# MingyuKim87/Safe_Denoiser

Hardware: AMD Instinct MI355X
Metric: images/sec (512x512, 50 steps, SD-v1.4 + repellency) (higher is better)
Workload: dtype bf16; 1 GPU; README-default end to end (safree = svf = lra = true, safree_neg_prompt_config.json:26-28): token ids -> CLIP -> SAFREE projection -> DDPM 50 steps x UNet on 3 guidance branches with per-prompt text switching + safe_denoiser.yaml repellency (kernel_fast, M=515, sigma 3.15, scale .33, margin 1.6, window 780<=t<=1000) -> VAE decode -> uint8 512x512 images; SD-v1.4 UNet / CLIP / VAE with random weigh; guidance_branches=3, text_encoder_precision=bf16x3, prompts_per_batch=64, latent_repeat=3, renoise_draws_rank0=3520, parallelism=prompt-shard x1

## Files before the change

include/sdn.h:

```cpp
#ifndef SDN_H_
#define SDN_H_

#include <stddef.h>
#include <stdint.h>

#ifdef __cplusplus
extern "C" {
#endif

#define SDN_OK            0
#define SDN_E_INVALID    -1
#define SDN_E_LAUNCH     -2
#define SDN_E_WORKSPACE  -3
#define SDN_E_ARCH       -4

int sdn_abi_version(void);
const char* sdn_device_arch_host(void);


#define SDN_REPEL_RBF     0
#define SDN_REPEL_SPARSE  1
#define SDN_QNORM_NONE    0
#define SDN_QNORM_CHANNEL 1
#define SDN_OUT_REPELLED  0
// ... 133 lines not shown
                          int32_t ld_mod, int32_t rows_per_batch, void* out, void* stream);

int sdn_patchify_bf16(const float* latents, int32_t batch, int32_t c, int32_t h, int32_t w, int32_t p, void* out, void* stream);
int sdn_patchify_f16(const float* latents, int32_t batch, int32_t c, int32_t h, int32_t w, int32_t p, void* out, void* stream);
int sdn_unpatchify_f32(const float* tokens, int32_t batch, int32_t c, int32_t h, int32_t w, int32_t p, float* out, void* stream);

int sdn_conv_in_bf16(const float* latents_nchw, const void* w, const float* bias, int32_t batch, int32_t cin,
                     int32_t h, int32_t wd, int32_t cout, void* out_nhwc, void* stream);
int sdn_conv_in_f16(const float* latents_nchw, const void* w, const float* bias, int32_t batch, int32_t cin,
                    int32_t h, int32_t wd, int32_t cout, void* out_nhwc, void* stream);

int sdn_timestep_embed_bf16(float timestep, int32_t batch, int32_t dim, void* out, void* stream);
int sdn_timestep_embed_f16(float timestep, int32_t batch, int32_t dim, void* out, void* stream);

int sdn_gemm_f32(const sdn_gemm_desc* d_host, const void* a, const void* a2, const void* w,
                 const float* bias, const float* rowbias, const float* rowgate, const void* residual, void* out,
                 void* stream);
int sdn_groupnorm_f32(const void* x, const void* x2, int32_t batch, int32_t hw, int32_t c1, int32_t c2,
                      int32_t groups, float eps, int32_t silu, const float* gamma, const float* beta,
                      void* out, float* stats_ws, void* stream);
int sdn_layernorm_f32(const void* x, int64_t rows, int32_t c, float eps, const float* gamma,
                      const float* beta, void* out, void* stream);
int sdn_attention_f32(const void* q, const void* k, const void* v, void* out, int32_t batch, int32_t heads,
                      int32_t nq, int32_t nk, int32_t head_dim, int32_t ldq, int32_t ldk, int32_t ldv,
                      int32_t ldo, float scale, void* stream);
int sdn_conv_in_f32(const float* latents_nchw, const void* w, const float* bias, int32_t batch, int32_t cin,
                    int32_t h, int32_t wd, int32_t cout, void* out_nhwc, void* stream);
int sdn_timestep_embed_f32(float timestep, int32_t batch, int32_t dim, void* out, void* stream);

int sdn_gemm_x3(const sdn_gemm_desc* d_host, const void* a, const void* a2, const void* w,
                const float* bias, const float* rowbias, const float* rowgate, const void* residual, void* out,
                void* stream);
int sdn_attention_x3(const void* q, const void* k, const void* v, void* out, int32_t batch, int32_t heads,
                     int32_t nq, int32_t nk, int32_t head_dim, int32_t ldq, int32_t ldk, int32_t ldv,
                     int32_t ldo, float scale, void* stream);

int sdn_layernorm_mod_f32(const void* x, int64_t rows, int32_t c, float eps, const float* scale, const float* shift,
                          int32_t ld_mod, int32_t rows_per_batch, void* out, void* stream);
int sdn_patchify_f32(const float* latents, int32_t batch, int32_t c, int32_t h, int32_t w, int32_t p, void* out, void* stream);
int sdn_joint_attention_f32(int32_t mode, const void* q, const void* k, const void* v, void* out,
                            const sdn_attn_segment2* seg2_host, int32_t batch, int32_t heads, int32_t n_total,
                            int32_t head_dim, int32_t ldq, int32_t ldk, int32_t ldv, int32_t ldo, float scale,
                            void* stream);

int sdn_split3(const float* x, const float* x2, int64_t rows, int32_t c1, int32_t c2, void* out_triple, void* stream);
int sdn_expand3_weights(const float* w, int64_t rows, int32_t cols, int32_t group, void* out_bf16, void* stream);
int sdn_groupnorm_f32_triple(const void* x, const void* x2, int32_t batch, int32_t hw, int32_t c1, int32_t c2, int32_t groups,
                             float eps, int32_t silu, const float* gamma, const float* beta, void* out_triple, float* stats_ws,
                             void* stream);
int sdn_layernorm_f32_triple(const void* x, int64_t rows, int32_t c, float eps, const float* gamma, const float* beta,
                             void* out_triple, void* stream);
int sdn_attention_x3_triple(const void* q, const void* k, const void* v, void* out_triple, int32_t batch, int32_t heads, int32_t nq,
                            int32_t nk, int32_t head_dim, int32_t ldq, int32_t ldk, int32_t ldv, int32_t ldo, float scale,
                            void* stream);
int sdn_attention_x3_pairs(const void* q, const void* k, const void* v, int32_t lo_offset_q, int32_t lo_offset_kv, void* out,
                           int32_t batch, int32_t heads, int32_t nq, int32_t nk, int32_t head_dim, int32_t ldq, int32_t ldk,
                           int32_t ldv, int32_t ldo, float scale, int32_t triple_out, void* stream);

int sdn_randn_philox_plan(int64_t numel, int32_t* grid_out, int64_t* offset_increment_out);
int sdn_randn_philox(const uint64_t* seeds, const uint64_t* offsets, const int32_t* rows, int32_t n_gen, int64_t numel,
                     float* out, void* stream);
int sdn_randn_philox_state(const uint64_t* seeds, uint64_t* offsets, const int32_t* flags, int32_t n_gen, int64_t numel,
                           float* out, void* stream);

typedef struct sdn_unet_config {
  int32_t in_channels, out_channels, sample_size;
  int32_t n_levels;
  int32_t block_out_channels[4];
  int32_t level_has_attn[4];
  int32_t layers_per_block;
  int32_t n_heads;
  int32_t cross_dim, text_len;
  int32_t norm_groups;
  int32_t dtype;
  int32_t latent_repeat;
} sdn_unet_config;

typedef struct sdn_unet sdn_unet;

#define SDN_P_VEC_F32     0
#define SDN_P_MAT         1
#define SDN_P_CONV3X3     2
#define SDN_P_GEGLU_MAT   3
#define SDN_P_GEGLU_VEC   4
#define SDN_P_POS_CROP    5
#define SDN_P_GLU_VALUE   7
#define SDN_P_GLU_GATE    8
#define SDN_P_DERIVED     6

typedef struct sdn_param_info {
  char     name[128];
  int32_t  kind;
  int32_t  rows, cols;
  int32_t  rows_padded;
  int64_t  offset;
} sdn_param_info;

int    sdn_unet_create(const sdn_unet_config* cfg_host, sdn_unet** out_host);
void   sdn_unet_destroy(sdn_unet* u);
int    sdn_unet_param_count(const sdn_unet* u);
int    sdn_unet_param_info(const sdn_unet* u, int32_t index, sdn_param_info* info_host);
size_t sdn_unet_weight_bytes(const sdn_unet* u);
size_t sdn_unet_workspace_bytes(sdn_unet* u, int32_t batch);
double sdn_unet_flops(sdn_unet* u, int32_t batch, double* attention_core_flops_host);

int sdn_unet_forward(sdn_unet* u, const void* weights, const float* latents, float timestep, const void* text,
                     float* out, int32_t batch, void* workspace, size_t workspace_bytes, void* stream);

typedef struct sdn_mmdit_config {
  int32_t in_channels, out_channels;
  int32_t sample_size, patch_size;
  int32_t num_layers;
  int32_t num_heads, head_dim;
  int32_t joint_dim, pooled_dim;
  int32_t text_len;
  int32_t time_dim;
  int32_t dtype;
} sdn_mmdit_config;
int sdn_mmdit_create(const sdn_mmdit_config* cfg_host, sdn_unet** out_host);
int sdn_mmdit_forward(sdn_unet* m, const void* weights, const float* latents, float timestep, const void* text,
                      const void* pooled, float* out, int32_t batch, void* workspace, size_t workspace_bytes,
                      void* stream);

int sdn_ln_fold(int32_t dtype, const void* w, const float* gamma, const float* beta, const float* bias, int32_t rows,
                int32_t cols, void* w_folded, float* c, float* d, void* stream);
int sdn_gemm_ln_bf16(const sdn_gemm_desc* desc, const void* a, const void* w_folded, const float* c, const float* d, float eps,
                     const float* row_stats, void* out, void* stream);
int sdn_gemm_ln_f16(const sdn_gemm_desc* desc, const void* a, const void* w_folded, const float* c, const float* d, float eps,
                    const float* row_stats, void* out, void* stream);
int sdn_row_stats_bf16(const void* x, int64_t rows, int32_t c, float eps, float* out, void* stream);
int sdn_row_stats_f16(const void* x, int64_t rows, int32_t c, float eps, float* out, void* stream);

int sdn_ffn_geglu_fused(int32_t dtype, int64_t M, int32_t C, const void* x, const float* row_stats, const void* w1_folded,
                        const float* c1, const float* d1, const void* w_cat, const float* b_cat, const void* residual, void* out,
                        float* col_stats, void* stream);

int sdn_gemm_stats_bf16(const sdn_gemm_desc* desc, const void* a, const void* a2, const void* w, const float* bias,
                        const float* rowbias, const void* residual, void* out, float* col_stats, void* stream);
int sdn_gemm_stats_f16(const sdn_gemm_desc* desc, const void* a, const void* a2, const void* w, const float* bias,
                       const float* rowbias, const void* residual, void* out, float* col_stats, void* stream);
int sdn_groupnorm_cols_bf16(const void* x, const void* x2, int32_t batch, int32_t hw, int32_t c1, int32_t c2, int32_t groups,
                            float eps, int32_t silu, const float* gamma, const float* beta, void* out, float* stats_ws,
                            const float* cols1, const float* cols2, void* stream);
int sdn_groupnorm_cols_f16(const void* x, const void* x2, int32_t batch, int32_t hw, int32_t c1, int32_t c2, int32_t groups,
                           float eps, int32_t silu, const float* gamma, const float* beta, void* out, float* stats_ws,
                           const float* cols1, const float* cols2, void* stream);

int sdn_gemm_splitk_bf16(const sdn_gemm_desc* d, const void* a, const void* a2, const void* w, const float* bias,
                         const float* rowbias, const float* rowgate, const void* residual, void* out, void* partials,
                         size_t partial_bytes, void* stream);
int sdn_gemm_splitk_f16(const sdn_gemm_desc* d, const void* a, const void* a2, const void* w, const float* bias,
                        const float* rowbias, const float* rowgate, const void* residual, void* out, void* partials,
                        size_t partial_bytes, void* stream);

int sdn_repeat(const void* in, size_t bytes, int32_t rep, void* out, void* stream);

int sdn_unet_prepare(sdn_unet* u, void* weights, void* stream);

typedef struct sdn_vae_config {
  int32_t latent_channels, out_channels;
  int32_t sample_size;
  int32_t n_levels;
  int32_t block_out_channels[4];
  int32_t layers_per_block;
  int32_t norm_groups;
  int32_t dtype;
} sdn_vae_config;
int sdn_vae_decoder_create(const sdn_vae_config* cfg_host, sdn_unet** out_host);
int sdn_vae_decode(sdn_unet* vae, const void* weights, const float* latents, float latent_scale, float* image,
                   int32_t batch, void* workspace, size_t workspace_bytes, void* stream);
int sdn_vae_encoder_create(const sdn_vae_config* cfg_host, sdn_unet** out_host);
int sdn_vae_encode(sdn_unet* vae_encoder, const void* weights, const float* image, float* moments, int32_t batch,
                   void* workspace, size_t workspace_bytes, void* stream);
int sdn_gaussian_sample(const float* moments, const float* noise, int32_t batch, int32_t latent_channels, int32_t hw,
                        float scale, float* out, void* stream);
int sdn_image_postprocess(const float* image_nchw, int32_t batch, int32_t channels, int32_t height, int32_t width,
                          float* out_nhwc01, uint8_t* out_nhwc_u8, void* stream);
int sdn_latent_mix(const float* z, const float* w, const float* bias, int32_t batch, int32_t channels, int32_t hw,
                   float in_scale, float* out, void* stream);
int sdn_softmax_rows(int32_t dtype, const float* scores, int64_t ld_scores, int64_t rows, int32_t n, float scale,
                     void* out, int64_t ld_out, void* stream);
int sdn_transpose16(const void* in, int32_t rows, int32_t cols, int64_t ld_in, void* out, int64_t ld_out, void* stream);

typedef struct sdn_clip_config {
  int32_t vocab_size;
  int32_t hidden_size, intermediate_size;
  int32_t num_layers, num_heads;
  int32_t max_position_embeddings;
  int32_t dtype;
} sdn_clip_config;
int sdn_clip_create(const sdn_clip_config* cfg_host, sdn_unet** out_host);
int sdn_clip_forward(sdn_unet* clip, const void* weights, const int32_t* input_ids, const int32_t* attention_mask,
                     void* last_hidden_state, int32_t batch, void* workspace, size_t workspace_bytes, void* stream);
int sdn_clip_embed(int32_t dtype, const int32_t* input_ids, const void* token_embedding, const void* position_embedding,
                   int64_t rows, int32_t seq_len, int32_t hidden, int32_t vocab, void* out, void* stream);
int sdn_masked_attention(int32_t dtype, const void* q, const void* k, const void* v, void* out, const int32_t* key_mask,
                         int32_t causal, int32_t batch, int32_t heads, int32_t n, int32_t head_dim, int32_t ldq,
                         int32_t ldk, int32_t ldv, int32_t ldo, float scale, void* stream);
int sdn_clip_embed_f32(const int32_t* input_ids, const void* token_embedding, const void* position_embedding, int64_t rows,
                       int32_t seq_len, int32_t hidden, int32_t vocab, void* out, void* stream);
int sdn_masked_attention_f32(const void* q, const void* k, const void* v, void* out, const int32_t* key_mask, int32_t causal,
                             int32_t batch, int32_t heads, int32_t n, int32_t head_dim, int32_t ldq, int32_t ldk, int32_t ldv,
                             int32_t ldo, float scale, void* stream);

typedef struct sdn_clip_proj_config {
  int32_t vocab_size;
  int32_t hidden_size, intermediate_size;
  int32_t num_layers, num_heads;
  int32_t max_position_embeddings;
  int32_t dtype;
  int32_t projection_dim;
  int32_t act;
  int32_t eos_token_id;
  int32_t hidden_tap;
} sdn_clip_proj_config;
int sdn_clip_proj_create(const sdn_clip_proj_config* cfg_host, sdn_unet** out_host);
int sdn_clip_proj_forward(sdn_unet* clip, const void* weights, const int32_t* input_ids, void* hidden, int64_t hidden_batch_stride,
                          int64_t hidden_row_stride, void* text_embeds, int64_t embeds_row_stride, int32_t batch, void* workspace,
                          size_t workspace_bytes, void* stream);
int sdn_clip_eos_rows(int32_t dtype, const int32_t* input_ids, const void* x, const float* gamma, const float* beta, int32_t batch,
                      int32_t seq_len, int32_t hidden, int32_t vocab, int32_t eos_token_id, float eps, void* out,
                      int32_t* positions, void* stream);
int sdn_copy_rows_strided(const void* src, int32_t batch, int32_t rows_per_batch, int32_t cols, int32_t elem_bytes, void* dst,
                          int64_t dst_batch_stride, int64_t dst_row_stride, void* stream);

typedef struct sdn_clip_vision_config {
  int32_t image_size, patch_size;
  int32_t hidden_size, intermediate_size;
  int32_t num_layers, num_heads;
  int32_t projection_dim;
  int32_t act;
  int32_t dtype;
} sdn_clip_vision_config;
int sdn_clip_vision_create(const sdn_clip_vision_config* cfg_host, sdn_unet** out_host);
int sdn_clip_vision_forward(sdn_unet* vision, const void* weights, const float* pixel_values, void* last_hidden_state,
                            void* image_embeds, int32_t batch, void* workspace, size_t workspace_bytes, void* stream);
int sdn_clip_patch_rows(int32_t dtype, const float* pixels, int32_t batch, int32_t image_size, int32_t patch_size, int32_t kpad,
                        void* out, void* stream);
int sdn_clip_vision_embed(int32_t dtype, const void* patch_proj, const float* class_embedding, const void* position_embedding,
                          const float* gamma, const float* beta, int32_t batch, int32_t tokens, int32_t hidden, float eps, void* out,
                          void* stream);
int sdn_clip_class_rows(int32_t dtype, const void* x, const float* gamma, const float* beta, int32_t batch, int32_t seq_len,
                        int32_t hidden, float eps, void* out, void* stream);
int sdn_image_resize_u8(const uint8_t* in, int32_t batch, int32_t in_size, int32_t out_size, const int32_t* coeffs,
                        const int32_t* bounds, int32_t ksize, uint8_t* tmp, uint8_t* out, void* stream);
int sdn_clip_normalize_u8(const uint8_t* in, int32_t batch, int32_t size, float mean_r, float mean_g, float mean_b, float std_r,
                          float std_g, float std_b, float* out, void* stream);
int sdn_embed_row_scores(const void* x, int32_t dtype_x, int64_t ldx, const void* y, int32_t dtype_y, int64_t ldy,
                         int32_t y_rows, int32_t rows, int32_t dim, int32_t normalize_y, float scale, float bias,
                         float* out, void* stream);
int sdn_image_resize_rect_u8(const uint8_t* in, int32_t batch, int32_t in_h, int32_t in_w, int32_t out_h, int32_t out_w,
                             const int32_t* coeffs_x, const int32_t* bounds_x, int32_t ksize_x, const int32_t* coeffs_y,
                             const int32_t* bounds_y, int32_t ksize_y, uint8_t* tmp, uint8_t* out_u8, float* out_f32, float mean_r,
                             float mean_g, float mean_b, float std_r, float std_g, float std_b, void* stream);

typedef struct sdn_t5_config {
  int32_t vocab_size;
  int32_t d_model, d_kv, d_ff;
  int32_t num_layers, num_heads;
  int32_t num_buckets, max_distance;
  float   eps;
  int32_t dtype;
} sdn_t5_config;
int sdn_t5_create(const sdn_t5_config* cfg_host, sdn_unet** out_host);
size_t sdn_t5_workspace_bytes(sdn_unet* t5, int32_t batch, int32_t n);
double sdn_t5_flops(sdn_unet* t5, int32_t batch, int32_t n, double* attention_core_flops_host);
int sdn_t5_forward(sdn_unet* t5, const void* weights, const int32_t* input_ids, const int32_t* attention_mask, int32_t n,
                   void* out, int32_t batch, void* workspace, size_t workspace_bytes, void* stream);
int sdn_rmsnorm(int32_t dtype, const void* x, int32_t x_is_f32, int64_t rows, int32_t c, float eps, const float* weight, void* out,
                void* stream);
int sdn_embed_tokens(int32_t dtype, const int32_t* input_ids, const void* token_embedding, int64_t rows, int32_t hidden,
                     int32_t vocab, float* out, void* stream);
int sdn_t5_bucket(int32_t relative_position, int32_t num_buckets, int32_t max_distance);
int sdn_t5_relative_bias(int32_t dtype, const void* table, int32_t num_buckets, int32_t max_distance, int32_t heads, int32_t n,
                         float* out, void* stream);
int sdn_bias_attention(int32_t dtype, const void* q, const void* k, const void* v, void* out, const float* bias,
                       const int32_t* key_mask, int32_t batch, int32_t heads, int32_t n, int32_t head_dim, int32_t ldq,
                       int32_t ldk, int32_t ldv, int32_t ldo, float scale, void* stream);

void sdn_unet_set_text_version(sdn_unet* u, uint64_t version);

void sdn_unet_set_graph_mode(sdn_unet* u, int32_t on);
void sdn_unet_set_split_k(sdn_unet* u, int32_t on);

typedef struct sdn_profile_row {
  char    kernel[24];
  int32_t launches;
  double  ms;
  double  flops;
  double  bytes;
} sdn_profile_row;
void sdn_unet_profile_next(sdn_unet* u);
int  sdn_unet_profile_read(sdn_unet* u, sdn_profile_row* rows_host, int32_t max_rows);

#ifdef __cplusplus
}
#endif
#endif
```

safe_denoiser_amd/_lib.py:

```python
from __future__ import annotations

import ctypes as C
import os

import torch

_HERE = os.path.dirname(os.path.abspath(__file__))
_LIB = None


class SdnUnavailable(RuntimeError):
    """libsdn.so is missing/unloadable, or there is no gfx950 device for a compute call."""


class SdnError(RuntimeError):
    """A libsdn entry point returned a negative status."""


_ERR = {-1: "SDN_E_INVALID (bad shape / null or misaligned pointer)", -2: "SDN_E_LAUNCH", -3: "SDN_E_WORKSPACE",
        -4: "SDN_E_ARCH"}


def lib_path() -> str:
    return os.environ.get("SDN_LIB", os.path.join(_HERE, "libsdn.so"))
# ... 44 lines not shown
class ClipProjConfig(C.Structure):
    _fields_ = [(n, C.c_int32) for n in ("vocab_size", "hidden_size", "intermediate_size", "num_layers", "num_heads",
                                         "max_position_embeddings", "dtype", "projection_dim", "act", "eos_token_id", "hidden_tap")]


class ClipVisionConfig(C.Structure):
    _fields_ = [(n, C.c_int32) for n in ("image_size", "patch_size", "hidden_size", "intermediate_size", "num_layers", "num_heads",
                                         "projection_dim", "act", "dtype")]


class T5Config(C.Structure):
    _fields_ = [(n, C.c_int32) for n in ("vocab_size", "d_model", "d_kv", "d_ff", "num_layers", "num_heads", "num_buckets",
                                         "max_distance")] + [("eps", C.c_float), ("dtype", C.c_int32)]


class AttnSegment2(C.Structure):
    _fields_ = [("q2", C.c_void_p), ("k2", C.c_void_p), ("v2", C.c_void_p), ("out2", C.c_void_p), ("n1", C.c_int32),
                ("ldq2", C.c_int32), ("ldk2", C.c_int32), ("ldv2", C.c_int32), ("ldo2", C.c_int32)]


class ParamInfo(C.Structure):
    _fields_ = [("name", C.c_char * 128), ("kind", C.c_int32), ("rows", C.c_int32), ("cols", C.c_int32),
                ("rows_padded", C.c_int32), ("offset", C.c_int64)]


_vp, _i32, _i64, _f32, _sz = C.c_void_p, C.c_int32, C.c_int64, C.c_float, C.c_size_t

SIGNATURES = {
    "sdn_abi_version": (C.c_int, []),
    "sdn_device_arch_host": (C.c_char_p, []),
    "sdn_repel_workspace_bytes": (_sz, [_i32, _i32, _i32, _i32]),
    "sdn_repel_apply": (C.c_int, [C.POINTER(RepelParams), _vp, _vp, _vp, _vp, _vp, _vp, _sz, _vp]),
    "sdn_repel_calibrate": (C.c_int, [C.POINTER(RepelParams), _vp, _vp, _vp, _vp, _sz, _vp]),
    "sdn_cfg_combine": (C.c_int, [_vp, _i32, _i32, _i64, _f32, _vp, _vp]),
    "sdn_sld_guidance": (C.c_int, [_vp, _i32, _i64, _f32, _f32, _f32, _f32, _f32, _i32, _vp, _vp, _vp]),
    "sdn_cfg_combine_rows": (C.c_int, [_vp, _i32, _i32, _i64, _vp, _vp, _vp]),
    "sdn_sld_guidance_rows": (C.c_int, [_vp, _i32, _i64, _vp, _f32, _f32, _f32, _f32, _i32, _vp, _vp, _vp]),
    "sdn_pred_x0": (C.c_int, [_vp, _vp, _i64, _f32, _f32, _f32, _vp, _vp]),
    "sdn_sched_step": (C.c_int, [_vp, _vp, _vp, _i64, _f32, _f32, _f32, _f32, _f32, _f32, _f32, _vp, _vp]),
    "sdn_add_noise": (C.c_int, [_vp, _vp, _i64, _f32, _f32, _vp, _vp]),
    "sdn_renoise_select": (C.c_int, [_vp, _vp, _vp, _vp, _i32, _i64, _f32, _f32, _vp]),
    "sdn_flow_euler_step": (C.c_int, [_vp, _vp, _i64, _f32, _f32, _vp, _vp]),
    "sdn_flow_endpoints": (C.c_int, [_vp, _vp, _i64, _f32, _vp, _vp, _vp]),
    "sdn_flow_renoise": (C.c_int, [_vp, _vp, _vp, _i64, _f32, _vp, _vp]),
    "sdn_gemm_bf16": (C.c_int, [C.POINTER(GemmDesc), _vp, _vp, _vp, _vp, _vp, _vp, _vp, _vp, _vp]),
    "sdn_gemm_f16": (C.c_int, [C.POINTER(GemmDesc), _vp, _vp, _vp, _vp, _vp, _vp, _vp, _vp, _vp]),
    "sdn_ln_fold": (C.c_int, [_i32, _vp, _vp, _vp, _vp, _i32, _i32, _vp, _vp, _vp, _vp]),
    "sdn_gemm_ln_bf16": (C.c_int, [C.POINTER(GemmDesc), _vp, _vp, _vp, _vp, _f32, _vp, _vp, _vp]),
    "sdn_gemm_ln_f16": (C.c_int, [C.POINTER(GemmDesc), _vp, _vp, _vp, _vp, _f32, _vp, _vp, _vp]),
    "sdn_row_stats_bf16": (C.c_int, [_vp, _i64, _i32, _f32, _vp, _vp]),
    "sdn_row_stats_f16": (C.c_int, [_vp, _i64, _i32, _f32, _vp, _vp]),
    "sdn_ffn_geglu_fused": (C.c_int, [_i32, _i64, _i32, _vp, _vp, _vp, _vp, _vp, _vp, _vp, _vp, _vp, _vp, _vp]),
    "sdn_gemm_stats_bf16": (C.c_int, [C.POINTER(GemmDesc), _vp, _vp, _vp, _vp, _vp, _vp, _vp, _vp, _vp]),
    "sdn_gemm_stats_f16": (C.c_int, [C.POINTER(GemmDesc), _vp, _vp, _vp, _vp, _vp, _vp, _vp, _vp, _vp]),
    "sdn_groupnorm_cols_bf16": (C.c_int, [_vp, _vp, _i32, _i32, _i32, _i32, _i32, _f32, _i32, _vp, _vp, _vp, _vp, _vp, _vp, _vp]),
    "sdn_groupnorm_cols_f16": (C.c_int, [_vp, _vp, _i32, _i32, _i32, _i32, _i32, _f32, _i32, _vp, _vp, _vp, _vp, _vp, _vp, _vp]),
    "sdn_gemm_splitk_bf16": (C.c_int, [C.POINTER(GemmDesc), _vp, _vp, _vp, _vp, _vp, _vp, _vp, _vp, _vp, _sz, _vp]),
    "sdn_gemm_splitk_f16": (C.c_int, [C.POINTER(GemmDesc), _vp, _vp, _vp, _vp, _vp, _vp, _vp, _vp, _vp, _sz, _vp]),
    "sdn_groupnorm_bf16": (C.c_int, [_vp, _vp, _i32, _i32, _i32, _i32, _i32, _f32, _i32, _vp, _vp, _vp, _vp, _vp]),
    "sdn_groupnorm_f16": (C.c_int, [_vp, _vp, _i32, _i32, _i32, _i32, _i32, _f32, _i32, _vp, _vp, _vp, _vp, _vp]),
    "sdn_layernorm_f16": (C.c_int, [_vp, _i64, _i32, _f32, _vp, _vp, _vp, _vp]),
    "sdn_conv_in_f16": (C.c_int, [_vp, _vp, _vp, _i32, _i32, _i32, _i32, _i32, _vp, _vp]),
    "sdn_timestep_embed_f16": (C.c_int, [_f32, _i32, _i32, _vp, _vp]),
    "sdn_layernorm_bf16": (C.c_int, [_vp, _i64, _i32, _f32, _vp, _vp, _vp, _vp]),
    "sdn_attention_bf16": (C.c_int, [_vp, _vp, _vp, _vp, _i32, _i32, _i32, _i32, _i32, _i32, _i32, _i32, _i32, _f32,
                                     _vp]),
    "sdn_attention_f16": (C.c_int, [_vp, _vp, _vp, _vp, _i32, _i32, _i32, _i32, _i32, _i32, _i32, _i32, _i32, _f32,
                                    _vp]),
    "sdn_conv_in_bf16": (C.c_int, [_vp, _vp, _vp, _i32, _i32, _i32, _i32, _i32, _vp, _vp]),
    "sdn_timestep_embed_bf16": (C.c_int, [_f32, _i32, _i32, _vp, _vp]),
    "sdn_gemm_f32": (C.c_int, [C.POINTER(GemmDesc), _vp, _vp, _vp, _vp, _vp, _vp, _vp, _vp, _vp]),
    "sdn_groupnorm_f32": (C.c_int, [_vp, _vp, _i32, _i32, _i32, _i32, _i32, _f32, _i32, _vp, _vp, _vp, _vp, _vp]),
    "sdn_layernorm_f32": (C.c_int, [_vp, _i64, _i32, _f32, _vp, _vp, _vp, _vp]),
    "sdn_attention_f32": (C.c_int, [_vp, _vp, _vp, _vp, _i32, _i32, _i32, _i32, _i32, _i32, _i32, _i32, _i32, _f32, _vp]),
    "sdn_randn_philox_plan": (C.c_int, [C.c_int64, C.POINTER(C.c_int32), C.POINTER(C.c_int64)]),
    "sdn_randn_philox": (C.c_int, [_vp, _vp, _vp, _i32, C.c_int64, _vp, _vp]),
    "sdn_randn_philox_state": (C.c_int, [_vp, _vp, _vp, _i32, C.c_int64, _vp, _vp]),
    "sdn_gemm_x3": (C.c_int, [C.POINTER(GemmDesc), _vp, _vp, _vp, _vp, _vp, _vp, _vp, _vp, _vp]),
    "sdn_attention_x3": (C.c_int, [_vp, _vp, _vp, _vp, _i32, _i32, _i32, _i32, _i32, _i32, _i32, _i32, _i32, _f32, _vp]),
    "sdn_conv_in_f32": (C.c_int, [_vp, _vp, _vp, _i32, _i32, _i32, _i32, _i32, _vp, _vp]),
    "sdn_timestep_embed_f32": (C.c_int, [_f32, _i32, _i32, _vp, _vp]),
    "sdn_unet_create": (C.c_int, [C.POINTER(UnetConfig), C.POINTER(_vp)]),
    "sdn_unet_destroy": (None, [_vp]),
    "sdn_unet_param_count": (C.c_int, [_vp]),
    "sdn_unet_param_info": (C.c_int, [_vp, _i32, C.POINTER(ParamInfo)]),
    "sdn_unet_weight_bytes": (_sz, [_vp]),
    "sdn_unet_workspace_bytes": (_sz, [_vp, _i32]),
    "sdn_unet_flops": (C.c_double, [_vp, _i32, C.POINTER(C.c_double)]),
    "sdn_unet_forward": (C.c_int, [_vp, _vp, _vp, _f32, _vp, _vp, _i32, _vp, _sz, _vp]),
    "sdn_mmdit_create": (C.c_int, [C.POINTER(MmditConfig), C.POINTER(_vp)]),
    "sdn_mmdit_forward": (C.c_int, [_vp, _vp, _vp, _f32, _vp, _vp, _vp, _i32, _vp, _sz, _vp]),
    "sdn_joint_attention": (C.c_int, [_i32, _vp, _vp, _vp, _vp, C.POINTER(AttnSegment2), _i32, _i32, _i32, _i32, _i32,
                                      _i32, _i32, _i32, _f32, _vp]),
    "sdn_layernorm_mod_bf16": (C.c_int, [_vp, _i64, _i32, _f32, _vp, _vp, _i32, _i32, _vp, _vp]),
    "sdn_layernorm_mod_f16": (C.c_int, [_vp, _i64, _i32, _f32, _vp, _vp, _i32, _i32, _vp, _vp]),
    "sdn_patchify_bf16": (C.c_int, [_vp, _i32, _i32, _i32, _i32, _i32, _vp, _vp]),
    "sdn_patchify_f16": (C.c_int, [_vp, _i32, _i32, _i32, _i32, _i32, _vp, _vp]),
    "sdn_unpatchify_f32": (C.c_int, [_vp, _i32, _i32, _i32, _i32, _i32, _vp, _vp]),
    "sdn_layernorm_mod_f32": (C.c_int, [_vp, _i64, _i32, _f32, _vp, _vp, _i32, _i32, _vp, _vp]),
    "sdn_patchify_f32": (C.c_int, [_vp, _i32, _i32, _i32, _i32, _i32, _vp, _vp]),
    "sdn_joint_attention_f32": (C.c_int, [_i32, _vp, _vp, _vp, _vp, C.POINTER(AttnSegment2), _i32, _i32, _i32, _i32, _i32,
                                          _i32, _i32, _i32, _f32, _vp]),
    "sdn_repeat": (C.c_int, [_vp, _sz, _i32, _vp, _vp]),
    "sdn_vae_decoder_create": (C.c_int, [C.POINTER(VaeConfig), C.POINTER(_vp)]),
    "sdn_vae_decode": (C.c_int, [_vp, _vp, _vp, _f32, _vp, _i32, _vp, _sz, _vp]),
    "sdn_vae_encoder_create": (C.c_int, [C.POINTER(VaeConfig), C.POINTER(_vp)]),
    "sdn_vae_encode": (C.c_int, [_vp, _vp, _vp, _vp, _i32, _vp, _sz, _vp]),
    "sdn_gaussian_sample": (C.c_int, [_vp, _vp, _i32, _i32, _i32, _f32, _vp, _vp]),
    "sdn_image_postprocess": (C.c_int, [_vp, _i32, _i32, _i32, _i32, _vp, _vp, _vp]),
    "sdn_latent_mix": (C.c_int, [_vp, _vp, _vp, _i32, _i32, _i32, _f32, _vp, _vp]),
    "sdn_softmax_rows": (C.c_int, [_i32, _vp, _i64, _i64, _i32, _f32, _vp, _i64, _vp]),
    "sdn_transpose16": (C.c_int, [_vp, _i32, _i32, _i64, _vp, _i64, _vp]),
    "sdn_clip_create": (C.c_int, [C.POINTER(ClipConfig), C.POINTER(_vp)]),
    "sdn_clip_forward": (C.c_int, [_vp, _vp, _vp, _vp, _vp, _i32, _vp, _sz, _vp]),
    "sdn_clip_embed": (C.c_int, [_i32, _vp, _vp, _vp, _i64, _i32, _i32, _i32, _vp, _vp]),
    "sdn_masked_attention": (C.c_int, [_i32, _vp, _vp, _vp, _vp, _vp, _i32, _i32, _i32, _i32, _i32, _i32, _i32, _i32, _i32,
                                       _f32, _vp]),
    "sdn_clip_proj_create": (C.c_int, [C.POINTER(ClipProjConfig), C.POINTER(_vp)]),
    "sdn_clip_proj_forward": (C.c_int, [_vp, _vp, _vp, _vp, _i64, _i64, _vp, _i64, _i32, _vp, _sz, _vp]),
    "sdn_clip_eos_rows": (C.c_int, [_i32, _vp, _vp, _vp, _vp, _i32, _i32, _i32, _i32, _i32, _f32, _vp, _vp, _vp]),
    "sdn_copy_rows_strided": (C.c_int, [_vp, _i32, _i32, _i32, _i32, _vp, _i64, _i64, _vp]),
    "sdn_clip_vision_create": (C.c_int, [C.POINTER(ClipVisionConfig), C.POINTER(_vp)]),
    "sdn_clip_vision_forward": (C.c_int, [_vp, _vp, _vp, _vp, _vp, _i32, _vp, _sz, _vp]),
    "sdn_clip_patch_rows": (C.c_int, [_i32, _vp, _i32, _i32, _i32, _i32, _vp, _vp]),
    "sdn_clip_vision_embed": (C.c_int, [_i32, _vp, _vp, _vp, _vp, _vp, _i32, _i32, _i32, _f32, _vp, _vp]),
    "sdn_clip_class_rows": (C.c_int, [_i32, _vp, _vp, _vp, _i32, _i32, _i32, _f32, _vp, _vp]),
    "sdn_image_resize_u8": (C.c_int, [_vp, _i32, _i32, _i32, _vp, _vp, _i32, _vp, _vp, _vp]),
    "sdn_clip_normalize_u8": (C.c_int, [_vp, _i32, _i32, _f32, _f32, _f32, _f32, _f32, _f32, _vp, _vp]),
    "sdn_image_resize_rect_u8": (C.c_int, [_vp, _i32, _i32, _i32, _i32, _i32, _vp, _vp, _i32, _vp, _vp, _i32, _vp, _vp, _vp, _f32, _f32,
                                           _f32, _f32, _f32, _f32, _vp]),
    "sdn_embed_row_scores": (C.c_int, [_vp, _i32, _i64, _vp, _i32, _i64, _i32, _i32, _i32, _i32, _f32, _f32, _vp, _vp]),
    "sdn_t5_create": (C.c_int, [C.POINTER(T5Config), C.POINTER(_vp)]),
    "sdn_t5_workspace_bytes": (_sz, [_vp, _i32, _i32]),
    "sdn_t5_flops": (C.c_double, [_vp, _i32, _i32, C.POINTER(C.c_double)]),
    "sdn_t5_forward": (C.c_int, [_vp, _vp, _vp, _vp, _i32, _vp, _i32, _vp, _sz, _vp]),
    "sdn_rmsnorm": (C.c_int, [_i32, _vp, _i32, _i64, _i32, _f32, _vp, _vp, _vp]),
    "sdn_embed_tokens": (C.c_int, [_i32, _vp, _vp, _i64, _i32, _i32, _vp, _vp]),
    "sdn_t5_bucket": (C.c_int, [_i32, _i32, _i32]),
    "sdn_t5_relative_bias": (C.c_int, [_i32, _vp, _i32, _i32, _i32, _i32, _vp, _vp]),
    "sdn_bias_attention": (C.c_int, [_i32, _vp, _vp, _vp, _vp, _vp, _vp, _i32, _i32, _i32, _i32, _i32, _i32, _i32, _i32, _f32,
                                     _vp]),
    "sdn_split3": (C.c_int, [_vp, _vp, _i64, _i32, _i32, _vp, _vp]),
    "sdn_expand3_weights": (C.c_int, [_vp, _i64, _i32, _i32, _vp, _vp]),
    "sdn_groupnorm_f32_triple": (C.c_int, [_vp, _vp, _i32, _i32, _i32, _i32, _i32, _f32, _i32, _vp, _vp, _vp, _vp, _vp]),
    "sdn_layernorm_f32_triple": (C.c_int, [_vp, _i64, _i32, _f32, _vp, _vp, _vp, _vp]),
    "sdn_attention_x3_triple": (C.c_int, [_vp, _vp, _vp, _vp, _i32, _i32, _i32, _i32, _i32, _i32, _i32, _i32, _i32, _f32, _vp]),
    "sdn_attention_x3_pairs": (C.c_int, [_vp, _vp, _vp, _i32, _i32, _vp, _i32, _i32, _i32, _i32, _i32, _i32, _i32, _i32, _i32, _f32, _i32, _vp]),
    "sdn_clip_embed_f32": (C.c_int, [_vp, _vp, _vp, _i64, _i32, _i32, _i32, _vp, _vp]),
    "sdn_masked_attention_f32": (C.c_int, [_vp, _vp, _vp, _vp, _vp, _i32, _i32, _i32, _i32, _i32, _i32, _i32, _i32, _i32, _f32, _vp]),
    "sdn_unet_prepare": (C.c_int, [_vp, _vp, _vp]),
    "sdn_unet_set_graph_mode": (None, [_vp, _i32]),
    "sdn_unet_set_text_version": (None, [_vp, C.c_uint64]),
    "sdn_unet_set_split_k": (None, [_vp, _i32]),
    "sdn_unet_profile_next": (None, [_vp]),
    "sdn_unet_profile_read": (C.c_int, [_vp, C.POINTER(ProfileRow), _i32]),
}


def lib():
    global _LIB
    if _LIB is None:
        path = lib_path()
        if not os.path.exists(path):
            raise SdnUnavailable(f"{path} not found: build it with `python -c 'import __graft_entry__ as g; g.build()'` "
                                 f"(or `make -C safe_denoiser_amd/csrc`).  There is no CPU fallback.")
        try:
            handle = C.CDLL(path)
        except OSError as e:
            raise SdnUnavailable(f"cannot load {path}: {e}") from e
        for name, (res, args) in SIGNATURES.items():
            fn = getattr(handle, name)
            fn.restype, fn.argtypes = res, args
        _LIB = handle
    return _LIB


def check(rc: int, what: str):
    if rc != 0:
        raise SdnError(f"{what} failed: {_ERR.get(rc, rc)}")


def require_gpu():
    if not torch.cuda.is_available():
        raise SdnUnavailable("no GPU visible: the safe-denoiser hot path only runs on an MI355X (gfx950); "
                             "there is no CPU fallback")


def dptr(t: torch.Tensor | None, dtype=None) -> int | None:
    if t is None:
        return None
    if not t.is_cuda:
        raise SdnUnavailable("tensor is not on the GPU: libsdn takes device pointers only (no CPU fallback)")
    if not t.is_contiguous():
        raise SdnError("tensor must be contiguous")
    if dtype is not None and t.dtype != dtype:
        raise SdnError(f"expected {dtype}, got {t.dtype}")
    return t.data_ptr()


def stream_ptr() -> int:
    return torch.cuda.current_stream().cuda_stream
```

safe_denoiser_amd/csrc/sdn_gemm.hip:

```cpp
#include <stdlib.h>

#include <type_traits>

#include "sdn_common.h"
#include "sdn_ops.h"

static int g_gemm_variant = 0;
static unsigned long long* g_gemm_stamps = nullptr;

#include "sdn_gemm_common.h"

namespace sdn_gemm_detail {

#define SDN_STAMP(IDX)                                                                                   \
  if (g.stamps && threadIdx.x == 0) {                                                                    \
    unsigned long long t_;                                                                               \
    asm volatile("s_memtime %0\n\ts_waitcnt lgkmcnt(0)" : "=s"(t_)::"memory");                          \
    g.stamps[(long)blockIdx.x * 8 + (IDX)] = t_;                                                         \
  }

template <typename T, int NREP, int WGM, int NSTAGE, int LNF, bool H8>
__device__ __forceinline__ void gemm_dma_body(const GemmArgs& g) {
#if defined(__HIP_DEVICE_COMPILE__)
  SDN_STAMP(0)
  constexpr int BM = 64 * WGM, THREADS = 128 * WGM, NWAVES = 2 * WGM;
  constexpr int BN = 32 * NREP;
  constexpr int A_PIECES = BM / 8 / NWAVES;
  constexpr int W_PIECES = (BN / 8 + NWAVES - 1) / NWAVES;
  constexpr int STAGE = (BM + BN) * 128;
  constexpr unsigned OOB = 0x80000000u;
  constexpr int LPI = A_PIECES + W_PIECES;
  static_assert(NSTAGE == 2 || (BN / 8) % NWAVES == 0, "counted waits need the same number of loads in every wave");
  __shared__ __attribute__((aligned(1024))) unsigned char smem[NSTAGE * STAGE];

  const int nt = g.tiles_m * g.tiles_n;
  const int tid = threadIdx.x, lane = tid & 63;
  const int wid = __builtin_amdgcn_readfirstlane(tid >> 6);
  const int wm = wid >> 1, wn = wid & 1;
  const int lrow = lane >> 3;
  int tile;
  {
    const int vid = blockIdx.x;
    const int q = nt >> 3, r = nt & 7, x = vid & 7;
    tile = (x < r ? x * (q + 1) : r * (q + 1) + (x - r) * q) + (vid >> 3);
  }
  int tm = tile / g.tiles_n, tn = tile - tm * g.tiles_n;
  if (g.panel) {
    const int per_blk = 8 * g.tiles_n;
    const int blk = tile / per_blk, rem = tile - blk * per_blk;
    const int rows = min(8, g.tiles_m - blk * 8);
    const int full = rows * g.panel;
    const int p = rem / full, r2 = rem - p * full;
    const int w = min(g.panel, g.tiles_n - p * g.panel);
    const int tl = r2 / w;
    tm = blk * 8 + tl; tn = p * g.panel + (r2 - tl * w);
  }
  const int m0 = tm * BM, n0 = tn * BN;
  const int lchunk = (lane & 7) ^ lrow;

  unsigned a_base[A_PIECES];
  unsigned a_aux[A_PIECES];
  const int ld1 = g.a_mode == 1 ? g.Cin : g.K1, ld2 = g.K - g.K1;
  if (g.a_mode == 1) {
    const int hw = g.Ho * g.Wo;
    const int Hi = g.upsample ? g.Hs * 2 : g.Hs, Wi = g.upsample ? g.Ws * 2 : g.Ws;
    const int mb = m0 + wid * A_PIECES * 8 + lrow;
    const int mm0 = mb < g.M ? mb : 0;
    int bb = mm0 / hw;
    int oy, ox;
    { const int p = mm0 - bb * hw; oy = p / g.Wo; ox = p - oy * g.Wo; }
#pragma unroll
    for (int i = 0; i < A_PIECES; ++i) {
      const int m = mb + i * 8;
      const bool ok = m < g.M;
      if (i > 0) {
        if (g.Wo >= 8) {
          ox += 8;
          if (ox >= g.Wo) { ox -= g.Wo; if (++oy >= g.Ho) { oy = 0; ++bb; } }
        } else {
          const int mm = ok ? m : 0;
          bb = mm / hw;
          const int p = mm - bb * hw;
          oy = p / g.Wo; ox = p - oy * g.Wo;
        }
      }
      const int cy = oy * g.stride + g.conv_off, cx = ox * g.stride + g.conv_off;
      const unsigned rb = (cy >= 1 ? 1u : 0u) | (cy < Hi ? 2u : 0u) | (cy + 1 < Hi ? 4u : 0u);
      const unsigned cb = (cx >= 1 ? 1u : 0u) | (cx < Wi ? 2u : 0u) | (cx + 1 < Wi ? 4u : 0u);
      unsigned mask = ((rb & 1u) ? cb : 0u) | ((rb & 2u) ? cb << 3 : 0u) | ((rb & 4u) ? cb << 6 : 0u);
      if (!ok) mask = 0u;
      a_aux[i] = mask | ((unsigned)(cy & 1) << 9) | ((unsigned)(cx & 1) << 10);
      const int sy = g.upsample ? cy >> 1 : cy, sx = g.upsample ? cx >> 1 : cx;
      a_base[i] = ok ? (unsigned)((((bb * g.Hs + sy) * g.Ws + sx) * g.Cin + lchunk * 8) * 2) : 0u;
    }
  } else {
#pragma unroll
    for (int i = 0; i < A_PIECES; ++i) {
      const int m = m0 + (wid * A_PIECES + i) * 8 + lrow;
      const bool ok = m < g.M;
      a_base[i] = ok ? (unsigned)(((long)m * ld1 + lchunk * 8) * 2) : OOB;
      a_aux[i] = (g.a2 && ok) ? (unsigned)(((long)m * ld2 + lchunk * 8) * 2) : OOB;
    }
  }
  unsigned w_off[W_PIECES];
  bool w_ok[W_PIECES];
#pragma unroll
  for (int i = 0; i < W_PIECES; ++i) {
    const int piece = wid * W_PIECES + i;
    w_ok[i] = piece * 8 < BN;
    w_off[i] = (unsigned)(((long)(n0 + piece * 8 + lrow) * g.K + lchunk * 8) * 2);
  }
  const __amdgpu_buffer_rsrc_t rs_w = make_rsrc(g.w, (unsigned)((long)g.N * g.K * 2));
  const long a_rows = g.a_mode == 1 ? (long)(g.M / (g.Ho * g.Wo)) * g.Hs * g.Ws : (long)g.M;
  const __amdgpu_buffer_rsrc_t rs_a1 = make_rsrc(g.a, (unsigned)(a_rows * ld1 * 2));
  const __amdgpu_buffer_rsrc_t rs_a2 = make_rsrc(g.a2 ? g.a2 : g.a, (unsigned)(g.a2 ? a_rows * ld2 * 2 : 0));

  const int kt0 = g.kt_per_split > 0 ? (int)blockIdx.y * g.kt_per_split : 0;
  int cur_k0 = kt0 * BK, cur_c0 = (kt0 / 9) * BK, cur_ty = (kt0 % 9) / 3, cur_tx = kt0 % 3, w_k0 = 0;
  auto issue_aw = [&](int buf, bool with_w) {
    unsigned char* sa = smem + buf * STAGE;
    unsigned char* sw = sa + BM * 128;
    if (g.a_mode == 1) {
      const int dy = cur_ty - 1, dx = cur_tx - 1, tap = cur_ty * 3 + cur_tx;
      if (!g.upsample) {
        const int delta = ((dy * g.Ws + dx) * g.Cin + cur_c0) * 2;
#pragma unroll
        for (int i = 0; i < A_PIECES; ++i) {
          const unsigned off = ((a_aux[i] >> tap) & 1u) ? a_base[i] + (unsigned)delta : OOB;
          __builtin_amdgcn_raw_ptr_buffer_load_lds(rs_a1, (lds_ptr_t)(sa + (wid * A_PIECES + i) * 1024), 16, off, 0, 0, 0);
        }
      } else {
#pragma unroll
        for (int i = 0; i < A_PIECES; ++i) {
          const int sy = ((int)((a_aux[i] >> 9) & 1u) + dy) >> 1, sx = ((int)((a_aux[i] >> 10) & 1u) + dx) >> 1;
          const int delta = ((sy * g.Ws + sx) * g.Cin + cur_c0) * 2;
          const unsigned off = ((a_aux[i] >> tap) & 1u) ? a_base[i] + (unsigned)delta : OOB;
          __builtin_amdgcn_raw_ptr_buffer_load_lds(rs_a1, (lds_ptr_t)(sa + (wid * A_PIECES + i) * 1024), 16, off, 0, 0, 0);
        }
      }
      w_k0 = (cur_ty * 3 + cur_tx) * g.Cin + cur_c0;
      if (++cur_tx == 3) { cur_tx = 0; if (++cur_ty == 3) { cur_ty = 0; cur_c0 += BK; } }
    } else {
      if (cur_k0 >= g.K1) {
        const unsigned kb = (unsigned)((cur_k0 - g.K1) * 2);
#pragma unroll
        for (int i = 0; i < A_PIECES; ++i)
          __builtin_amdgcn_raw_ptr_buffer_load_lds(rs_a2, (lds_ptr_t)(sa + (wid * A_PIECES + i) * 1024), 16, a_aux[i] + kb, 0, 0, 0);
      } else {
        const unsigned kb = (unsigned)(cur_k0 * 2);
#pragma unroll
        for (int i = 0; i < A_PIECES; ++i)
          __builtin_amdgcn_raw_ptr_buffer_load_lds(rs_a1, (lds_ptr_t)(sa + (wid * A_PIECES + i) * 1024), 16, a_base[i] + kb, 0, 0, 0);
      }
    }
    if (!with_w) return;
#pragma unroll
    for (int i = 0; i < W_PIECES; ++i) {
      if (w_ok[i])
        __builtin_amdgcn_raw_ptr_buffer_load_lds(rs_w, (lds_ptr_t)(sw + (wid * W_PIECES + i) * 1024), 16,
                                                 w_off[i] + (unsigned)((g.a_mode == 1 ? w_k0 : cur_k0) * 2), 0, 0, 0);
    }
    cur_k0 += BK;
  };
  auto issue = [&](int buf) { issue_aw(buf, true); };
  auto issue_w_only = [&](int buf) {
    unsigned char* sw = smem + buf * STAGE + BM * 128;
#pragma unroll
    for (int i = 0; i < W_PIECES; ++i) {
      if (w_ok[i])
        __builtin_amdgcn_raw_ptr_buffer_load_lds(rs_w, (lds_ptr_t)(sw + (wid * W_PIECES + i) * 1024), 16,
                                                 w_off[i] + (unsigned)((g.a_mode == 1 ? w_k0 : cur_k0) * 2), 0, 0, 0);
    }
    cur_k0 += BK;
  };

  const int fr = lane & 15, fq = lane >> 4;
  const int nk = g.kt_per_split > 0 ? min(g.kt_per_split, g.K / BK - kt0) : g.K / BK;
  SDN_STAMP(7)
  if constexpr (NSTAGE == 2) issue(0);
  f32x4 acc[4][NREP];
  if (g.bias) {
    f32x4 bv[NREP];
#pragma unroll
    for (int j = 0; j < NREP; ++j) bv[j] = *reinterpret_cast<const f32x4*>(g.bias + n0 + wn * 16 * NREP + j * 16 + fq * 4);
#pragma unroll
    for (int i = 0; i < 4; ++i)
#pragma unroll
      for (int j = 0; j < NREP; ++j) acc[i][j] = bv[j];
  } else {
#pragma unroll
    for (int i = 0; i < 4; ++i)
#pragma unroll
      for (int j = 0; j < NREP; ++j) acc[i][j] = (f32x4){0.f, 0.f, 0.f, 0.f};
  }
  if (g.rowbias) {
#pragma unroll
    for (int i = 0; i < 4; ++i) {
      const int m = m0 + wm * 64 + i * 16 + fr;
      const int b = m < g.M ? m / g.rows_per_batch : 0;
      const float* rbp = g.rowbias + (long)b * g.ld_rowbias + n0 + wn * 16 * NREP + fq * 4;
#pragma unroll
      for (int j = 0; j < NREP; ++j) acc[i][j] += *reinterpret_cast<const f32x4*>(rbp + j * 16);
    }
  }

  if (g.res_pre) {
    const unsigned short* r16 = reinterpret_cast<const unsigned short*>(g.res_pre);
#pragma unroll
    for (int i = 0; i < 4; ++i) {
      const int m = m0 + wm * 64 + i * 16 + fr;
      const unsigned short* rp = r16 + (long)(m < g.M ? m : 0) * g.ldc + n0 + wn * 16 * NREP + fq * 4;
#pragma unroll
      for (int j = 0; j < NREP; ++j) {
        const uint2 rr = *reinterpret_cast<const uint2*>(rp + j * 16);
        acc[i][j][0] += T::to_f(rr.x & 0xffff); acc[i][j][1] += T::to_f(rr.x >> 16);
        acc[i][j][2] += T::to_f(rr.y & 0xffff); acc[i][j][3] += T::to_f(rr.y >> 16);
      }
    }
  }
  if (g.x3_out && g.residual) {
    const float* resf = reinterpret_cast<const float*>(g.residual);
#pragma unroll
    for (int i = 0; i < 4; ++i) {
      const int m = m0 + wm * 64 + i * 16 + fr;
      const float* rp = resf + (long)(m < g.M ? m : 0) * g.ldc + n0 + wn * 16 * NREP + fq * 4;
#pragma unroll
      for (int j = 0; j < NREP; ++j) acc[i][j] += *reinterpret_cast<const f32x4*>(rp + j * 16);
    }
  }

  if constexpr (NSTAGE == 2) {
    asm volatile("s_waitcnt vmcnt(0)" ::: "memory");
    __syncthreads();
  } else {
#pragma unroll
    for (int s = 0; s < NSTAGE - 1; ++s) issue(s);
    asm volatile("s_waitcnt vmcnt(%0)" ::"n"((NSTAGE - 2) * LPI) : "memory");
    __builtin_amdgcn_s_barrier();
  }
  SDN_STAMP(1)

  [[maybe_unused]] float ln_s1[4] = {0.f, 0.f, 0.f, 0.f}, ln_s2[4] = {0.f, 0.f, 0.f, 0.f};
  [[maybe_unused]] float ln_mu[4], ln_rs[4];
  if constexpr (LNF == 2) {
#pragma unroll
    for (int i = 0; i < 4; ++i) {
      const int m = m0 + wm * 64 + i * 16 + fr;
      const float2 st2 = *reinterpret_cast<const float2*>(g.ln_stats + 2 * (long)(m < g.M ? m : 0));
      ln_mu[i] = st2.x; ln_rs[i] = st2.y;
    }
  }
  auto k_iter = [&](const int kt, auto f8_c) __attribute__((always_inline)) {
    const int buf = kt & (NSTAGE - 1);
    int ipos = (NSTAGE == 2 && WGM == 4 && !(g.dbg & 8)) ? ((g.dbg & 4) ? 1 : (g.a_mode == 1 ? 2 : ((g.act == 2 && g.K >= 1280) ? 1 : 4))) : 0;
    if (NSTAGE == 2 && WGM == 4 && !(g.dbg & (32 | 8 | 4))) ipos = ((wid >= 4) != ((g.dbg & 64) != 0)) ? 0 : ((g.dbg & 128) ? ipos : 2);
    const bool more = kt + NSTAGE - 1 < nk && !(g.dbg & 2);
    if (ipos == 0 && more) issue((kt + NSTAGE - 1) & (NSTAGE - 1));
    const unsigned char* sa = smem + buf * STAGE + (wm * 64) * 128;
    const unsigned char* sw = smem + buf * STAGE + BM * 128 + (wn * 16 * NREP) * 128;
#ifdef SDN_NO_FRAG_PIPE
    constexpr bool kFragPipe = false;
#else
    constexpr bool kFragPipe = WGM == 4 && (NREP == 10 || NREP == 8) && LNF != 1;
#endif
    constexpr bool f8_tile = decltype(f8_c)::value;
    if constexpr (H8 && f8_tile) {
      {
        typedef __attribute__((ext_vector_type(8))) int i32x8;
        union F8 { typename T::v8 h[2]; i32x8 v; };
        const bool seg1 = kt < g.h8_t16 + (nk - g.h8_t16) / 2;
        const int s_act = seg1 ? 0x74747474 : 0x7f7f7f7f, s_w = seg1 ? 0x7f7f7f7f : 0x74747474;
        F8 av[4], wv[3];
#pragma unroll
        for (int i = 0; i < 4; ++i) {
          av[i].h[0] = *reinterpret_cast<const typename T::v8*>(sa + lds_off(i * 16 + fr, fq));
          av[i].h[1] = *reinterpret_cast<const typename T::v8*>(sa + lds_off(i * 16 + fr, 4 + fq));
        }
#pragma unroll
        for (int j = 0; j < 2; ++j) {
          wv[j].h[0] = *reinterpret_cast<const typename T::v8*>(sw + lds_off(j * 16 + fr, fq));
          wv[j].h[1] = *reinterpret_cast<const typename T::v8*>(sw + lds_off(j * 16 + fr, 4 + fq));
        }
        __builtin_amdgcn_sched_barrier(0);
#pragma unroll
        for (int j = 0; j < NREP; ++j) {
          if (j + 2 < NREP) {
            wv[(j + 2) % 3].h[0] = *reinterpret_cast<const typename T::v8*>(sw + lds_off((j + 2) * 16 + fr, fq));
            wv[(j + 2) % 3].h[1] = *reinterpret_cast<const typename T::v8*>(sw + lds_off((j + 2) * 16 + fr, 4 + fq));
          }
          __builtin_amdgcn_sched_barrier(0);
          __builtin_amdgcn_s_setprio(1);
#pragma unroll
          for (int i = 0; i < 4; ++i)
            acc[i][j] = __builtin_amdgcn_mfma_scale_f32_16x16x128_f8f6f4(wv[j % 3].v, av[i].v, acc[i][j], 0, 0, 0, s_w, 0, s_act);
          __builtin_amdgcn_s_setprio(0);
          __builtin_amdgcn_sched_barrier(0);
          if (j == NREP / 2 - 1 && more && ipos != 0) issue((kt + 1) & 1);
        }
      }
    }
    if constexpr (kFragPipe) {
      if constexpr (!f8_tile) {
      typename T::v8 fa[2][4], fw[2][2];
#pragma unroll
      for (int i = 0; i < 4; ++i) fa[0][i] = *reinterpret_cast<const typename T::v8*>(sa + lds_off(i * 16 + fr, fq));
#pragma unroll
      for (int j = 0; j < 2; ++j) fw[0][j] = *reinterpret_cast<const typename T::v8*>(sw + lds_off(j * 16 + fr, fq));
      constexpr int G = NREP / 2;
#pragma unroll
      for (int gi = 0; gi < 2 * G; ++gi) {
        const int ks = gi / G, g = gi % G;
        if (gi + 1 < 2 * G) {
          const int ks1 = (gi + 1) / G, g1 = (gi + 1) % G;
#pragma unroll
          for (int j = 0; j < 2; ++j)
            fw[(gi + 1) & 1][j] = *reinterpret_cast<const typename T::v8*>(sw + lds_off((2 * g1 + j) * 16 + fr, ks1 * 4 + fq));
        }
        if (gi == 2) {
#pragma unroll
          for (int i = 0; i < 4; ++i) fa[1][i] = *reinterpret_cast<const typename T::v8*>(sa + lds_off(i * 16 + fr, 4 + fq));
        }
        __builtin_amdgcn_s_setprio(1);
#pragma unroll
        for (int i = 0; i < 4; ++i)
#pragma unroll
          for (int j = 0; j < 2; ++j) acc[i][2 * g + j] = T::mfma16(fw[gi & 1][j], fa[ks][i], acc[i][2 * g + j]);
        __builtin_amdgcn_s_setprio(0);
        if (gi == 2 && more) { if (ipos == 1) issue((kt + 1) & 1); else if (ipos == 4) issue_aw((kt + 1) & 1, false); }
        if (gi == G - 1 && more) { if (ipos == 2) issue((kt + 1) & 1); else if (ipos == 4) issue_w_only((kt + 1) & 1); }
      }
      }
    } else {
#pragma unroll
    for (int ks = 0; ks < 2; ++ks) {
      constexpr int JC = NREP > 5 ? NREP / 2 : NREP;
      typename T::v8 fa[4];
#pragma unroll
      for (int i = 0; i < 4; ++i) fa[i] = *reinterpret_cast<const typename T::v8*>(sa + lds_off(i * 16 + fr, ks * 4 + fq));
      if constexpr (LNF == 1) {
#pragma unroll
        for (int i = 0; i < 4; ++i) { ln_s1[i] = T::dot_ones(fa[i], ln_s1[i]); ln_s2[i] = T::dot_self(fa[i], ln_s2[i]); }
      }
#define SDN_MMA_PART(J0)                                                                                              \
      {                                                                                                                \
        typename T::v8 fw[JC];                                                                                         \
        _Pragma("unroll") for (int j = 0; j < JC; ++j)                                                                 \
          fw[j] = *reinterpret_cast<const typename T::v8*>(sw + lds_off(((J0) + j) * 16 + fr, ks * 4 + fq));          \
        _Pragma("unroll") for (int i = 0; i < 4; ++i)                                                                  \
          _Pragma("unroll") for (int j = 0; j < JC; ++j)                                                               \
            acc[i][(J0) + j] = T::mfma16(fw[j], fa[i], acc[i][(J0) + j]);                                              \
      }
      __builtin_amdgcn_s_setprio(1);
      SDN_MMA_PART(0)
      __builtin_amdgcn_s_setprio(0);
      if (ipos == 1 && ks == 0 && more) issue((kt + 1) & 1);
      if (ipos == 4 && ks == 0 && more) issue_aw((kt + 1) & 1, false);
      __builtin_amdgcn_s_setprio(1);
      if constexpr (NREP > JC) SDN_MMA_PART(JC)
      __builtin_amdgcn_s_setprio(0);
#undef SDN_MMA_PART
      if (ipos == 2 && ks == 0 && more) issue((kt + 1) & 1);
      if (ipos == 4 && ks == 0 && more) issue_w_only((kt + 1) & 1);
    }
    }
    if constexpr (NSTAGE == 2) {
      asm volatile("s_waitcnt vmcnt(0)" ::: "memory");
      __syncthreads();
    } else {
      const int later = nk - kt - 2;
      if (later >= NSTAGE - 2) asm volatile("s_waitcnt vmcnt(%0)" ::"n"((NSTAGE - 2) * LPI) : "memory");
      else if (later == 1 && NSTAGE > 3) asm volatile("s_waitcnt vmcnt(%0)" ::"n"(LPI) : "memory");
      else asm volatile("s_waitcnt vmcnt(0)" ::: "memory");
      asm volatile("s_waitcnt lgkmcnt(0)" ::: "memory");
      __builtin_amdgcn_s_barrier();
    }
    };
  if constexpr (H8) {
    for (int kt = 0; kt < g.h8_t16; ++kt) k_iter(kt, std::false_type{});
    for (int kt = g.h8_t16; kt < nk; ++kt) k_iter(kt, std::true_type{});
  } else {
    for (int kt = 0; kt < nk; ++kt) k_iter(kt, std::false_type{});
  }

  SDN_STAMP(2)
  if constexpr (LNF == 1) {
    const float invk = 1.0f / (float)g.K;
#pragma unroll
    for (int i = 0; i < 4; ++i) {
      float a1 = ln_s1[i], a2 = ln_s2[i];
      a1 += __shfl_xor(a1, 16, 64); a2 += __shfl_xor(a2, 16, 64);
      a1 += __shfl_xor(a1, 32, 64); a2 += __shfl_xor(a2, 32, 64);
      const float mu = a1 * invk;
      const float var = fmaxf(a2 * invk - mu * mu, 0.f);
      ln_mu[i] = mu; ln_rs[i] = __builtin_amdgcn_rsqf(var + g.ln_eps);
    }
  }
  constexpr int CW_PAD = (BN + 8) * 2;
  const bool staged = g.out_kind == 0 && g.n_valid == g.N;
  const int out_cols = g.act == 2 ? BN / 2 : BN;
  const bool res_lds = staged && g.res_lds;
  const int CW = res_lds ? BN * 2 : CW_PAD;
  const bool lean = staged && !g.rowgate && g.act == 0 && (res_lds || !g.residual);
  const bool lean_gelu = staged && !g.rowgate && g.act == 3 && !g.residual;
  const bool lean_erf = g.act == SDN_ACT_GELU;
  const bool lean_gate = staged && g.rowgate && g.act == 0 && res_lds;
  const __amdgpu_buffer_rsrc_t rs_res = make_rsrc(g.residual ? g.residual : g.a, g.res_bytes);
  constexpr int PASSES = (BM * CW_PAD + 2 * STAGE - 1) / (2 * STAGE);
  constexpr int WM_PER_PASS = WGM / PASSES, ROWS_PER_PASS = 64 * WM_PER_PASS;
  static_assert(WGM % PASSES == 0, "pass split must divide the wave rows");
  static_assert(PASSES <= 2, "epilogue is written for at most two staging passes");
#define SDN_PASS 0
#include "sdn_gemm_epilogue.inc"
#undef SDN_PASS
  if constexpr (PASSES > 1) {
#define SDN_PASS 1
#include "sdn_gemm_epilogue.inc"
#undef SDN_PASS
  }
  SDN_STAMP(3)
#endif
}

template <typename T, int NREP, int WGM, int NSTAGE, int LNF = 0>
__global__ void __launch_bounds__(128 * WGM, NSTAGE > 2 ? 1 : 2)
k_gemm_dma(const GemmArgs g) { gemm_dma_body<T, NREP, WGM, NSTAGE, LNF, false>(g); }

template <typename T, int NREP>
__global__ void __launch_bounds__(512, 2)
k_gemm_h8(const GemmArgs g) { gemm_dma_body<T, NREP, 4, 2, 0, true>(g); }


template <typename T>
__global__ void __launch_bounds__(256)
k_splitk_reduce(const float* __restrict__ part, int splits, long slice, int M, int N, const float* __restrict__ bias,
                const float* __restrict__ rowbias, int ld_rowbias, const float* __restrict__ rowgate, int ld_rowgate,
                int rows_per_batch, const unsigned short* __restrict__ residual, int residual_bcast, int ldc, int act,
                unsigned short* __restrict__ out) {
  const int nq = N / 4;
  const long total = (long)M * nq;
  for (long e = (long)blockIdx.x * 256 + threadIdx.x; e < total; e += (long)gridDim.x * 256) {
    const int m = (int)(e / nq), n = (int)(e - (long)m * nq) * 4;
    f32x4 v = *reinterpret_cast<const f32x4*>(part + (long)m * N + n);
    for (int s = 1; s < splits; ++s) v += *reinterpret_cast<const f32x4*>(part + (long)s * slice + (long)m * N + n);
    if (bias) v += *reinterpret_cast<const f32x4*>(bias + n);
    const int b = rows_per_batch > 0 ? m / rows_per_batch : 0;
    if (rowbias) v += *reinterpret_cast<const f32x4*>(rowbias + (long)b * ld_rowbias + n);
    if (rowgate) v *= *reinterpret_cast<const f32x4*>(rowgate + (long)b * ld_rowgate + n);
    if (residual) {
      const long rrow = residual_bcast ? (long)(m - b * rows_per_batch) : (long)m;
      const uint2 rr = *reinterpret_cast<const uint2*>(residual + rrow * ldc + n);
      v[0] += T::to_f(rr.x & 0xffff); v[1] += T::to_f(rr.x >> 16); v[2] += T::to_f(rr.y & 0xffff); v[3] += T::to_f(rr.y >> 16);
    }
    if (act == 1) { v[0] = silu_f(v[0]); v[1] = silu_f(v[1]); v[2] = silu_f(v[2]); v[3] = silu_f(v[3]); }
    if (act == 3) { v[0] = gelu_tanh(v[0]); v[1] = gelu_tanh(v[1]); v[2] = gelu_tanh(v[2]); v[3] = gelu_tanh(v[3]); }
    if (act == 4) { v[0] = quick_gelu(v[0]); v[1] = quick_gelu(v[1]); v[2] = quick_gelu(v[2]); v[3] = quick_gelu(v[3]); }
    uint2 pk; pk.x = T::pack2(v[0], v[1]); pk.y = T::pack2(v[2], v[3]);
    *reinterpret_cast<uint2*>(out + (long)m * ldc + n) = pk;
  }
}

}

int sdn_gemm_pick_split(int M, int N, int K, int act, int out_kind) {
  if (act == SDN_ACT_GEGLU_TANH) act = SDN_ACT_GEGLU;
  if (out_kind != SDN_OUT_BF16 || act == SDN_ACT_GEGLU || (N & 3)) return 1;
  const int nrep = sdn_gemm_pick_tile(M, N, K, act, 0);
  const int bm = nrep >= 8 ? 256 : 128;
  const long tiles = (long)((M + bm - 1) / bm) * (N / (32 * nrep));
  const int nk = K / 64;
  if (tiles >= 96 || nk < 16) return 1;
  int s = (int)(256 / tiles);
  if (s > nk / 8) s = nk / 8;
  if (s > 16) s = 16;
  return s < 2 ? 1 : s;
}

namespace sdn_gemm_detail {

template <typename T, int NREP, int WGM, int NSTAGE = 2, int LNF = 0>
int launch_dma(const GemmArgs& ga, hipStream_t st) {
  const int grid = ga.tiles_m * ga.tiles_n;
  const int splits = ga.kt_per_split > 0 ? (ga.K / BK + ga.kt_per_split - 1) / ga.kt_per_split : 1;
  record_gemm_launch(ga.kt_per_split > 0 ? 3 : 1, T::kDtype, NREP, WGM, NSTAGE, LNF, ga.tiles_m, ga.tiles_n, splits, 0);
  hipLaunchKernelGGL((k_gemm_dma<T, NREP, WGM, NSTAGE, LNF>), dim3(grid, splits), dim3(128 * WGM), 0, st, ga);
  return sdn_launch_status();
}

template <typename T>
int dispatch_dma(int nrep, const GemmArgs& g, hipStream_t st) {
  if (g.h8_t16 > 0) {
    if constexpr (T::kDtype == 1) {
      const int grid = g.tiles_m * g.tiles_n;
      if (nrep == 10) hipLaunchKernelGGL((k_gemm_h8<T, 10>), dim3(grid), dim3(512), 0, st, g);
      else if (nrep == 8) hipLaunchKernelGGL((k_gemm_h8<T, 8>), dim3(grid), dim3(512), 0, st, g);
      else return SDN_E_INVALID;
      return sdn_launch_status();
    } else {
      return SDN_E_INVALID;
    }
  }
  if (g.ln_c && g.ln_stats) {
    switch (nrep) {
      case 10: return launch_dma<T, 10, 4, 2, 2>(g, st);
      case 5: return launch_dma<T, 5, 2, 2, 2>(g, st);
      case 4: return launch_dma<T, 4, 2, 2, 2>(g, st);
      case 2: return launch_dma<T, 2, 2, 2, 2>(g, st);
      default: return SDN_E_INVALID;
    }
  }
  if (g.ln_c) {
    switch (nrep) {
      case 10: return launch_dma<T, 10, 4, 2, 1>(g, st);
      case 5: return launch_dma<T, 5, 2, 2, 1>(g, st);
      case 2: return launch_dma<T, 2, 2, 2, 1>(g, st);
      default: return SDN_E_INVALID;
    }
  }
  switch (nrep) {
    case 10: return launch_dma<T, 10, 4>(g, st);
    case 8: return launch_dma<T, 8, 4>(g, st);
    case 5:
      if (g.tiles_m * g.tiles_n <= 256 && g.K >= 8 * BK && g.kt_per_split == 0 && g_gemm_variant != 5) return launch_dma<T, 5, 2, 4>(g, st);
      return launch_dma<T, 5, 2>(g, st);
    case 4: return launch_dma<T, 4, 2>(g, st);
    case 2: return launch_dma<T, 2, 2>(g, st);
    default: return launch_dma<T, 1, 2>(g, st);
  }
}

inline bool al16(const void* p) { return (reinterpret_cast<uintptr_t>(p) & 15) == 0; }

}
using namespace sdn_gemm_detail;

int sdn_gemm_pick_nrep(int n_padded, int act) {
  if (act == SDN_ACT_GEGLU_TANH) act = SDN_ACT_GEGLU;
  if (act == SDN_ACT_GEGLU) return (n_padded % 128 == 0) ? 4 : ((n_padded % 64 == 0) ? 2 : 0);
  if (n_padded % 160 == 0) return 5;
  if (n_padded % 128 == 0) return 4;
  if (n_padded % 64 == 0) return 2;
  if (n_padded % 32 == 0) return 1;
  return 0;
}

extern "C" void sdn_debug_set_gemm_variant(int v) { g_gemm_variant = v; }
static long long g_gemm_launches[2] = {0, 0};
extern "C" void sdn_debug_gemm_launch_counts(long long* out2, int reset) {
  if (out2) { out2[0] = g_gemm_launches[0]; out2[1] = g_gemm_launches[1]; }
  if (reset) g_gemm_launches[0] = g_gemm_launches[1] = 0;
}
extern "C" void sdn_debug_set_gemm_stamps(void* p) { g_gemm_stamps = (unsigned long long*)p; }
static int g_last_launch[SDN_LL_COUNT] = {0};
void sdn_gemm_detail::record_gemm_launch(int family, int dtype, int nrep, int wgm, int nstage, int lnf, int tiles_m, int tiles_n,
                                         int splits, int aux) {
  const int v[SDN_LL_COUNT] = {family, dtype, nrep, wgm, nstage, lnf, tiles_m, tiles_n, splits, aux};
  for (int i = 0; i < SDN_LL_COUNT; ++i) g_last_launch[i] = v[i];
}
extern "C" void sdn_debug_gemm_last_launch(int* out, int n) {
  for (int i = 0; out && i < n; ++i) out[i] = i < SDN_LL_COUNT ? g_last_launch[i] : 0;
}

int sdn_gemm_pick_tile(int M, int N, int K, int act, int epilogue_reads) {
  if (act == SDN_ACT_GEGLU_TANH) act = SDN_ACT_GEGLU;
  int nrep = sdn_gemm_pick_nrep(N, act);
  if (g_gemm_variant == 2) return nrep;
  if (g_gemm_variant != 3) {
    int big = (N % 320 == 0) ? 10 : ((N % 256 == 0) ? 8 : 0);
    if (big == 10 && N % 256 == 0 && act == SDN_ACT_NONE && g_gemm_variant != 14) {
      const long tm = (M + 255) / 256;
      const long w10 = (tm * (N / 320) + 255) / 256 * 320, w8 = (tm * (N / 256) + 255) / 256 * 256;
      if (w8 < w10) big = 8;
    }
    const bool long_k = K >= 2048 || (K >= 1280 && act == SDN_ACT_GEGLU) || (K >= 1536 && (act == SDN_ACT_NONE || act == SDN_ACT_GELU_TANH));
    const bool short_ok = !epilogue_reads && K >= 320 && g_gemm_variant != 9;
    if (big && (long_k || short_ok)) {
      const long tiles = (long)((M + 255) / 256) * (N / (32 * big));
      if (tiles >= 192) return big;
    }
  }
  const int tiles_m = (M + 127) / 128;
  if (nrep > 2 && N % 64 == 0 && tiles_m * (N / (32 * nrep)) < 256) nrep = 2;
  return nrep;
}

static int sdn_gemm_impl(int dtype, const sdn_gemm_desc* d, const void* a, const void* a2, const void* w,
                         const float* bias, const float* rowbias, const float* rowgate, const void* residual, void* out,
                         void* stream, void* partials = nullptr, size_t partial_bytes = 0, const float* ln_c = nullptr,
                         const float* ln_d = nullptr, float ln_eps = 0.f, const float* ln_stats = nullptr, float* col_stats = nullptr) {
  if (!d || !a || !w || !out) return SDN_E_INVALID;
  sdn_gemm_desc dd = *d;
  const bool glu_tanh = dd.act == SDN_ACT_GEGLU_TANH;
  const bool stream32 = dd.f32_stream != 0;
  if (glu_tanh) {
    if (dd.x3_out || stream32 || ln_c || ln_d || partials || dd.split_k > 1 || col_stats) return SDN_E_INVALID;
    dd.act = SDN_ACT_GEGLU;
  }
  if (stream32) {
    if (dd.f32_stream != 1 || dd.x3_out || dd.act != SDN_ACT_NONE || dd.a_mode != SDN_A_PLAIN || dd.res_pre || dd.residual_bcast ||
        dd.out_kind != SDN_OUT_F32 || rowgate || dd.split_k > 1 || partials || ln_c || ln_d || col_stats || (dd.n_valid > 0 && dd.n_valid != dd.N))
      return SDN_E_INVALID;
  }
  d = &dd;
  if (d->M < 0 || d->N <= 0 || d->K <= 0 || (d->K % BK) != 0) return SDN_E_INVALID;
  if (d->M == 0) return SDN_OK;
  const int n_valid = d->n_valid > 0 ? d->n_valid : d->N;
  if (n_valid > d->N) return SDN_E_INVALID;
  if (sdn_gemm_pick_nrep(d->N, d->act) == 0) return SDN_E_INVALID;
  const int x3 = stream32 ? 1 : d->x3_out;
  const bool h8 = x3 == 5;
  if (x3 < 0 || x3 > 5 || (x3 && !stream32 && ((dtype != 0) != h8 || rowgate || d->split_k > 1 || partials || ln_c || col_stats || n_valid != d->N)))
    return SDN_E_INVALID;
  if (h8 && (d->a_mode != SDN_A_PLAIN || d->act != SDN_ACT_NONE || (d->K % 256) != 0 || d->res_pre || (d->K1 > 0 && d->K1 < d->K)))
    return SDN_E_INVALID;
  if (x3 && ((x3 == 2) != (d->act == SDN_ACT_GEGLU) || (x3 != 2 && d->act != SDN_ACT_NONE) || (residual && !al16(residual)) || !al16(out)))
    return SDN_E_INVALID;
  const bool res_pre = d->res_pre && residual && !x3 && !rowgate && !d->residual_bcast && d->split_k <= 1 && !partials && !ln_c &&
                       d->out_kind == SDN_OUT_BF16 && n_valid == d->N && d->act == SDN_ACT_NONE;
  int nrep = sdn_gemm_pick_tile(d->M, d->N, d->K, d->act, ((residual && !x3 && !res_pre) || rowgate) ? 1 : 0);
  if ((ln_c || ln_d) && nrep == 8 && d->N % 320 == 0) nrep = 10;
  if (h8) {
    if (d->N % 256 == 0) nrep = 8;
    else if (nrep < 8) return SDN_E_INVALID;
  }
  if (!al16(a) || !al16(w) || (a2 && !al16(a2)) || (residual && (reinterpret_cast<uintptr_t>(residual) & 7)) ||
      (reinterpret_cast<uintptr_t>(out) & 7) || (bias && !al16(bias)) || (rowbias && !al16(rowbias)))
    return SDN_E_INVALID;
  GemmArgs g{};
  g.a = (const __bf16*)a; g.a2 = (const __bf16*)a2; g.w = (const __bf16*)w;
  g.bias = bias; g.rowbias = rowbias; g.rowgate = rowgate; g.residual = res_pre ? nullptr : (const __bf16*)residual; g.out = out;
  g.res_pre = res_pre ? (const __bf16*)residual : nullptr;
  g.M = d->M; g.N = d->N; g.K = d->K;
  g.a_mode = d->a_mode;
  if (d->a_mode == SDN_A_PLAIN) {
    g.K1 = (d->K1 > 0 && d->K1 < d->K) ? d->K1 : d->K;
    if (g.K1 != d->K && (!a2 || (g.K1 % BK) != 0)) return SDN_E_INVALID;
  } else if (d->a_mode == SDN_A_CONV3X3) {
    if (d->Cin <= 0 || (d->Cin % BK) != 0 || d->K != 9 * d->Cin || d->Hs <= 0 || d->Ws <= 0 || d->Ho <= 0 ||
        d->Wo <= 0 || (d->stride != 1 && d->stride != 2) || d->M % (d->Ho * d->Wo) != 0)
      return SDN_E_INVALID;
    const int Hi = d->upsample ? 2 * d->Hs : d->Hs, Wi = d->upsample ? 2 * d->Ws : d->Ws;
    if (d->asym_pad != 0 && (d->asym_pad != 1 || d->stride != 2 || d->upsample)) return SDN_E_INVALID;
    const int pad2 = d->asym_pad ? 1 : 2;
    if ((Hi + pad2 - 3) / d->stride + 1 != d->Ho || (Wi + pad2 - 3) / d->stride + 1 != d->Wo) return SDN_E_INVALID;
    g.K1 = d->K; g.Hs = d->Hs; g.Ws = d->Ws; g.Cin = d->Cin; g.Ho = d->Ho; g.Wo = d->Wo; g.stride = d->stride;
    g.upsample = d->upsample; g.conv_off = d->asym_pad ? 1 : 0;
  } else {
    return SDN_E_INVALID;
  }
  if (d->act < 0 || (d->act > 4 && d->act != SDN_ACT_GELU) || d->out_kind < 0 || d->out_kind > 2) return SDN_E_INVALID;
  if (d->act == SDN_ACT_GELU && (x3 || d->out_kind != SDN_OUT_BF16 || n_valid != d->N || rowgate || residual || d->split_k > 1 || partials ||
                                 ln_c || ln_d || col_stats))
    return SDN_E_INVALID;
  if (d->act == SDN_ACT_GEGLU && ((d->out_kind != SDN_OUT_BF16 && !x3) || rowbias || rowgate || residual || n_valid != d->N))
    return SDN_E_INVALID;
  if ((rowbias || rowgate || d->residual_bcast || d->out_kind == SDN_OUT_F32_NCHW) && d->rows_per_batch <= 0) return SDN_E_INVALID;
  if (rowgate && !al16(rowgate)) return SDN_E_INVALID;
  g.x3_out = h8 ? 1 : x3;
  g.glu_tanh = glu_tanh ? 1 : 0;
  g.h8_t16 = h8 ? d->K / 128 : 0;
  g.act = d->act; g.out_kind = x3 ? SDN_OUT_F32 : d->out_kind; g.rows_per_batch = d->rows_per_batch; g.ld_rowbias = d->ld_rowbias;
  g.ld_rowgate = d->ld_rowgate; g.residual_bcast = d->residual_bcast;
  g.n_valid = n_valid;
  g.ldc = d->ldc > 0 ? d->ldc : (d->act == SDN_ACT_GEGLU ? d->N / 2 : n_valid);
  if (!x3 && d->out_kind == SDN_OUT_BF16 && ((g.ldc & 7) || !al16(out))) return SDN_E_INVALID;
  if (x3 && (g.ldc & 3)) return SDN_E_INVALID;
  const int bn = 32 * nrep;
  const int bm = nrep >= 8 ? 256 : 128;
  g.tiles_m = (d->M + bm - 1) / bm; g.tiles_n = d->N / bn;
  {
    const long res_rows = d->residual_bcast ? (long)d->rows_per_batch : (long)d->M;
    const long res_bytes = res_rows * g.ldc * 2;
    g.res_lds = !x3 && !res_pre && residual != nullptr && al16(residual) && res_bytes < (1L << 31) && g_gemm_variant != 4;
    g.res_bytes = g.res_lds ? (unsigned)res_bytes : 0u;
  }
  if (col_stats) {
    if (d->out_kind != SDN_OUT_BF16 || n_valid != d->N || d->act == SDN_ACT_GEGLU || d->split_k > 1 ||
        (reinterpret_cast<uintptr_t>(col_stats) & 7))
      return SDN_E_INVALID;
    g.col_stats = col_stats;
  }
  if (ln_c || ln_d) {
    if (!ln_c || !ln_d || !al16(ln_c) || !al16(ln_d) || d->a_mode != SDN_A_PLAIN || g.K1 != d->K || bias || rowbias || rowgate ||
        residual || d->out_kind != SDN_OUT_BF16 || n_valid != d->N || d->split_k > 1 ||
        (d->act != SDN_ACT_NONE && d->act != SDN_ACT_GEGLU) || (ln_stats && (reinterpret_cast<uintptr_t>(ln_stats) & 7)) ||
        (ln_stats ? (nrep != 10 && nrep != 5 && nrep != 4 && nrep != 2) : (nrep != 10 && nrep != 5 && nrep != 2)))
      return SDN_E_INVALID;
    g.ln_c = ln_c; g.ln_d = ln_d; g.ln_eps = ln_eps; g.ln_stats = ln_stats;
  }
  g.panel = (g.tiles_n > 4 && g_gemm_variant != 15) ? 4 : 0;
  g.dbg = g_gemm_variant >= 16 ? (g_gemm_variant >> 4) : 0;
  g.stamps = g_gemm_stamps;
  hipStream_t st = (hipStream_t)stream;
  const long a_rows = d->a_mode == SDN_A_CONV3X3 ? (long)(d->M / (d->Ho * d->Wo)) * d->Hs * d->Ws : (long)d->M;
  const long a_ld1 = d->a_mode == SDN_A_CONV3X3 ? d->Cin : g.K1, a_ld2 = d->a_mode == SDN_A_CONV3X3 ? 0 : d->K - g.K1;
  if (a_rows * a_ld1 * 2 >= (1L << 31) || a_rows * a_ld2 * 2 >= (1L << 31) || (long)d->N * d->K * 2 >= (1L << 31))
    return SDN_E_INVALID;
  if (d->split_k > 1) {
    const int nk = d->K / BK;
    if (!partials || d->out_kind != SDN_OUT_BF16 || d->act == SDN_ACT_GEGLU || n_valid != d->N || (d->N & 3) || d->split_k > nk ||
        (reinterpret_cast<uintptr_t>(partials) & 15))
      return SDN_E_INVALID;
    const int per = (nk + d->split_k - 1) / d->split_k, splits = (nk + per - 1) / per;
    const long slice = (long)d->M * d->N;
    if (partial_bytes < (size_t)splits * slice * 4) return SDN_E_WORKSPACE;
    GemmArgs gp = g;
    gp.bias = nullptr; gp.rowbias = nullptr; gp.rowgate = nullptr; gp.residual = nullptr; gp.res_lds = 0; gp.res_bytes = 0;
    gp.act = 0; gp.out_kind = SDN_OUT_F32; gp.out = partials; gp.ldc = d->N; gp.n_valid = d->N;
    gp.kt_per_split = per; gp.split_stride = slice * 4;
    const int rc = dtype == 0 ? dispatch_dma<SdnBF16>(nrep, gp, st) : dispatch_dma<SdnF16>(nrep, gp, st);
    if (rc != SDN_OK) return rc;
    const long total = slice / 4;
    long grid = (total + 255) / 256;
    if (grid > 4096) grid = 4096;
    if (dtype == 0)
      hipLaunchKernelGGL((k_splitk_reduce<SdnBF16>), dim3((unsigned)grid), dim3(256), 0, st, (const float*)partials, splits, slice,
                         d->M, d->N, bias, rowbias, d->ld_rowbias, rowgate, d->ld_rowgate, d->rows_per_batch,
                         (const unsigned short*)residual, d->residual_bcast, g.ldc, d->act, (unsigned short*)out);
    else
      hipLaunchKernelGGL((k_splitk_reduce<SdnF16>), dim3((unsigned)grid), dim3(256), 0, st, (const float*)partials, splits, slice,
                         d->M, d->N, bias, rowbias, d->ld_rowbias, rowgate, d->ld_rowgate, d->rows_per_batch,
                         (const unsigned short*)residual, d->residual_bcast, g.ldc, d->act, (unsigned short*)out);
    return sdn_launch_status();
  }
  if (nrep == 10 && g_gemm_variant != 13) {
    const int rc = dispatch_conv_slab(dtype, g, st);
    if (rc != SDN_GEMM_NOT_SLAB) { ++g_gemm_launches[0]; return rc; }
  }
  ++g_gemm_launches[1];
  return dtype == 0 ? dispatch_dma<SdnBF16>(nrep, g, st) : dispatch_dma<SdnF16>(nrep, g, st);
}

extern "C" int sdn_gemm_bf16(const sdn_gemm_desc* d, const void* a, const void* a2, const void* w, const float* bias,
                             const float* rowbias, const float* rowgate, const void* residual, void* out, void* stream) {
  return sdn_gemm_impl(0, d, a, a2, w, bias, rowbias, rowgate, residual, out, stream);
}
extern "C" int sdn_gemm_f16(const sdn_gemm_desc* d, const void* a, const void* a2, const void* w, const float* bias,
                            const float* rowbias, const float* rowgate, const void* residual, void* out, void* stream) {
  return sdn_gemm_impl(1, d, a, a2, w, bias, rowbias, rowgate, residual, out, stream);
}

extern "C" int sdn_gemm_stats_bf16(const sdn_gemm_desc* d, const void* a, const void* a2, const void* w, const float* bias,
                                   const float* rowbias, const void* residual, void* out, float* col_stats, void* stream) {
  if (!col_stats) return SDN_E_INVALID;
  return sdn_gemm_impl(0, d, a, a2, w, bias, rowbias, nullptr, residual, out, stream, nullptr, 0, nullptr, nullptr, 0.f, nullptr, col_stats);
}
extern "C" int sdn_gemm_stats_f16(const sdn_gemm_desc* d, const void* a, const void* a2, const void* w, const float* bias,
                                  const float* rowbias, const void* residual, void* out, float* col_stats, void* stream) {
  if (!col_stats) return SDN_E_INVALID;
  return sdn_gemm_impl(1, d, a, a2, w, bias, rowbias, nullptr, residual, out, stream, nullptr, 0, nullptr, nullptr, 0.f, nullptr, col_stats);
}

extern "C" int sdn_gemm_splitk_bf16(const sdn_gemm_desc* d, const void* a, const void* a2, const void* w, const float* bias,
                                    const float* rowbias, const float* rowgate, const void* residual, void* out, void* partials,
                                    size_t partial_bytes, void* stream) {
  return sdn_gemm_impl(0, d, a, a2, w, bias, rowbias, rowgate, residual, out, stream, partials, partial_bytes);
}
extern "C" int sdn_gemm_splitk_f16(const sdn_gemm_desc* d, const void* a, const void* a2, const void* w, const float* bias,
                                   const float* rowbias, const float* rowgate, const void* residual, void* out, void* partials,
                                   size_t partial_bytes, void* stream) {
  return sdn_gemm_impl(1, d, a, a2, w, bias, rowbias, rowgate, residual, out, stream, partials, partial_bytes);
}

extern "C" int sdn_gemm_ln_bf16(const sdn_gemm_desc* d, const void* a, const void* w_folded, const float* c, const float* dvec,
                                float eps, const float* row_stats, void* out, void* stream) {
  return sdn_gemm_impl(0, d, a, nullptr, w_folded, nullptr, nullptr, nullptr, nullptr, out, stream, nullptr, 0, c, dvec, eps, row_stats);
}
extern "C" int sdn_gemm_ln_f16(const sdn_gemm_desc* d, const void* a, const void* w_folded, const float* c, const float* dvec,
                               float eps, const float* row_stats, void* out, void* stream) {
  return sdn_gemm_impl(1, d, a, nullptr, w_folded, nullptr, nullptr, nullptr, nullptr, out, stream, nullptr, 0, c, dvec, eps, row_stats);
}

namespace {
template <typename T>
__global__ void __launch_bounds__(256)
k_ln_fold(const unsigned short* __restrict__ w, const float* __restrict__ gamma, const float* __restrict__ beta,
          const float* __restrict__ bias, int K, unsigned short* __restrict__ wf, float* __restrict__ c, float* __restrict__ dvec) {
  __shared__ float red[8];
  const long n = blockIdx.x;
  float sc = 0.f, sd = 0.f;
  for (int k = threadIdx.x; k < K; k += 256) {
    const float wv = T::to_f(w[n * K + k]);
    const unsigned r = T::pack2(wv * gamma[k], 0.f) & 0xffffu;
    wf[n * K + k] = (unsigned short)r;
    sc += T::to_f(r);
    sd = fmaf(beta[k], wv, sd);
  }
  sc = block_sum<4>(sc, red);
  sd = block_sum<4>(sd, red + 4);
  if (threadIdx.x == 0) { c[n] = sc; dvec[n] = sd + (bias ? bias[n] : 0.f); }
}
}

extern "C" int sdn_ln_fold(int32_t dtype, const void* w, const float* gamma, const float* beta, const float* bias, int32_t rows,
                           int32_t cols, void* w_folded, float* c, float* dvec, void* stream) {
  if (!w || !gamma || !beta || !w_folded || !c || !dvec || rows <= 0 || cols <= 0 || dtype < 0 || dtype > 1) return SDN_E_INVALID;
  if (dtype == 1)
    hipLaunchKernelGGL((k_ln_fold<SdnF16>), dim3(rows), dim3(256), 0, (hipStream_t)stream, (const unsigned short*)w, gamma, beta,
                       bias, cols, (unsigned short*)w_folded, c, dvec);
  else
    hipLaunchKernelGGL((k_ln_fold<SdnBF16>), dim3(rows), dim3(256), 0, (hipStream_t)stream, (const unsigned short*)w, gamma, beta,
                       bias, cols, (unsigned short*)w_folded, c, dvec);
  return sdn_launch_status();
}

namespace {
template <typename T>
__global__ void __launch_bounds__(256)
k_linear_pair_fold(const unsigned short* __restrict__ wa, const unsigned short* __restrict__ wb, const float* __restrict__ ba,
                   const float* __restrict__ bb, int C, int K, unsigned short* __restrict__ wcat, float* __restrict__ bcat) {
  const int n = blockIdx.y;
  const int k = blockIdx.x * 256 + threadIdx.x;
  const int KC = K + C;
  if (k < K) {
    float acc = 0.f;
    for (int j = 0; j < C; ++j) acc = fmaf(T::to_f(wb[(long)n * C + j]), T::to_f(wa[(long)j * K + k]), acc);
    wcat[(long)n * KC + k] = (unsigned short)(T::pack2(acc, 0.f) & 0xffffu);
  } else if (k < KC) {
    wcat[(long)n * KC + k] = wb[(long)n * C + (k - K)];
  }
  if (blockIdx.x == 0 && threadIdx.x == 0) {
    float acc = bb ? bb[n] : 0.f;
    if (ba) for (int j = 0; j < C; ++j) acc = fmaf(T::to_f(wb[(long)n * C + j]), ba[j], acc);
    bcat[n] = acc;
  }
}
}

int sdn_linear_pair_fold(int dtype, const void* wa, const void* wb, const float* ba, const float* bb, int C, int K, void* w_cat,
                         float* b_cat, void* stream) {
  if (!wa || !wb || !w_cat || !b_cat || C <= 0 || K <= 0 || dtype < 0 || dtype > 1) return SDN_E_INVALID;
  const dim3 grid((K + C + 255) / 256, C);
  if (dtype == 1)
    hipLaunchKernelGGL((k_linear_pair_fold<SdnF16>), grid, dim3(256), 0, (hipStream_t)stream, (const unsigned short*)wa,
                       (const unsigned short*)wb, ba, bb, C, K, (unsigned short*)w_cat, b_cat);
  else
    hipLaunchKernelGGL((k_linear_pair_fold<SdnBF16>), grid, dim3(256), 0, (hipStream_t)stream, (const unsigned short*)wa,
                       (const unsigned short*)wb, ba, bb, C, K, (unsigned short*)w_cat, b_cat);
  return sdn_launch_status();
}
```

safe_denoiser_amd/csrc/sdn_gemm_epilogue.inc:

```
{
  constexpr int pass = SDN_PASS;
  if (pass > 0) __syncthreads();
#ifndef SDN_EPI_RES_PRELOADED
  if (res_lds) {
    constexpr int CPR = BN / 8;
    constexpr int RES_PIECES = ROWS_PER_PASS * CPR / 64 / NWAVES;
    static_assert(RES_PIECES * 64 * NWAVES == ROWS_PER_PASS * CPR, "residual slab must split into whole 1-KiB pieces per wave");
#pragma unroll
    for (int q = 0; q < RES_PIECES; ++q) {
      const int piece = wid * RES_PIECES + q;
      const int e = piece * 64 + lane;
      const int r = e / CPR, c = e - r * CPR;
      const int m = m0 + pass * ROWS_PER_PASS + r;
      const int rrow = g.residual_bcast ? m % g.rows_per_batch : m;
      const unsigned off = m < g.M ? (unsigned)(((long)rrow * g.ldc + n0 + c * 8) * 2) : OOB;
      __builtin_amdgcn_raw_ptr_buffer_load_lds(rs_res, (lds_ptr_t)(smem + piece * 1024), 16, off, 0, 0, 0);
    }
    asm volatile("s_waitcnt vmcnt(0)" ::: "memory");
    __syncthreads();
  }
#endif
  if (wm / WM_PER_PASS == pass) {
  if (g.x3_out) {
    if (g.x3_out == 1) {
// ... 114 lines not shown
      const int ml = (wm % WM_PER_PASS) * 64 + i * 16 + fr;
#pragma unroll
      for (int j = 0; j + 1 < NREP; j += 2) {
        const f32x4 hv = acc[i][j], gv = acc[i][j + 1];
        uint2 pk;
        pk.x = T::pack2(hv[0] * gelu_tanh(gv[0]), hv[1] * gelu_tanh(gv[1]));
        pk.y = T::pack2(hv[2] * gelu_tanh(gv[2]), hv[3] * gelu_tanh(gv[3]));
        const int nl = ((wn * 16 * NREP + j * 16) >> 1) + fq * 4;
        *reinterpret_cast<uint2*>(smem + ml * CW_PAD + nl * 2) = pk;
      }
    }
  } else if (g.act == 2) {
#pragma unroll
    for (int i = 0; i < 4; ++i) {
      const int ml = (wm % WM_PER_PASS) * 64 + i * 16 + fr;
#pragma unroll
      for (int j = 0; j + 1 < NREP; j += 2) {
        const f32x4 hv = acc[i][j], gv = acc[i][j + 1];
        uint2 pk;
        pk.x = T::pack2(hv[0] * gelu_erf(gv[0]), hv[1] * gelu_erf(gv[1]));
        pk.y = T::pack2(hv[2] * gelu_erf(gv[2]), hv[3] * gelu_erf(gv[3]));
        const int nl = ((wn * 16 * NREP + j * 16) >> 1) + fq * 4;
        *reinterpret_cast<uint2*>(smem + ml * CW_PAD + nl * 2) = pk;
      }
    }
  } else if (lean && res_lds) {
    unsigned char* slot0 = smem + ((wm % WM_PER_PASS) * 64 + fr) * (BN * 2) + (wn * 16 * NREP + fq * 4) * 2;
#pragma unroll
    for (int i = 0; i < 4; ++i)
#pragma unroll
      for (int j = 0; j < NREP; ++j) {
        uint2* slot = reinterpret_cast<uint2*>(slot0 + i * 16 * (BN * 2) + j * 32);
        const uint2 rr = *slot;
        const f32x4 v = acc[i][j];
        uint2 pk;
        pk.x = T::pack2(v[0] + T::to_f(rr.x & 0xffff), v[1] + T::to_f(rr.x >> 16));
        pk.y = T::pack2(v[2] + T::to_f(rr.y & 0xffff), v[3] + T::to_f(rr.y >> 16));
        *slot = pk;
      }
  } else if (lean) {
    unsigned char* slot0 = smem + ((wm % WM_PER_PASS) * 64 + fr) * CW_PAD + (wn * 16 * NREP + fq * 4) * 2;
#pragma unroll
    for (int i = 0; i < 4; ++i)
#pragma unroll
      for (int j = 0; j < NREP; ++j) {
        const f32x4 v = acc[i][j];
        uint2 pk; pk.x = T::pack2(v[0], v[1]); pk.y = T::pack2(v[2], v[3]);
        *reinterpret_cast<uint2*>(slot0 + i * 16 * CW_PAD + j * 32) = pk;
      }
  } else if (lean_gelu) {
    unsigned char* slot0 = smem + ((wm % WM_PER_PASS) * 64 + fr) * CW_PAD + (wn * 16 * NREP + fq * 4) * 2;
#pragma unroll
    for (int i = 0; i < 4; ++i)
#pragma unroll
      for (int j = 0; j < NREP; ++j) {
        const f32x4 v = acc[i][j];
        uint2 pk; pk.x = T::pack2(gelu_tanh(v[0]), gelu_tanh(v[1])); pk.y = T::pack2(gelu_tanh(v[2]), gelu_tanh(v[3]));
        *reinterpret_cast<uint2*>(slot0 + i * 16 * CW_PAD + j * 32) = pk;
      }
  } else if (lean_erf) {
    unsigned char* slot0 = smem + ((wm % WM_PER_PASS) * 64 + fr) * CW_PAD + (wn * 16 * NREP + fq * 4) * 2;
#pragma unroll
    for (int i = 0; i < 4; ++i)
#pragma unroll
      for (int j = 0; j < NREP; ++j) {
        const f32x4 v = acc[i][j];
        uint2 pk; pk.x = T::pack2(gelu_erf(v[0]), gelu_erf(v[1])); pk.y = T::pack2(gelu_erf(v[2]), gelu_erf(v[3]));
        *reinterpret_cast<uint2*>(slot0 + i * 16 * CW_PAD + j * 32) = pk;
      }
  } else if (lean_gate) {
    unsigned char* slot0 = smem + ((wm % WM_PER_PASS) * 64 + fr) * (BN * 2) + (wn * 16 * NREP + fq * 4) * 2;
#pragma unroll
    for (int i = 0; i < 4; ++i) {
      const int m = m0 + pass * ROWS_PER_PASS + (wm % WM_PER_PASS) * 64 + i * 16 + fr;
      const int b = m < g.M ? m / g.rows_per_batch : 0;
      const float* gp = g.rowgate + (long)b * g.ld_rowgate + n0 + wn * 16 * NREP + fq * 4;
      f32x4 gt[NREP];
#pragma unroll
      for (int j = 0; j < NREP; ++j) gt[j] = *reinterpret_cast<const f32x4*>(gp + j * 16);
#pragma unroll
      for (int j = 0; j < NREP; ++j) {
        uint2* slot = reinterpret_cast<uint2*>(slot0 + i * 16 * (BN * 2) + j * 32);
        const uint2 rr = *slot;
        const f32x4 v = acc[i][j] * gt[j];
        uint2 pk;
        pk.x = T::pack2(v[0] + T::to_f(rr.x & 0xffff), v[1] + T::to_f(rr.x >> 16));
        pk.y = T::pack2(v[2] + T::to_f(rr.y & 0xffff), v[3] + T::to_f(rr.y >> 16));
        *slot = pk;
      }
    }
  } else {
#pragma unroll
  for (int i = 0; i < 4; ++i) {
    const int ml = (wm % WM_PER_PASS) * 64 + i * 16 + fr;
    const int m = m0 + pass * ROWS_PER_PASS + ml;
    const bool row_ok = m < g.M;
    const int b = (g.rows_per_batch > 0 && row_ok) ? m / g.rows_per_batch : 0;
    unsigned short* out16 = reinterpret_cast<unsigned short*>(g.out);
#pragma unroll
    for (int j = 0; j < NREP; ++j) {
      const int nl = wn * 16 * NREP + j * 16 + fq * 4;
      const int n = n0 + nl;
      f32x4 v = acc[i][j];
      if (g.rowgate && row_ok) {
        const float4 gt = *reinterpret_cast<const float4*>(g.rowgate + (long)b * g.ld_rowgate + n);
        v[0] *= gt.x; v[1] *= gt.y; v[2] *= gt.z; v[3] *= gt.w;
      }
      if (res_lds) {
        const uint2 rr = *reinterpret_cast<const uint2*>(smem + ml * CW + nl * 2);
        v[0] += T::to_f(rr.x & 0xffff); v[1] += T::to_f(rr.x >> 16); v[2] += T::to_f(rr.y & 0xffff); v[3] += T::to_f(rr.y >> 16);
      } else if (g.residual && row_ok) {
        const long rrow = g.residual_bcast ? (long)(m - b * g.rows_per_batch) : (long)m;
        const uint2 rr = *reinterpret_cast<const uint2*>(reinterpret_cast<const unsigned short*>(g.residual) + rrow * g.ldc + n);
        v[0] += T::to_f(rr.x & 0xffff); v[1] += T::to_f(rr.x >> 16); v[2] += T::to_f(rr.y & 0xffff); v[3] += T::to_f(rr.y >> 16);
      }
      if (g.act == 1) { v[0] = silu_f(v[0]); v[1] = silu_f(v[1]); v[2] = silu_f(v[2]); v[3] = silu_f(v[3]); }
      if (g.act == 3) { v[0] = gelu_tanh(v[0]); v[1] = gelu_tanh(v[1]); v[2] = gelu_tanh(v[2]); v[3] = gelu_tanh(v[3]); }
      if (g.act == 4) { v[0] = quick_gelu(v[0]); v[1] = quick_gelu(v[1]); v[2] = quick_gelu(v[2]); v[3] = quick_gelu(v[3]); }
      if (staged) {
        uint2 pk; pk.x = T::pack2(v[0], v[1]); pk.y = T::pack2(v[2], v[3]);
        *reinterpret_cast<uint2*>(smem + ml * CW + nl * 2) = pk;
      } else if (!row_ok) {
      } else if (g.out_kind == 0) {
        for (int e = 0; e < 4; ++e)
          if (n + e < g.n_valid) out16[(long)m * g.ldc + n + e] = (unsigned short)(T::pack2(v[e], 0.f) & 0xffff);
      } else if (g.out_kind == 1) {
        float* outf = reinterpret_cast<float*>(reinterpret_cast<char*>(g.out) + (long)blockIdx.y * g.split_stride);
        if (g.n_valid == g.N && (g.ldc & 3) == 0) {
          *reinterpret_cast<f32x4*>(outf + (long)m * g.ldc + n) = v;
        } else {
          for (int e = 0; e < 4; ++e)
            if (n + e < g.n_valid) outf[(long)m * g.ldc + n + e] = v[e];
        }
      } else {
        const int p = m - b * g.rows_per_batch;
        for (int e = 0; e < 4; ++e)
          if (n + e < g.n_valid)
            reinterpret_cast<float*>(g.out)[((long)b * g.n_valid + n + e) * g.rows_per_batch + p] = v[e];
      }
    }
  }
  }
  }
  if (pass == 0) SDN_STAMP(4)
  if ((staged || g.act == 2) && !g.x3_out) {
    __syncthreads();
    if (pass == 0) SDN_STAMP(5)
    const int cpr = out_cols / 8;
    const int col0 = g.act == 2 ? (n0 >> 1) : n0;
    unsigned short* out16 = reinterpret_cast<unsigned short*>(g.out);
    for (int e = tid; e < ROWS_PER_PASS * cpr; e += THREADS) {
      const int r = e / cpr, c = e - r * cpr;
      const int m = m0 + pass * ROWS_PER_PASS + r;
      if (m < g.M && !(g.dbg & 1))
        *reinterpret_cast<u32x4*>(out16 + (long)m * g.ldc + col0 + c * 8) = *reinterpret_cast<const u32x4*>(smem + r * CW + c * 16);
    }
    if (g.col_stats) {
      constexpr int CPR = BN / 8, RG = 8;
      static_assert(RG * CPR <= THREADS, "column-sum mapping needs RG * CPR threads");
      float* scr = reinterpret_cast<float*>(smem + NSTAGE * STAGE - RG * BN * 8);
      static_assert(NSTAGE * STAGE - RG * BN * 8 >= ROWS_PER_PASS * CW_PAD, "column-sum scratch must not overlap the staged slab");
      int rows_here = g.M - (m0 + pass * ROWS_PER_PASS);
      rows_here = rows_here > ROWS_PER_PASS ? ROWS_PER_PASS : rows_here;
      if (tid < RG * CPR) {
        const int rg = tid / CPR, c = tid - rg * CPR;
        float cs[8] = {0.f, 0.f, 0.f, 0.f, 0.f, 0.f, 0.f, 0.f}, cq[8] = {0.f, 0.f, 0.f, 0.f, 0.f, 0.f, 0.f, 0.f};
        for (int r = rg; r < rows_here; r += RG) {
          const u32x4 v = *reinterpret_cast<const u32x4*>(smem + r * CW + c * 16);
          const unsigned w4[4] = {v[0], v[1], v[2], v[3]};
#pragma unroll
          for (int k = 0; k < 4; ++k) {
            const float lo = T::to_f(w4[k] & 0xffff), hi = T::to_f(w4[k] >> 16);
            cs[2 * k] += lo; cq[2 * k] = fmaf(lo, lo, cq[2 * k]);
            cs[2 * k + 1] += hi; cq[2 * k + 1] = fmaf(hi, hi, cq[2 * k + 1]);
          }
        }
#pragma unroll
        for (int k = 0; k < 8; ++k) *reinterpret_cast<float2*>(scr + 2 * (rg * BN + c * 8 + k)) = make_float2(cs[k], cq[k]);
      }
      __syncthreads();
      if (tid < BN && rows_here > 0) {
        float ts = 0.f, tq = 0.f;
#pragma unroll
        for (int rg = 0; rg < RG; ++rg) { const float2 v = *reinterpret_cast<const float2*>(scr + 2 * (rg * BN + tid)); ts += v.x; tq += v.y; }
        const long blk = (long)(m0 / 128) + pass * (ROWS_PER_PASS / 128);
        *reinterpret_cast<float2*>(g.col_stats + 2 * (blk * g.N + n0 + tid)) = make_float2(ts, tq);
      }
    }
    if (pass == 0) SDN_STAMP(6)
  }
}
```

safe_denoiser_amd/csrc/sdn_ops.h:

```cpp
#pragma once
#include "../../include/sdn.h"

int sdn_gemm_pick_nrep(int n_padded, int act);
int sdn_gemm_pick_tile(int M, int N, int K, int act, int epilogue_reads = 0);

int sdn_temb_from_device(int dtype, const float* t_dev, int batch, int dim, void* out, void* stream);
int sdn_set_scalar(float* dst, float v, void* stream);

int sdn_gemm_pick_split(int M, int N, int K, int act, int out_kind);

int sdn_temb_f32(float timestep, const float* t_dev, int batch, int dim, void* out, void* stream);

int sdn_linear_pair_fold(int dtype, const void* wa, const void* wb, const float* ba, const float* bb, int C, int K, void* w_cat,
                         float* b_cat, void* stream);


int sdn_conv_slab_shape_ok(int M, int N, int Cin, int side, int stride, int upsample, int asym_pad, int out_kind, int n_valid);

enum { SDN_NL_KERNEL, SDN_NL_DTYPE, SDN_NL_NQ, SDN_NL_R, SDN_NL_NCH, SDN_NL_CT, SDN_NL_NTILES, SDN_NL_ROWS_PER_TILE, SDN_NL_RPC,
       SDN_NL_NCHUNK, SDN_NL_STATS_SRC, SDN_NL_TRIPLE, SDN_NL_COUNT };
struct sdn_norm_launch { int kernel, dtype, nq, r, nch, ct, ntiles, rows_per_tile, rpc, nchunk, stats_src, triple; };
void record_norm_launch(const sdn_norm_launch& l);
```

safe_denoiser_amd/csrc/sdn_plan.h:

```cpp
#pragma once
#include <stdio.h>
#include <string.h>

#include <map>
#include <set>
#include <string>
#include <tuple>
#include <vector>

#include "sdn_common.h"
#include "sdn_ops.h"

namespace sdn_plan {

enum ModelKind { UNET, MMDIT, VAE_DECODER, VAE_ENCODER, CLIP, CLIP_PROJ, T5, CLIP_VISION };

enum Space { SP_NONE = 0, SP_W = 1, SP_WS = 2, SP_IN = 3, SP_TEXT = 4, SP_OUT = 5, SP_POOLED = 6, SP_KV = 7, SP_OUT2 = 8 };
struct Ref { int space = SP_NONE; int64_t off = 0; };

struct Call {
  const void* weights; void* workspace; size_t workspace_bytes; int32_t batch; void* stream;
  const void *in = nullptr, *text = nullptr, *pooled = nullptr;
  void *out = nullptr, *out2 = nullptr;
  float scalar = 0.f; int n = 0;
  const int32_t* mask = nullptr;
  int64_t out_bs = 0, out_rs = 0, out2_rs = 0;
  int64_t kv_base = 0;
  Call(const void* w, void* ws, size_t ws_bytes, int32_t b, void* s) : weights(w), workspace(ws), workspace_bytes(ws_bytes), batch(b), stream(s) {}
  const char* operator()(const Ref& r) const {
    switch (r.space) {
      case SP_W: return (const char*)weights + r.off;
      case SP_WS: return (const char*)workspace + r.off;
      case SP_KV: return (const char*)workspace + kv_base + r.off;
      case SP_IN: return (const char*)in + r.off;
      case SP_TEXT: return (const char*)text + r.off;
      case SP_OUT: return (const char*)out + r.off;
      case SP_OUT2: return (const char*)out2 + r.off;
      case SP_POOLED: return (const char*)pooled + r.off;
      default: return nullptr;
    }
  }
};

enum OpKind { OP_TEMB, OP_CONV_IN, OP_GEMM, OP_GN, OP_LN, OP_ATTN, OP_PATCHIFY, OP_UNPATCHIFY, OP_LATENT_MIX, OP_SOFTMAX,
              OP_TRANSPOSE, OP_GAUSS, OP_REPEAT, OP_CLIP_EMBED, OP_MATTN, OP_ROWSTATS, OP_FFN, OP_SPLIT3,
              OP_RMSNORM, OP_EMBED, OP_T5_BIAS, OP_BATTN, OP_EOS_ROWS, OP_COPY_ROWS, OP_PATCH_ROWS, OP_VISION_EMBED, OP_CLASS_ROWS };

struct Op {
  int kind;
  sdn_gemm_desc gd;
  Ref a, a2, w, bias, rowbias, rowgate, residual, out, aux;
  Ref q2, k2, v2, out2;
  Ref col, cols1, cols2;
  Ref ln_c, ln_d, ln_stats;
  int ln = 0;
  int text_kv = 0;
  int x3t = 0;
  int pair_in = 0;
  int tri_out = 0;
  int dyn_ldc = 0;
  int n1 = 0, mod = 0, ld_mod = 0, patch = 0;
  int batch = 0, hw = 0, c1 = 0, c2 = 0, groups = 0, silu = 0;
  float eps = 0.f;
  int64_t rows = 0;
  int heads = 0, nq = 0, nk = 0, hd = 0, ldq = 0, ldk = 0, ldv = 0, ldo = 0;
  float scale = 0.f;
  Ref k, v;
  char label[24] = {0};
  double flops = 0.0;
  double bytes = 0.0;
};

struct Arena {
  std::map<int64_t, int64_t> free_;
  int64_t top = 0, peak = 0;
  static int64_t up(int64_t v) { return (v + 255) & ~(int64_t)255; }
  int64_t alloc(int64_t bytes) {
    bytes = up(bytes);
    for (auto it = free_.begin(); it != free_.end(); ++it) {
      if (it->second >= bytes) {
        const int64_t off = it->first, rest = it->second - bytes;
        free_.erase(it);
        if (rest > 0) free_[off + bytes] = rest;
        return off;
      }
    }
    if (!free_.empty()) {
      auto last = std::prev(free_.end());
      if (last->first + last->second == top) {
        const int64_t off = last->first;
        free_.erase(last);
        top = off + bytes;
        if (top > peak) peak = top;
        return off;
      }
    }
    const int64_t off = top;
    top += bytes;
    if (top > peak) peak = top;
    return off;
  }
  void release(int64_t off, int64_t bytes) {
    bytes = up(bytes);
    auto it = free_.emplace(off, bytes).first;
    auto nx = std::next(it);
    if (nx != free_.end() && it->first + it->second == nx->first) { it->second += nx->second; free_.erase(nx); }
    if (it != free_.begin()) {
      auto pv = std::prev(it);
      if (pv->first + pv->second == it->first) { pv->second += it->second; free_.erase(it); }
    }
  }
};

struct Act {
  int64_t off = -1, bytes = 0; int C = 0, hw = 0, side = 0;
  int64_t content = 0;
  int64_t st_off = -1, st_bytes = 0;
};

struct Plan {
  int batch = 0;
  int64_t tscalar_off = -1;
  std::vector<Op> ops;
  int64_t ws_bytes = 0;
  int64_t kv_base = 0;
  double flops = 0.0, attn_flops = 0.0;
};

}

struct sdn_unet {
  sdn_plan::ModelKind kind = sdn_plan::UNET;
  sdn_unet_config cfg;
  sdn_mmdit_config mcfg;
  sdn_vae_config vcfg;
  sdn_clip_config ccfg;
  sdn_clip_proj_config pcfg;
  sdn_t5_config tcfg;
  sdn_clip_vision_config vis;
  std::vector<sdn_param_info> params;
  std::map<std::string, int> param_index;
  int64_t weight_bytes = 0;
  std::map<int, sdn_plan::Plan> plans;
  int tproj_total = 0;
  int64_t subbatch_bytes = 0;
  bool profile_next = false;
  bool use_graph = false;
  bool gn_fuse = true;
  bool ln_fold = true;
  int ln_prepass_all = 0;
  bool ff_fuse = true;
  bool ffn_own_stats = true;
  bool ffn_fuse = true;
  struct FoldJob { int64_t w, gamma, beta, bias, wf, c, d; int rows, cols; int kind = 0; int group = 0; };
  std::vector<FoldJob> fold_jobs;
  uint64_t text_version = 0, kv_version = 0;
  int kv_batch = 0;
  const void *kv_w = nullptr, *kv_text = nullptr, *kv_ws = nullptr;
  bool x3_pairs = true;
  bool res_pre = true;
  bool x3_expand = true;
  bool split_k = false;
  struct GraphKey {
    int batch; const void *w, *lat, *text, *pooled, *out, *ws;
    bool operator<(const GraphKey& o) const {
      return std::tie(batch, w, lat, text, pooled, out, ws) < std::tie(o.batch, o.w, o.lat, o.text, o.pooled, o.out, o.ws);
    }
  };
  std::map<GraphKey, hipGraphExec_t> graphs;
  hipStream_t cap_stream = nullptr;
  ~sdn_unet() {
    for (auto& kv : graphs) (void)hipGraphExecDestroy(kv.second);
    for (auto e : ev) (void)hipEventDestroy(e);
    if (cap_stream) (void)hipStreamDestroy(cap_stream);
  }
  std::vector<hipEvent_t> ev;
  int profiled_batch = 0;
  int profiled_n = 0;
  int dtype() const {
    switch (kind) {
      case sdn_plan::MMDIT: return mcfg.dtype;
      case sdn_plan::VAE_DECODER: case sdn_plan::VAE_ENCODER: return vcfg.dtype;
      case sdn_plan::CLIP: return ccfg.dtype;
      case sdn_plan::CLIP_PROJ: return pcfg.dtype;
      case sdn_plan::T5: return tcfg.dtype;
      case sdn_plan::CLIP_VISION: return vis.dtype;
      default: return cfg.dtype;
    }
  }
  bool is_vae() const { return kind == sdn_plan::VAE_DECODER || kind == sdn_plan::VAE_ENCODER; }
  bool is_clip() const { return kind == sdn_plan::CLIP || kind == sdn_plan::CLIP_PROJ; }
};

namespace sdn_plan {

struct Builder {
  sdn_unet* u;
  Plan* plan;
  Arena arena;
  int B;
  int seq = 0;
  int es = 2;
  bool x3t = false;
  bool x3t_hold = false;
  std::set<int64_t> tri;
  Ref tproj;
  int tproj_cursor = 0;
  Ref gn_stats;
  Ref pending_cols;
  int64_t kv_top = 0;
  bool res_pre_next = false;
  bool triple_out_next = false;
  bool pair_out_next = false;
  bool plan_bad = false;
  bool force_x3t_next = false;
  std::set<int64_t> pairs;
  struct Res { std::string pfx; int cout; };

  Ref param(const std::string& name, int kind, int rows, int cols, int rows_padded = 0);
  Ref stacked(const std::vector<std::string>& names, int rows_each, int cols);
  Ref stacked_vec(const std::vector<std::string>& names, int n_each);
  Ref derived(const std::string& name, int64_t bytes);
  Act act(int64_t rows, int C, int hw = 0, int side = 0, int esz = 0);
  Act act_gn(int64_t rows, int C, int hw, int side);
  void want_stats(const Act& out) { pending_cols = out.st_off >= 0 ? Ref{SP_WS, out.st_off} : Ref(); }
  void drop(Act& t);
  static Ref R(const Act& t) { return Ref{SP_WS, t.off}; }
  Ref x3_weight(Ref w, int rows, int cols, int group);
  Act split3(Ref a, Ref a2, int64_t rows, int c1, int c2, int hw = 0, int side = 0);
  bool x3t_on(const Ref& a) const { return x3t && !x3t_hold && a.space == SP_WS; }
  void gemm(int64_t M, int N, int K, Ref a, Ref w, Ref bias, Ref out, int act_ = SDN_ACT_NONE, Ref residual = Ref(),
            int out_kind = SDN_OUT_BF16, int n_valid = 0, Ref a2 = Ref(), int K1 = 0, Ref rowbias = Ref(),
            int rows_per_batch = 0, int ld_rowbias = 0);
  void push_gemm(Op& o);
  void conv3x3(const Act& in, int cout, int n_pad, Ref w, Ref bias, Ref out, int stride, int upsample, Ref residual,
               Ref rowbias, int ld_rowbias, int out_kind = SDN_OUT_BF16, int n_valid = 0, int asym_pad = 0);
  void groupnorm(const Act& x, const Act* x2, float eps, int silu, Ref gamma, Ref beta, const Act& out);
  void layernorm(const Act& x, Ref gamma, Ref beta, const Act& out);
  void repeat(const Act& in, const Act& out, int rep);
  void attention(Ref q, Ref k, Ref v, Ref out, int nq, int nk, int C, int ldq, int ldk, int ldv, bool kv_pairs = false);

  void gemm_ln(const Act& x, int64_t rows, int N, int K, const std::string& wname, Ref w, Ref gamma, Ref beta, Ref bias,
               Ref out, int act_, bool prepass);
  Act resnet(const std::string& pfx, Act& x, Act* skip, int cout);
  Act transformer(const std::string& pfx, Act& x);
  void transformer_body(const std::string& pfx, Act& x, const Act& out, int64_t text_off, int rep = 1,
                        const Act* x_full = nullptr);
  std::vector<Res> enumerate_resnets() const;
  void build();

  void gemm_ex(int64_t M, int N, int K, Ref a, Ref w, Ref bias, Ref out, int act_, Ref residual, int out_kind,
               Ref rowbias, Ref rowgate, int rows_per_batch, int ld_row, int residual_bcast = 0);
  void ln_mod(const Act& x, int64_t rows, int rows_per_batch, Ref scale, Ref shift, int ld, const Act& out);
  Ref fcol(int col) const { return Ref{SP_WS, tproj.off + (int64_t)col * 4}; }
  void build_mmdit();

  Act vae_resnet(const std::string& pfx, Act& x, int cout);
  Act vae_attention(const std::string& pfx, Act& x);
  void build_vae();
  void build_vae_encoder();

  void build_clip();
  Ref glu_pair(const std::string& value_name, const std::string& gate_name, int F, int K);
  void t5_gemm(int64_t M, int N, int K, Ref a, Ref w, Ref out, int act_, bool into_stream);
  void t5_rmsnorm(Ref x, bool x_f32, int64_t rows, int C, Ref w, Ref out);
  void build_t5();

  void build_clip_vision();
};

Plan* get_plan(sdn_unet* u, int batch, int n = 0);
int run_plan(sdn_unet* u, const Call& c);
void drop_graphs(sdn_unet* u);

}
```

safe_denoiser_amd/csrc/sdn_plan_api.hip:

```cpp
#include "sdn_plan.h"

using namespace sdn_plan;

template <class F, class V> static void set_plan_toggle(sdn_unet* u, F sdn_unet::*field, V value) {
  u->*field = value;
  drop_graphs(u);
  u->plans.clear();
}

extern "C" {

int sdn_unet_create(const sdn_unet_config* cfg, sdn_unet** out) {
  if (!cfg || !out) return SDN_E_INVALID;
  if (cfg->n_levels < 1 || cfg->n_levels > 4 || cfg->layers_per_block < 1 || cfg->n_heads <= 0 ||
      cfg->in_channels <= 0 || cfg->in_channels > 16 || cfg->out_channels <= 0 || cfg->out_channels > 32 ||
      cfg->sample_size <= 0 || (cfg->sample_size % (1 << (cfg->n_levels - 1))) != 0 || cfg->cross_dim % 64 != 0 ||
      cfg->text_len <= 0 || cfg->norm_groups <= 0 || cfg->norm_groups > 64 || cfg->dtype < 0 || cfg->dtype > 3 ||
      cfg->latent_repeat < 0 || cfg->latent_repeat > 8)
    return SDN_E_INVALID;
  for (int i = 0; i < cfg->n_levels; ++i) {
    const int c = cfg->block_out_channels[i];
    if (c <= 0 || c % 64 != 0 || c % cfg->norm_groups != 0 || c % cfg->n_heads != 0) return SDN_E_INVALID;
    const int hd = c / cfg->n_heads;
    if (cfg->level_has_attn[i] && hd != 40 && hd != 64 && hd != 80 && hd != 160) return SDN_E_INVALID;
    if (sdn_gemm_pick_nrep(c, SDN_ACT_NONE) == 0 || sdn_gemm_pick_nrep(8 * c, SDN_ACT_GEGLU) == 0) return SDN_E_INVALID;
  }
  {
    const int hd_mid = cfg->block_out_channels[cfg->n_levels - 1] / cfg->n_heads;
    if (hd_mid != 40 && hd_mid != 64 && hd_mid != 80 && hd_mid != 160) return SDN_E_INVALID;
  }
  sdn_unet* u = new sdn_unet();
  u->cfg = *cfg;
  if (cfg->dtype >= 2) { u->gn_fuse = false; u->ln_fold = false; u->ff_fuse = false; }
  get_plan(u, cfg->latent_repeat > 1 ? cfg->latent_repeat : 1);
  *out = u;
  return SDN_OK;
}

int sdn_mmdit_create(const sdn_mmdit_config* cfg, sdn_unet** out) {
  if (!cfg || !out) return SDN_E_INVALID;
  const int C = cfg->num_heads * cfg->head_dim;
  if (cfg->in_channels <= 0 || cfg->out_channels <= 0 || cfg->sample_size <= 0 || cfg->patch_size <= 0 ||
      cfg->sample_size % cfg->patch_size != 0 || cfg->num_layers <= 0 || cfg->num_heads <= 0 || cfg->head_dim != 64 ||
      C % 128 != 0 || cfg->joint_dim % 64 != 0 || cfg->pooled_dim % 64 != 0 || cfg->time_dim % 64 != 0 ||
      (cfg->in_channels * cfg->patch_size * cfg->patch_size) % 64 != 0 ||
      (cfg->out_channels * cfg->patch_size * cfg->patch_size) % 32 != 0 || cfg->text_len <= 0 || cfg->dtype < 0 ||
      cfg->dtype > 3 || C > 2048)
    return SDN_E_INVALID;
  sdn_unet* u = new sdn_unet();
  memset(&u->cfg, 0, sizeof(u->cfg));
  u->mcfg = *cfg;
  u->kind = MMDIT;
  get_plan(u, 1);
  *out = u;
  return SDN_OK;
}

int sdn_vae_decoder_create(const sdn_vae_config* cfg, sdn_unet** out) {
  if (!cfg || !out) return SDN_E_INVALID;
  if (cfg->n_levels < 1 || cfg->n_levels > 4 || cfg->layers_per_block < 1 || cfg->latent_channels <= 0 ||
      cfg->latent_channels > 16 || cfg->out_channels <= 0 || cfg->out_channels > 32 || cfg->sample_size <= 0 ||
      cfg->norm_groups <= 0 || cfg->norm_groups > 64 || cfg->dtype < 0 || cfg->dtype > 1)
    return SDN_E_INVALID;
  for (int i = 0; i < cfg->n_levels; ++i) {
    const int c = cfg->block_out_channels[i];
    if (c <= 0 || c % 64 != 0 || c % cfg->norm_groups != 0 || sdn_gemm_pick_nrep(c, SDN_ACT_NONE) == 0) return SDN_E_INVALID;
  }
  const int hw = cfg->sample_size * cfg->sample_size;
  if (hw % 64 != 0 || hw > 16384 || (hw > 4096 && hw % 4096 != 0) || sdn_gemm_pick_nrep(hw, SDN_ACT_NONE) == 0) return SDN_E_INVALID;
  sdn_unet* u = new sdn_unet();
  memset(&u->cfg, 0, sizeof(u->cfg));
  u->cfg.norm_groups = cfg->norm_groups;
  u->vcfg = *cfg;
  u->kind = VAE_DECODER;
  get_plan(u, 1);
  *out = u;
  return SDN_OK;
}

int sdn_vae_encoder_create(const sdn_vae_config* cfg, sdn_unet** out) {
  if (!cfg || !out) return SDN_E_INVALID;
  sdn_unet* u = nullptr;
  const int rc = sdn_vae_decoder_create(cfg, &u);
  if (rc != SDN_OK) return rc;
  if (2 * cfg->latent_channels > 16) { delete u; return SDN_E_INVALID; }
  u->kind = VAE_ENCODER;
  u->plans.clear(); u->params.clear(); u->param_index.clear(); u->weight_bytes = 0;
  get_plan(u, 1);
  *out = u;
  return SDN_OK;
}

int sdn_clip_create(const sdn_clip_config* cfg, sdn_unet** out) {
  if (!cfg || !out) return SDN_E_INVALID;
  if (cfg->vocab_size <= 0 || cfg->hidden_size <= 0 || cfg->hidden_size % 128 != 0 || cfg->hidden_size > 1024 ||
      cfg->intermediate_size <= 0 || cfg->intermediate_size % 128 != 0 || cfg->num_layers <= 0 || cfg->num_heads <= 0 ||
      cfg->hidden_size != 64 * cfg->num_heads || cfg->max_position_embeddings <= 0 || cfg->max_position_embeddings > 4096 ||
      cfg->dtype < 0 || cfg->dtype > 3)
    return SDN_E_INVALID;
  sdn_unet* u = new sdn_unet();
  memset(&u->cfg, 0, sizeof(u->cfg));
  if (cfg->dtype >= 2) { u->gn_fuse = false; u->ln_fold = false; u->ff_fuse = false; }
  u->ccfg = *cfg;
  u->kind = CLIP;
  get_plan(u, 1);
  *out = u;
  return SDN_OK;
}

int sdn_clip_proj_create(const sdn_clip_proj_config* cfg, sdn_unet** out) {
  if (!cfg || !out) return SDN_E_INVALID;
  if (cfg->vocab_size <= 0 || cfg->hidden_size <= 0 || cfg->hidden_size % 128 != 0 || cfg->hidden_size > 1280 ||
      cfg->intermediate_size <= 0 || cfg->intermediate_size % 128 != 0 || cfg->num_layers <= 0 || cfg->num_heads <= 0 ||
      cfg->hidden_size != 64 * cfg->num_heads || cfg->max_position_embeddings <= 0 || cfg->max_position_embeddings > 4096 ||
      cfg->dtype < 0 || cfg->dtype > 3 || cfg->projection_dim <= 0 || cfg->projection_dim % 32 != 0 ||
      (cfg->act != SDN_ACT_QUICK_GELU && cfg->act != SDN_ACT_GELU) || cfg->eos_token_id < 0 || cfg->hidden_tap < 1 ||
      cfg->hidden_tap > cfg->num_layers)
    return SDN_E_INVALID;
  sdn_unet* u = new sdn_unet();
  memset(&u->cfg, 0, sizeof(u->cfg));
  if (cfg->dtype >= 2) { u->gn_fuse = false; u->ln_fold = false; u->ff_fuse = false; }
  u->pcfg = *cfg;
  u->ccfg.vocab_size = cfg->vocab_size; u->ccfg.hidden_size = cfg->hidden_size; u->ccfg.intermediate_size = cfg->intermediate_size;
  u->ccfg.num_layers = cfg->num_layers; u->ccfg.num_heads = cfg->num_heads; u->ccfg.max_position_embeddings = cfg->max_position_embeddings;
  u->ccfg.dtype = cfg->dtype;
  u->kind = CLIP_PROJ;
  get_plan(u, 1);
  *out = u;
  return SDN_OK;
}

int sdn_t5_create(const sdn_t5_config* cfg, sdn_unet** out) {
  if (!cfg || !out) return SDN_E_INVALID;
  if (cfg->vocab_size <= 0 || cfg->d_model <= 0 || cfg->d_model % 64 != 0 || cfg->d_kv != 64 || cfg->d_ff <= 0 || cfg->d_ff % 64 != 0 ||
      cfg->num_layers <= 0 || cfg->num_heads <= 0 || cfg->num_heads > 512 || cfg->num_buckets < 4 || cfg->num_buckets > 64 ||
      (cfg->num_buckets & 3) || cfg->max_distance <= cfg->num_buckets / 4 || !(cfg->eps > 0.f) || cfg->dtype < 0 || cfg->dtype > 1)
    return SDN_E_INVALID;
  sdn_unet* u = new sdn_unet();
  memset(&u->cfg, 0, sizeof(u->cfg));
  u->tcfg = *cfg;
  u->kind = T5;
  get_plan(u, 1);
  *out = u;
  return SDN_OK;
}

int sdn_unet_prepare(sdn_unet* u, void* weights, void* stream) {
  if (!u || !weights) return SDN_E_INVALID;
  char* W = (char*)weights;
  const int dt = u->dtype() == 1 ? 1 : 0;
  for (const auto& j : u->fold_jobs) {
    if (j.kind == 2) {
      const int rc2 = sdn_expand3_weights((const float*)(W + j.w), j.rows, j.cols, j.group, W + j.wf, stream);
      if (rc2 != SDN_OK) return rc2;
      continue;
    }
    if (j.kind == 1) {
      const int rc1 = sdn_linear_pair_fold(dt, W + j.w, W + j.gamma, (const float*)(W + j.beta), (const float*)(W + j.bias), j.rows, j.cols,
                                           W + j.wf, (float*)(W + j.c), stream);
      if (rc1 != SDN_OK) return rc1;
      continue;
    }
    const int rc = sdn_ln_fold(dt, W + j.w, (const float*)(W + j.gamma), (const float*)(W + j.beta),
                               j.bias >= 0 ? (const float*)(W + j.bias) : nullptr, j.rows, j.cols, W + j.wf, (float*)(W + j.c),
                               (float*)(W + j.d), stream);
    if (rc != SDN_OK) return rc;
  }
  return SDN_OK;
}

void sdn_unet_destroy(sdn_unet* u) { delete u; }

int sdn_unet_param_count(const sdn_unet* u) { return u ? (int)u->params.size() : 0; }

int sdn_unet_param_info(const sdn_unet* u, int32_t index, sdn_param_info* info) {
  if (!u || !info || index < 0 || index >= (int)u->params.size()) return SDN_E_INVALID;
  *info = u->params[index];
  return SDN_OK;
}

size_t sdn_unet_weight_bytes(const sdn_unet* u) { return u ? (size_t)u->weight_bytes : 0; }

static int vae_chunk(const sdn_unet* v) {
  const sdn_vae_config& c = v->vcfg;
  const int64_t side = (int64_t)c.sample_size << (c.n_levels - 1);
  int64_t cmax = 0;
  for (int i = 0; i < c.n_levels; ++i) if (c.block_out_channels[i] > cmax) cmax = c.block_out_channels[i];
  int64_t cap = (((int64_t)1 << 32) - 1) / (side * side * cmax * 2);
  if (cap > 8) cap = 8;
  return cap < 1 ? 0 : (int)cap;
}

size_t sdn_unet_workspace_bytes(sdn_unet* u, int32_t batch) {
  if (!u || batch <= 0) return 0;
  if (u->kind == T5) return sdn_t5_workspace_bytes(u, batch, 512);
  if (u->is_vae()) {
    const int cap = vae_chunk(u);
    if (cap == 0) return 0;
    if (batch > cap) batch = cap;
  }
  const int64_t b = get_plan(u, batch)->ws_bytes;
  return b < 0 ? 0 : (size_t)b;
}

double sdn_unet_flops(sdn_unet* u, int32_t batch, double* attn) {
  if (!u || batch <= 0) return 0.0;
  Plan* p = get_plan(u, batch);
  if (attn) *attn = p->attn_flops;
  return p->flops;
}

static int vae_run(sdn_unet* v, Call call, const float* in, int64_t in_n, float* out, int64_t out_n, int32_t batch) {
  if (batch < 0 || (batch > 0 && (!in || !out))) return SDN_E_INVALID;
  const int cap = vae_chunk(v);
  if (cap == 0) return SDN_E_INVALID;
  for (int lo = 0; lo < batch; lo += cap) {
    call.batch = batch - lo < cap ? batch - lo : cap;
    call.in = in + lo * in_n; call.out = out + lo * out_n;
    const int rc = run_plan(v, call);
    if (rc != SDN_OK) return rc;
  }
  return SDN_OK;
}

int sdn_vae_decode(sdn_unet* v, const void* weights, const float* latents, float latent_scale, float* image, int32_t batch,
                   void* workspace, size_t workspace_bytes, void* stream) {
  if (!v || v->kind != VAE_DECODER) return SDN_E_INVALID;
  const sdn_vae_config& c = v->vcfg;
  const int64_t side = (int64_t)c.sample_size << (c.n_levels - 1);
  Call call(weights, workspace, workspace_bytes, 0, stream);
  call.scalar = latent_scale;
  return vae_run(v, call, latents, (int64_t)c.latent_channels * c.sample_size * c.sample_size, image, (int64_t)c.out_channels * side * side, batch);
}

int sdn_vae_encode(sdn_unet* v, const void* weights, const float* image, float* moments, int32_t batch, void* workspace,
                   size_t workspace_bytes, void* stream) {
  if (!v || v->kind != VAE_ENCODER) return SDN_E_INVALID;
  const sdn_vae_config& c = v->vcfg;
  const int64_t side = (int64_t)c.sample_size << (c.n_levels - 1);
  return vae_run(v, Call(weights, workspace, workspace_bytes, 0, stream), image, (int64_t)c.out_channels * side * side, moments,
                 (int64_t)2 * c.latent_channels * c.sample_size * c.sample_size, batch);
}

int sdn_clip_forward(sdn_unet* m, const void* weights, const int32_t* input_ids, const int32_t* attention_mask,
                     void* last_hidden_state, int32_t batch, void* workspace, size_t workspace_bytes, void* stream) {
  if (!m || m->kind != CLIP || !input_ids || !last_hidden_state) return SDN_E_INVALID;
  Call call(weights, workspace, workspace_bytes, batch, stream);
  call.in = input_ids; call.mask = attention_mask; call.out = last_hidden_state;
  return run_plan(m, call);
}

int sdn_clip_proj_forward(sdn_unet* m, const void* weights, const int32_t* input_ids, void* hidden, int64_t hidden_batch_stride,
                          int64_t hidden_row_stride, void* text_embeds, int64_t embeds_row_stride, int32_t batch, void* workspace,
                          size_t workspace_bytes, void* stream) {
  if (!m || m->kind != CLIP_PROJ || !input_ids || !hidden || !text_embeds) return SDN_E_INVALID;
  const sdn_clip_proj_config& c = m->pcfg;
  if (hidden_row_stride < c.hidden_size || hidden_batch_stride < (int64_t)c.max_position_embeddings * hidden_row_stride ||
      embeds_row_stride < c.projection_dim || embeds_row_stride > 0x7fffffff || (hidden_row_stride & 7) || (hidden_batch_stride & 7) ||
      (embeds_row_stride & 7) || (reinterpret_cast<uintptr_t>(hidden) & 15) || (reinterpret_cast<uintptr_t>(text_embeds) & 15))
    return SDN_E_INVALID;
  Call call(weights, workspace, workspace_bytes, batch, stream);
  call.in = input_ids; call.out = hidden; call.out2 = text_embeds;
  call.out_bs = hidden_batch_stride; call.out_rs = hidden_row_stride; call.out2_rs = embeds_row_stride;
  return run_plan(m, call);
}

size_t sdn_t5_workspace_bytes(sdn_unet* m, int32_t batch, int32_t n) {
  if (!m || m->kind != T5 || batch <= 0 || batch > (1 << 20) || n < 2 || n > 512) return 0;
  const int64_t b = get_plan(m, batch, n)->ws_bytes;
  return b < 0 ? 0 : (size_t)b;
}

double sdn_t5_flops(sdn_unet* m, int32_t batch, int32_t n, double* attn) {
  if (!m || m->kind != T5 || batch <= 0 || batch > (1 << 20) || n < 2 || n > 512) return 0.0;
  Plan* p = get_plan(m, batch, n);
  if (attn) *attn = p->attn_flops;
  return p->flops;
}

int sdn_t5_forward(sdn_unet* m, const void* weights, const int32_t* input_ids, const int32_t* attention_mask, int32_t n,
                   void* out, int32_t batch, void* workspace, size_t workspace_bytes, void* stream) {
  if (!m || m->kind != T5 || n < 2 || n > 512 || batch > (1 << 20) || !input_ids || !out) return SDN_E_INVALID;
  Call call(weights, workspace, workspace_bytes, batch, stream);
  call.in = input_ids; call.mask = attention_mask; call.n = n; call.out = out;
  return run_plan(m, call);
}

int sdn_unet_forward(sdn_unet* u, const void* weights, const float* latents, float timestep, const void* text,
                     float* out, int32_t batch, void* workspace, size_t workspace_bytes, void* stream) {
  if (!u || u->kind != UNET || !latents || !text || !out) return SDN_E_INVALID;
  Call call(weights, workspace, workspace_bytes, batch, stream);
  call.in = latents; call.scalar = timestep; call.text = text; call.out = out;
  return run_plan(u, call);
}

int sdn_mmdit_forward(sdn_unet* u, const void* weights, const float* latents, float timestep, const void* text,
                      const void* pooled, float* out, int32_t batch, void* workspace, size_t workspace_bytes,
                      void* stream) {
  if (!u || u->kind != MMDIT || !latents || !text || !pooled || !out) return SDN_E_INVALID;
  Call call(weights, workspace, workspace_bytes, batch, stream);
  call.in = latents; call.scalar = timestep; call.text = text; call.pooled = pooled; call.out = out;
  return run_plan(u, call);
}

void sdn_unet_set_text_version(sdn_unet* u, uint64_t version) {
  if (!u) return;
  u->text_version = version;
  if (version == 0) u->kv_version = 0;
}

void sdn_unet_profile_next(sdn_unet* u) { if (u) u->profile_next = true; }

void sdn_unet_set_split_k(sdn_unet* u, int32_t on) {
  if (!u || u->kind == T5 || u->kind == CLIP_PROJ || u->kind == CLIP_VISION || u->split_k == (on != 0)) return;
  if (u->dtype() >= 2) return;
  set_plan_toggle(u, &sdn_unet::split_k, on != 0);
}

void sdn_unet_set_graph_mode(sdn_unet* u, int32_t on) {
  if (!u) return;
  u->use_graph = on != 0;
  if (!on) drop_graphs(u);
}


void sdn_debug_set_x3_expand(sdn_unet* u, int on) { if (u && u->x3_expand != (on != 0)) set_plan_toggle(u, &sdn_unet::x3_expand, on != 0); }

void sdn_debug_set_res_pre(sdn_unet* u, int on) { if (u && u->res_pre != (on != 0)) set_plan_toggle(u, &sdn_unet::res_pre, on != 0); }

void sdn_debug_set_ln_fold(sdn_unet* u, int on) { if (u) set_plan_toggle(u, &sdn_unet::ln_fold, on != 0); }

void sdn_debug_set_ln_prepass_all(sdn_unet* u, int on) { if (u) set_plan_toggle(u, &sdn_unet::ln_prepass_all, on); }

void sdn_debug_set_ffn_fuse(sdn_unet* u, int on) { if (u) set_plan_toggle(u, &sdn_unet::ffn_fuse, on != 0); }

void sdn_debug_set_ff_fuse(sdn_unet* u, int on) { if (u) set_plan_toggle(u, &sdn_unet::ff_fuse, on != 0); }

void sdn_debug_set_ffn_own_stats(sdn_unet* u, int on) { if (u) set_plan_toggle(u, &sdn_unet::ffn_own_stats, on != 0); }

void sdn_debug_set_x3_pairs(sdn_unet* u, int on) { if (u) set_plan_toggle(u, &sdn_unet::x3_pairs, on != 0); }

void sdn_debug_set_gn_fuse(sdn_unet* u, int on) { if (u) set_plan_toggle(u, &sdn_unet::gn_fuse, on != 0); }

void sdn_debug_set_subbatch_bytes(sdn_unet* u, long long bytes) {
  if (u && u->kind != MMDIT) set_plan_toggle(u, &sdn_unet::subbatch_bytes, (int64_t)bytes);
}

}
```

safe_denoiser_amd/csrc/sdn_plan_core.hip:

```cpp
#include <math.h>

#include "sdn_plan.h"

namespace sdn_plan {

Ref Builder::param(const std::string& name, int kind, int rows, int cols, int rows_padded) {
  auto it = u->param_index.find(name);
  if (it != u->param_index.end()) return Ref{SP_W, u->params[it->second].offset};
  sdn_param_info pi;
  memset(&pi, 0, sizeof(pi));
  snprintf(pi.name, sizeof(pi.name), "%s", name.c_str());
  pi.kind = kind; pi.rows = rows; pi.cols = cols; pi.rows_padded = rows_padded > rows ? rows_padded : rows;
  const int64_t esz = (kind == SDN_P_VEC_F32 || kind == SDN_P_GEGLU_VEC) ? 4 : es;
  const int64_t bytes = (int64_t)pi.rows_padded * (cols > 0 ? cols : 1) * esz;
  pi.offset = u->weight_bytes;
  u->weight_bytes += (bytes + 255) & ~(int64_t)255;
  u->param_index[name] = (int)u->params.size();
  u->params.push_back(pi);
  return Ref{SP_W, pi.offset};
}
Ref Builder::stacked(const std::vector<std::string>& names, int rows_each, int cols) {
  Ref first;
  int64_t expect = -1;
  for (size_t i = 0; i < names.size(); ++i) {
    Ref r = param(names[i], SDN_P_MAT, rows_each, cols);
    if (i == 0) first = r;
    else if (r.off != expect) { fprintf(stderr, "libsdn: stacked weight %s is not contiguous\n", names[i].c_str()); abort(); }
    expect = r.off + (int64_t)rows_each * cols * es;
  }
  return first;
}
Ref Builder::stacked_vec(const std::vector<std::string>& names, int n_each) {
  Ref first; int64_t expect = -1;
  for (size_t i = 0; i < names.size(); ++i) {
    Ref r = param(names[i], SDN_P_VEC_F32, n_each, 0);
    if (i == 0) first = r;
    else if (r.off != expect) { fprintf(stderr, "libsdn: stacked bias %s is not contiguous\n", names[i].c_str()); abort(); }
    expect = r.off + (int64_t)n_each * 4;
  }
  return first;
}
Ref Builder::derived(const std::string& name, int64_t bytes) {
  auto it = u->param_index.find(name);
  if (it != u->param_index.end()) return Ref{SP_W, u->params[it->second].offset};
  sdn_param_info pi; memset(&pi, 0, sizeof(pi));
  snprintf(pi.name, sizeof(pi.name), "%s", name.c_str());
  pi.kind = SDN_P_DERIVED; pi.rows = (int)bytes; pi.cols = 0; pi.rows_padded = (int)bytes;
  pi.offset = u->weight_bytes;
  u->weight_bytes += (bytes + 255) & ~(int64_t)255;
  u->param_index[name] = (int)u->params.size();
  u->params.push_back(pi);
  return Ref{SP_W, pi.offset};
}

Act Builder::act(int64_t rows, int C, int hw, int side, int esz) {
  const bool dflt = esz == 0;
  if (esz == 0) esz = es;
  Act t; t.content = rows * C * esz;
  t.bytes = (x3t && dflt) ? rows * C * 6 : t.content;
  t.off = arena.alloc(t.bytes); t.C = C; t.hw = hw; t.side = side; return t;
}
Act Builder::act_gn(int64_t rows, int C, int hw, int side) {
  Act t = act(rows, C, hw, side);
  if (u->gn_fuse && !u->split_k && hw > 0 && hw % 128 == 0) {
    t.st_bytes = ((rows + 127) / 128) * (int64_t)C * 8;
    t.st_off = arena.alloc(t.st_bytes);
  }
  return t;
}
void Builder::drop(Act& t) {
  if (t.off >= 0) { arena.release(t.off, t.bytes); tri.erase(t.off); pairs.erase(t.off); }
  if (t.st_off >= 0) arena.release(t.st_off, t.st_bytes);
  t.off = -1; t.st_off = -1;
}

Ref Builder::x3_weight(Ref w, int rows, int cols, int group) {
  const std::string name = "x3@" + std::to_string((long long)w.off);
  const bool fresh = u->param_index.find(name) == u->param_index.end();
  Ref d = derived(name, (int64_t)rows * 3 * cols * 2);
  if (fresh) { sdn_unet::FoldJob j{w.off, -1, -1, -1, d.off, -1, -1, rows, cols}; j.kind = 2; j.group = group; u->fold_jobs.push_back(j); }
  return d;
}
Act Builder::split3(Ref a, Ref a2, int64_t rows, int c1, int c2, int hw, int side) {
  Act t = act(rows, c1 + c2, hw, side);
  Op o; o.kind = OP_SPLIT3; o.a = a; o.a2 = a2; o.rows = rows; o.c1 = c1; o.c2 = c2; o.out = R(t);
  o.bytes = 10.0 * (double)rows * (c1 + c2);
  snprintf(o.label, sizeof(o.label), "k_split3");
  plan->ops.push_back(o);
  tri.insert(t.off);
  return t;
}

void Builder::gemm(int64_t M, int N, int K, Ref a, Ref w, Ref bias, Ref out, int act_, Ref residual,
                   int out_kind, int n_valid, Ref a2, int K1, Ref rowbias,
                   int rows_per_batch, int ld_rowbias) {
  const bool forced = force_x3t_next && x3t && !x3t_hold;
  force_x3t_next = false;
  if ((x3t_on(a) || forced) && (act_ == SDN_ACT_NONE || act_ == SDN_ACT_GEGLU) && out_kind != SDN_OUT_F32_NCHW && n_valid == 0) {
    Act tmp; Ref au = a;
    if (a.space != SP_WS || !tri.count(a.off)) { tmp = split3(a, a2, M, a2.space != SP_NONE ? K1 : K, a2.space != SP_NONE ? K - K1 : 0); au = R(tmp); }
    Op o; o.kind = OP_GEMM; memset(&o.gd, 0, sizeof(o.gd));
    o.x3t = 1;
    o.gd.M = (int)M; o.gd.N = N; o.gd.K = 3 * K; o.gd.a_mode = SDN_A_PLAIN; o.gd.act = act_; o.gd.out_kind = SDN_OUT_F32;
    const bool tri_o = triple_out_next && act_ == SDN_ACT_NONE;
    const bool pair_o = pair_out_next && act_ == SDN_ACT_NONE && !tri_o && residual.space == SP_NONE;
    triple_out_next = false; pair_out_next = false;
    o.gd.x3_out = act_ == SDN_ACT_GEGLU ? 2 : (tri_o ? 3 : (pair_o ? 4 : 1)); o.gd.rows_per_batch = rows_per_batch; o.gd.ld_rowbias = ld_rowbias;
    if (pair_o && out.space == SP_WS) pairs.insert(out.off);
    o.a = au; o.w = x3_weight(w, N, K, K); o.bias = bias; o.rowbias = rowbias; o.residual = residual; o.out = out;
    o.flops = 2.0 * (double)M * (double)N * (double)K;
    o.bytes = 6.0 * ((double)M * K + (double)N * K) + 4.0 * (double)M * (act_ == SDN_ACT_GEGLU ? 0.75 * N : N) +
              (residual.space != SP_NONE ? 4.0 * (double)M * N : 0.0);
    snprintf(o.label, sizeof(o.label), "k_gemm<%d>x3", sdn_gemm_pick_tile((int)M, N, 3 * K, act_));
    push_gemm(o);
    if ((act_ == SDN_ACT_GEGLU || tri_o) && out.space == SP_WS) tri.insert(out.off);
    if (tmp.off >= 0) drop(tmp);
    return;
  }
  triple_out_next = false; pair_out_next = false;
  const bool rp = res_pre_next && residual.space != SP_NONE && act_ == SDN_ACT_NONE && out_kind == SDN_OUT_BF16 && n_valid == 0 && es == 2;
  res_pre_next = false;
  Op o; o.kind = OP_GEMM; memset(&o.gd, 0, sizeof(o.gd));
  o.gd.res_pre = rp ? 1 : 0;
  o.gd.M = (int)M; o.gd.N = N; o.gd.K = K; o.gd.a_mode = SDN_A_PLAIN; o.gd.K1 = K1; o.gd.act = act_;
  o.gd.out_kind = out_kind; o.gd.n_valid = n_valid; o.gd.rows_per_batch = rows_per_batch; o.gd.ld_rowbias = ld_rowbias;
  o.a = a; o.a2 = a2; o.w = w; o.bias = bias; o.rowbias = rowbias; o.residual = residual; o.out = out;
  o.flops = 2.0 * (double)M * (double)(n_valid > 0 ? n_valid : N) * (double)K;
  o.bytes = 2.0 * ((double)M * K + (double)N * K + (double)M * (act_ == SDN_ACT_GEGLU ? N / 2 : N)) +
            (residual.space != SP_NONE ? 2.0 * (double)M * N : 0.0);
  snprintf(o.label, sizeof(o.label), "k_gemm<%d>%s", sdn_gemm_pick_tile((int)M, N, K, act_, residual.space != SP_NONE && !rp), rp ? "/rp" : "");
  push_gemm(o);
}
void Builder::push_gemm(Op& o) {
  o.col = pending_cols; pending_cols = Ref();
  const int nv = o.gd.n_valid > 0 ? o.gd.n_valid : o.gd.N;
  const int split = (!u->split_k || nv != o.gd.N) ? 1 : sdn_gemm_pick_split(o.gd.M, o.gd.N, o.gd.K, o.gd.act, o.gd.out_kind);
  if (split > 1) {
    const int64_t bytes = (int64_t)split * o.gd.M * o.gd.N * 4;
    const int64_t off = arena.alloc(bytes);
    o.gd.split_k = split; o.aux = Ref{SP_WS, off}; o.rows = bytes;
    arena.release(off, bytes);
    const size_t L = strlen(o.label);
    if (L + 3 < sizeof(o.label)) snprintf(o.label + L, sizeof(o.label) - L, "/s%d", split);
  }
  plan->ops.push_back(o);
  plan->flops += o.flops;
}
void Builder::conv3x3(const Act& in, int cout, int n_pad, Ref w, Ref bias, Ref out, int stride, int upsample, Ref residual,
                      Ref rowbias, int ld_rowbias, int out_kind, int n_valid, int asym_pad) {
  const int Hi = upsample ? in.side * 2 : in.side;
  const int Ho = (Hi + (asym_pad ? 1 : 2) - 3) / stride + 1;
  if (x3t_on(R(in))) {
    Act tmp; Ref au = R(in);
    if (!tri.count(in.off)) { tmp = split3(R(in), Ref(), (int64_t)B * in.side * in.side, in.C, 0, in.hw, in.side); au = R(tmp); }
    Op o; o.kind = OP_GEMM; memset(&o.gd, 0, sizeof(o.gd));
    o.x3t = 1;
    o.gd.M = B * Ho * Ho; o.gd.N = n_pad; o.gd.K = 27 * in.C; o.gd.a_mode = SDN_A_CONV3X3;
    o.gd.Hs = in.side; o.gd.Ws = in.side; o.gd.Cin = 3 * in.C; o.gd.Ho = Ho; o.gd.Wo = Ho; o.gd.stride = stride;
    o.gd.upsample = upsample; o.gd.asym_pad = asym_pad; o.gd.n_valid = n_valid; o.gd.rows_per_batch = Ho * Ho; o.gd.ld_rowbias = ld_rowbias;
    if (out_kind == SDN_OUT_F32_NCHW) { o.gd.out_kind = out_kind; o.gd.x3_out = 0; }
    else { o.gd.out_kind = SDN_OUT_F32; o.gd.x3_out = 1; }
    o.a = au; o.w = x3_weight(w, n_pad, 9 * in.C, in.C); o.bias = bias; o.rowbias = rowbias; o.residual = residual; o.out = out;
    o.flops = 2.0 * (double)o.gd.M * (double)cout * 9.0 * in.C;
    o.bytes = 6.0 * ((double)B * in.side * in.side * in.C + (double)n_pad * 9 * in.C) + 4.0 * (double)o.gd.M * cout +
              (residual.space != SP_NONE ? 4.0 * (double)o.gd.M * cout : 0.0);
    if (Ho == in.side && sdn_conv_slab_shape_ok(o.gd.M, n_pad, 3 * in.C, in.side, stride, upsample, asym_pad, SDN_OUT_BF16, n_valid) &&
        sdn_gemm_pick_tile(o.gd.M, n_pad, o.gd.K, SDN_ACT_NONE) == 10)
      snprintf(o.label, sizeof(o.label), "k_conv_slab<%d>/x3", in.side);
    else
      snprintf(o.label, sizeof(o.label), "k_gemm<%d>x3", sdn_gemm_pick_tile(o.gd.M, n_pad, o.gd.K, SDN_ACT_NONE));
    push_gemm(o);
    if (tmp.off >= 0) drop(tmp);
    return;
  }
  Op o; o.kind = OP_GEMM; memset(&o.gd, 0, sizeof(o.gd));
  o.gd.res_pre = (res_pre_next && residual.space != SP_NONE && out_kind == SDN_OUT_BF16 && n_valid == 0 && es == 2) ? 1 : 0;
  res_pre_next = false;
  o.gd.M = B * Ho * Ho; o.gd.N = n_pad; o.gd.K = 9 * in.C; o.gd.a_mode = SDN_A_CONV3X3;
  o.gd.Hs = in.side; o.gd.Ws = in.side; o.gd.Cin = in.C; o.gd.Ho = Ho; o.gd.Wo = Ho; o.gd.stride = stride;
  o.gd.upsample = upsample; o.gd.asym_pad = asym_pad; o.gd.out_kind = out_kind; o.gd.n_valid = n_valid; o.gd.rows_per_batch = Ho * Ho;
  o.gd.ld_rowbias = ld_rowbias;
  o.a = R(in); o.w = w; o.bias = bias; o.rowbias = rowbias; o.residual = residual; o.out = out;
  o.flops = 2.0 * (double)o.gd.M * (double)cout * (double)o.gd.K;
  o.bytes = 2.0 * ((double)B * in.side * in.side * in.C + (double)n_pad * o.gd.K + (double)o.gd.M * cout) +
            (residual.space != SP_NONE ? 2.0 * (double)o.gd.M * cout : 0.0);
  if (Ho == in.side && sdn_conv_slab_shape_ok(o.gd.M, n_pad, in.C, in.side, stride, upsample, asym_pad, out_kind, n_valid) &&
      sdn_gemm_pick_tile(o.gd.M, n_pad, o.gd.K, SDN_ACT_NONE) == 10)
    snprintf(o.label, sizeof(o.label), "k_conv_slab<%d>", in.side);
  else
    snprintf(o.label, sizeof(o.label), "k_gemm<%d>", sdn_gemm_pick_tile(o.gd.M, n_pad, o.gd.K, SDN_ACT_NONE));
  push_gemm(o);
}
void Builder::groupnorm(const Act& x, const Act* x2, float eps, int silu, Ref gamma, Ref beta, const Act& out) {
  Op o; o.kind = OP_GN; o.a = R(x); if (x2) o.a2 = R(*x2);
  o.batch = B; o.hw = x.hw; o.c1 = x.C; o.c2 = x2 ? x2->C : 0; o.groups = u->cfg.norm_groups; o.eps = eps;
  o.silu = silu; o.w = gamma; o.bias = beta; o.out = R(out); o.aux = gn_stats;
  if (x3t) { o.tri_out = 1; tri.insert(out.off); }
  if (x.st_off >= 0 && (!x2 || x2->st_off >= 0)) {
    o.cols1 = Ref{SP_WS, x.st_off};
    if (x2) o.cols2 = Ref{SP_WS, x2->st_off};
  }
  o.bytes = 2.0 * (o.cols1.space != SP_NONE ? 2.0 : 3.0) * (double)B * x.hw * (o.c1 + o.c2);
  snprintf(o.label, sizeof(o.label), o.cols1.space != SP_NONE ? "k_gn_apply" : "k_gn_stats+apply");
  plan->ops.push_back(o);
}
void Builder::layernorm(const Act& x, Ref gamma, Ref beta, const Act& out) {
  Op o; o.kind = OP_LN; o.a = R(x); o.rows = (int64_t)B * x.hw; o.c1 = x.C; o.eps = 1e-5f; o.w = gamma; o.bias = beta;
  o.out = R(out);
  if (x3t) { o.tri_out = 1; tri.insert(out.off); }
  o.bytes = 2.0 * 2.0 * (double)o.rows * x.C;
  snprintf(o.label, sizeof(o.label), "k_layernorm");
  plan->ops.push_back(o);
}
void Builder::repeat(const Act& in, const Act& out, int rep) {
  Op o; o.kind = OP_REPEAT; o.a = R(in); o.out = R(out); o.rows = in.content; o.c1 = rep;
  o.bytes = (double)in.content * (1 + rep);
  snprintf(o.label, sizeof(o.label), "k_repeat");
  plan->ops.push_back(o);
}
void Builder::attention(Ref q, Ref k, Ref v, Ref out, int nq, int nk, int C, int ldq, int ldk, int ldv, bool kv_pairs) {
  Op o; o.kind = OP_ATTN; o.a = q; o.k = k; o.v = v; o.out = out; o.batch = B; o.heads = u->cfg.n_heads;
  o.nq = nq; o.nk = nk; o.hd = C / u->cfg.n_heads; o.ldq = ldq; o.ldk = ldk; o.ldv = ldv; o.ldo = C;
  o.scale = 1.0f / sqrtf((float)o.hd);
  if (x3t && out.space == SP_WS) { o.tri_out = 1; tri.insert(out.off); }
  if (q.space == SP_WS && pairs.count(q.off)) {
    o.pair_in = kv_pairs ? 2 : 1; pairs.erase(q.off);
  } else if (kv_pairs) {
    plan_bad = true;
  }
  const double f = 4.0 * (double)B * o.heads * (double)nq * (double)nk * (double)o.hd;
  o.flops = f;
  o.bytes = 2.0 * (double)B * C * (2.0 * nq + 2.0 * nk);
  snprintf(o.label, sizeof(o.label), "k_attn<%d>", o.hd);
  plan->ops.push_back(o);
  plan->flops += f; plan->attn_flops += f;
}

Plan* get_plan(sdn_unet* u, int batch, int n) {
  if (u->kind == T5 && n == 0) n = 512;
  const int key = u->kind == T5 ? batch * 1024 + n : batch;
  auto it = u->plans.find(key);
  if (it != u->plans.end()) return &it->second;
  if (u->kind == T5 && u->plans.size() >= 64) {
    u->plans.clear();
    u->profiled_batch = 0;
  }
  Plan& p = u->plans[key];
  p.batch = batch;
  Builder b{u, &p};
  b.B = batch;
  b.seq = n;
  b.es = u->dtype() >= 2 ? 4 : 2;
  b.x3t = u->kind == UNET && u->dtype() == 3 && u->x3_expand;
  switch (u->kind) {
    case UNET: b.build(); break;
    case MMDIT: b.build_mmdit(); break;
    case VAE_DECODER: b.build_vae(); break;
    case VAE_ENCODER: b.build_vae_encoder(); break;
    case CLIP: case CLIP_PROJ: b.build_clip(); break;
    case T5: b.build_t5(); break;
    case CLIP_VISION: b.build_clip_vision(); break;
  }
  return &p;
}

}
```

safe_denoiser_amd/csrc/sdn_plan_unet.hip:

```cpp
#include <math.h>

#include "sdn_plan.h"

namespace sdn_plan {

void Builder::gemm_ln(const Act& x, int64_t rows, int N, int K, const std::string& wname, Ref w, Ref gamma, Ref beta, Ref bias,
                      Ref out, int act_, bool prepass) {
  const bool fresh = u->param_index.find(wname + "#ln") == u->param_index.end();
  Ref wf = derived(wname + "#ln", (int64_t)N * K * 2), c = derived(wname + "#ln_c", (int64_t)N * 4), d = derived(wname + "#ln_d", (int64_t)N * 4);
  if (fresh) u->fold_jobs.push_back({w.off, gamma.off, beta.off, bias.space == SP_NONE ? -1 : bias.off, wf.off, c.off, d.off, N, K});
  Act st;
  if (prepass) {
    st = act(rows, 2, 0, 0, 4);
    Op o; o.kind = OP_ROWSTATS; o.a = R(x); o.rows = rows; o.c1 = K; o.eps = 1e-5f; o.out = R(st);
    o.bytes = 2.0 * rows * K; snprintf(o.label, sizeof(o.label), "k_row_stats"); plan->ops.push_back(o);
  }
  Op o; o.kind = OP_GEMM; memset(&o.gd, 0, sizeof(o.gd));
  o.gd.M = (int)rows; o.gd.N = N; o.gd.K = K; o.gd.a_mode = SDN_A_PLAIN; o.gd.act = act_; o.gd.out_kind = SDN_OUT_BF16;
  o.a = R(x); o.w = wf; o.out = out; o.ln = 1; o.ln_c = c; o.ln_d = d; o.eps = 1e-5f;
  if (prepass) o.ln_stats = R(st);
  o.flops = 2.0 * (double)rows * N * K;
  o.bytes = 2.0 * ((double)rows * K + (double)N * K + (double)rows * (act_ == SDN_ACT_GEGLU ? N / 2 : N));
  { int t = sdn_gemm_pick_tile((int)rows, N, K, act_);
    if (t == 8 && N % 320 == 0) t = 10;
// ... 208 lines not shown
      v.push_back({buf, c.block_out_channels[i]});
    }
  const int top = c.block_out_channels[c.n_levels - 1];
  v.push_back({"mid_block.resnets.0", top});
  v.push_back({"mid_block.resnets.1", top});
  for (int i = 0; i < c.n_levels; ++i)
    for (int j = 0; j <= c.layers_per_block; ++j) {
      snprintf(buf, sizeof(buf), "up_blocks.%d.resnets.%d", i, j);
      v.push_back({buf, c.block_out_channels[c.n_levels - 1 - i]});
    }
  return v;
}

void Builder::build() {
  const sdn_unet_config& c = u->cfg;
  const int S = c.sample_size, ch0 = c.block_out_channels[0], tdim = 4 * ch0;
  char buf[96];

  Ref l1w = param("time_embedding.linear_1.weight", SDN_P_MAT, tdim, ch0), l1b = param("time_embedding.linear_1.bias", SDN_P_VEC_F32, tdim, 0);
  Ref l2w = param("time_embedding.linear_2.weight", SDN_P_MAT, tdim, tdim), l2b = param("time_embedding.linear_2.bias", SDN_P_VEC_F32, tdim, 0);
  const std::vector<Res> rs = enumerate_resnets();
  int total = 0;
  Ref tpw, tpb;
  {
    int64_t expect = -1;
    for (size_t i = 0; i < rs.size(); ++i) {
      Ref r = param(rs[i].pfx + ".time_emb_proj.weight", SDN_P_MAT, rs[i].cout, tdim);
      if (i == 0) tpw = r; else if (r.off != expect) { fprintf(stderr, "libsdn: time_emb_proj not contiguous\n"); abort(); }
      expect = r.off + (int64_t)rs[i].cout * tdim * es;
      total += rs[i].cout;
    }
    expect = -1;
    for (size_t i = 0; i < rs.size(); ++i) {
      Ref r = param(rs[i].pfx + ".time_emb_proj.bias", SDN_P_VEC_F32, rs[i].cout, 0);
      if (i == 0) tpb = r; else if (r.off != expect) { fprintf(stderr, "libsdn: time_emb_proj bias not contiguous\n"); abort(); }
      expect = r.off + (int64_t)rs[i].cout * 4;
    }
  }
  u->tproj_total = total;
  gn_stats = Ref{SP_WS, arena.alloc((int64_t)B * 129 * 64 * 2 * 4)};
  plan->tscalar_off = arena.alloc(256);
  Act tsin = act(B, ch0);
  { Op o; o.kind = OP_TEMB; o.batch = B; o.c1 = ch0; o.out = R(tsin); snprintf(o.label, sizeof(o.label), "k_temb"); plan->ops.push_back(o); }
  x3t_hold = true;
  Act t1 = act(B, tdim);
  gemm(B, tdim, ch0, R(tsin), l1w, l1b, R(t1), SDN_ACT_SILU);
  drop(tsin);
  Act semb = act(B, tdim);
  gemm(B, tdim, tdim, R(t1), l2w, l2b, R(semb), SDN_ACT_SILU);
  drop(t1);
  Act tp = act(B, total, 0, 0, 4);
  tproj = R(tp);
  gemm(B, total, tdim, R(semb), tpw, tpb, R(tp), SDN_ACT_NONE, Ref(), SDN_OUT_F32);
  drop(semb);
  x3t_hold = false;

  Ref ciw = param("conv_in.weight", SDN_P_CONV3X3, ch0, 9 * c.in_channels), cib = param("conv_in.bias", SDN_P_VEC_F32, ch0, 0);
  const int rep = (c.latent_repeat > 1 && c.level_has_attn[0] && u->subbatch_bytes == 0) ? c.latent_repeat : 1;
  if (B % rep != 0) { plan->ws_bytes = -1; return; }
  const int Bfull = B, Bp = B / rep;
  Act hp = act((int64_t)Bp * S * S, ch0, S * S, S);
  { Op o; o.kind = OP_CONV_IN; o.batch = Bp; o.c1 = c.in_channels; o.c2 = ch0; o.hw = S; o.a = Ref{SP_IN, 0}; o.w = ciw; o.bias = cib; o.out = R(hp);
    o.flops = 2.0 * Bp * S * S * (double)ch0 * 9 * c.in_channels; o.bytes = (double)Bp * S * S * (4.0 * c.in_channels + 2.0 * ch0);
    snprintf(o.label, sizeof(o.label), "k_conv_in"); plan->ops.push_back(o);
    plan->flops += o.flops; }
  Act h = hp;
  if (rep > 1) { h = act((int64_t)B * S * S, ch0, S * S, S); repeat(hp, h, rep); }

  std::vector<Act> skips;
  skips.push_back(h);
  Act cur = h;
  bool cur_is_skip = true;

  for (int i = 0; i < c.n_levels; ++i) {
    const int cout = c.block_out_channels[i];
    for (int j = 0; j < c.layers_per_block; ++j) {
      snprintf(buf, sizeof(buf), "down_blocks.%d.resnets.%d", i, j);
      if (rep > 1 && i == 0 && j == 0) {
        B = Bp;
        Act rp = resnet(buf, hp, nullptr, cout);
        B = Bfull;
        drop(hp);
        Act rf = act((int64_t)B * rp.hw, cout, rp.hw, rp.side);
        repeat(rp, rf, rep);
        snprintf(buf, sizeof(buf), "down_blocks.%d.attentions.%d", i, j);
        Act t = act_gn((int64_t)B * rp.hw, cout, rp.hw, rp.side);
        transformer_body(buf, rp, t, 0, rep, &rf);
        drop(rp); drop(rf);
        cur = t; skips.push_back(cur); cur_is_skip = true;
        continue;
      }
      Act r = resnet(buf, cur, nullptr, cout);
      if (!cur_is_skip) drop(cur);
      cur = r; cur_is_skip = false;
      if (c.level_has_attn[i]) {
        snprintf(buf, sizeof(buf), "down_blocks.%d.attentions.%d", i, j);
        Act t = transformer(buf, cur);
        drop(cur);
        cur = t;
      }
      skips.push_back(cur); cur_is_skip = true;
    }
    if (i + 1 < c.n_levels) {
      snprintf(buf, sizeof(buf), "down_blocks.%d.downsamplers.0.conv", i);
      Ref w = param(std::string(buf) + ".weight", SDN_P_CONV3X3, cout, 9 * cout), bb = param(std::string(buf) + ".bias", SDN_P_VEC_F32, cout, 0);
      const int s2 = cur.side / 2;
      Act d = act_gn((int64_t)B * s2 * s2, cout, s2 * s2, s2);
      want_stats(d);
      conv3x3(cur, cout, cout, w, bb, R(d), 2, 0, Ref(), Ref(), 0);
      cur = d; skips.push_back(cur); cur_is_skip = true;
    }
  }
  {
    Act r = resnet("mid_block.resnets.0", cur, nullptr, cur.C);
    cur = r; cur_is_skip = false;
    Act t = transformer("mid_block.attentions.0", cur);
    drop(cur); cur = t;
    Act r2 = resnet("mid_block.resnets.1", cur, nullptr, cur.C);
    drop(cur); cur = r2;
  }
  for (int i = 0; i < c.n_levels; ++i) {
    const int lvl = c.n_levels - 1 - i, cout = c.block_out_channels[lvl];
    for (int j = 0; j <= c.layers_per_block; ++j) {
      Act skip = skips.back(); skips.pop_back();
      snprintf(buf, sizeof(buf), "up_blocks.%d.resnets.%d", i, j);
      Act r = resnet(buf, cur, &skip, cout);
      drop(cur); drop(skip);
      cur = r;
      if (c.level_has_attn[lvl]) {
        snprintf(buf, sizeof(buf), "up_blocks.%d.attentions.%d", i, j);
        Act t = transformer(buf, cur);
        drop(cur); cur = t;
      }
    }
    if (i + 1 < c.n_levels) {
      snprintf(buf, sizeof(buf), "up_blocks.%d.upsamplers.0.conv", i);
      Ref w = param(std::string(buf) + ".weight", SDN_P_CONV3X3, cout, 9 * cout), bb = param(std::string(buf) + ".bias", SDN_P_VEC_F32, cout, 0);
      const int s2 = cur.side * 2;
      Act up = act_gn((int64_t)B * s2 * s2, cout, s2 * s2, s2);
      want_stats(up);
      conv3x3(cur, cout, cout, w, bb, R(up), 1, 1, Ref(), Ref(), 0);
      drop(cur); cur = up;
    }
  }
  Ref og = param("conv_norm_out.weight", SDN_P_VEC_F32, ch0, 0), ob = param("conv_norm_out.bias", SDN_P_VEC_F32, ch0, 0);
  const int npad = 32;
  Ref cow = param("conv_out.weight", SDN_P_CONV3X3, c.out_channels, 9 * ch0, npad);
  Ref cob = param("conv_out.bias", SDN_P_VEC_F32, c.out_channels, 0, npad);
  Act g = act((int64_t)B * S * S, ch0, S * S, S);
  groupnorm(cur, nullptr, 1e-5f, 1, og, ob, g);
  drop(cur);
  conv3x3(g, c.out_channels, npad, cow, cob, Ref{SP_OUT, 0}, 1, 0, Ref(), Ref(), 0, SDN_OUT_F32_NCHW, c.out_channels);
  drop(g);
  plan->kv_base = Arena::up(arena.peak);
  plan->ws_bytes = plan_bad ? -1 : plan->kv_base + kv_top;
}

}
```

safe_denoiser_amd/unet.py:

```python
from __future__ import annotations

import ctypes as C
import math
from types import SimpleNamespace

import torch

from . import _lib
from ._model import ALL_DTYPES, P_CONV3X3, P_DERIVED, P_GEGLU_MAT, P_GEGLU_VEC, P_MAT, P_VEC_F32, EngineModel

SD14_CONFIG = dict(in_channels=4, out_channels=4, sample_size=64, block_out_channels=(320, 640, 1280, 1280),
                   down_block_types=("CrossAttnDownBlock2D", "CrossAttnDownBlock2D", "CrossAttnDownBlock2D",
                                     "DownBlock2D"),
                   layers_per_block=2, attention_head_dim=8, cross_attention_dim=768, norm_num_groups=32)

class UNetOutput:
    __slots__ = ("sample",)

    def __init__(self, sample):
        self.sample = sample


def _interleave16(t: torch.Tensor) -> torch.Tensor:
    f = t.shape[0] // 2
    v, g = t[:f], t[f:]
    rest = t.shape[1:]
    return torch.stack([v.reshape(f // 16, 16, *rest), g.reshape(f // 16, 16, *rest)], dim=1).reshape(2 * f, *rest)


class UNet2DConditionModel(EngineModel):
    def __init__(self, text_len: int = 77, dtype=torch.bfloat16, latent_repeat: int = 1, precision: str | None = None, **config):
        code = self._storage(dtype, precision, ALL_DTYPES,
                             "storage dtype must be torch.bfloat16, torch.float16 or torch.float32 (the precision mode)")
        self.latent_repeat = max(1, int(latent_repeat))
        cfg = dict(SD14_CONFIG)
        cfg.update(config)
        self.config = SimpleNamespace(**cfg)
        self.in_channels = cfg["in_channels"]
        self.text_len = text_len
        boc = list(cfg["block_out_channels"])
        n = len(boc)
        c = _lib.UnetConfig(in_channels=cfg["in_channels"], out_channels=cfg["out_channels"],
                            sample_size=cfg["sample_size"], n_levels=n,
                            block_out_channels=(C.c_int32 * 4)(*(boc + [0] * (4 - n))),
                            level_has_attn=(C.c_int32 * 4)(*([1 if "CrossAttn" in t else 0
                                                              for t in cfg["down_block_types"]] + [0] * (4 - n))),
                            layers_per_block=cfg["layers_per_block"], n_heads=cfg["attention_head_dim"],
                            cross_dim=cfg["cross_attention_dim"], text_len=text_len,
                            norm_groups=cfg["norm_num_groups"],
                            dtype=code, latent_repeat=self.latent_repeat)
        self.tail_split = False
        self._create("sdn_unet_create", c)

    def _source_shape(self, p: dict) -> tuple:
        if p["name"].endswith(("proj_in.weight", "proj_out.weight", "conv_shortcut.weight")):
            return (p["rows"], p["cols"], 1, 1)
        return super()._source_shape(p)

    @staticmethod
    def _is_norm_param(name: str) -> bool:
        return ".norm" in name or name.startswith("conv_norm_out")

    def _pack_one(self, p: dict, t: torch.Tensor) -> torch.Tensor:
        t = super()._pack_one(p, t)
        return _interleave16(t) if p["kind"] in (P_GEGLU_MAT, P_GEGLU_VEC) else t

    def sibling(self, latent_repeat: int | None = None):
        net = UNet2DConditionModel(text_len=self.text_len, dtype=self.dtype, precision=self.precision,
                                   latent_repeat=self.latent_repeat if latent_repeat is None else latent_repeat, **vars(self.config))
        net._weights = self._weights
        return net

    def set_graph_mode(self, on: bool = True):
        _lib.lib().sdn_unet_set_graph_mode(self._h, 1 if on else 0)
        return self

    def set_text_version(self, version: int = 0):
        _lib.lib().sdn_unet_set_text_version(self._h, int(version))
        self._text_version = int(version)
        return self

    def set_split_k(self, on: bool = True):
        _lib.lib().sdn_unet_set_split_k(self._h, 1 if on else 0)
        self._ws = {}
        return self

    def prepare_text(self, encoder_hidden_states: torch.Tensor) -> torch.Tensor:
        e = encoder_hidden_states
        if e.shape[1] != self.text_len or e.shape[2] != self.config.cross_attention_dim:
            raise _lib.SdnError(f"encoder_hidden_states must be [B,{self.text_len},{self.config.cross_attention_dim}]")
        return e.to(self.dtype).contiguous()

    TAIL_MAX_SAMPLES = 12

    def set_tail_split(self, on: bool = True):
        self.tail_split = bool(on)
        return self

    def _tail_split_of(self, b: int):
        rep = self.latent_repeat
        if not self.tail_split or rep <= 1:
            return None
        p = b // rep
        q = 64 // math.gcd(64, rep)
        pm = p // q * q
        r = p - pm
        if pm == 0 or r == 0 or r * rep > self.TAIL_MAX_SAMPLES:
            return None
        return pm, r

    def max_samples(self) -> int:
        c = self.config
        boc = list(c.block_out_channels)
        n = len(boc)
        worst = max((c.sample_size >> i) ** 2 * (boc[min(i + 1, n - 1)] + boc[i]) * 2 for i in range(n))
        cap = ((1 << 31) - 1) // worst
        if self.precision in ("fp32", "bf16x3"):
            cap = min(cap, 3 * (cap // 4))
        return cap

    def _chunks_of(self, b: int):
        rep = self.latent_repeat
        p = b // rep
        cap = self.max_samples() // rep
        if p <= cap:
            ts = self._tail_split_of(b)
            return None if ts is None else [(0, ts[0], False), (ts[0], ts[1], True)]
        q = 64 // math.gcd(64, rep)
        per = cap // q * q if cap >= q else cap
        chunks = [(lo, min(per, p - lo), False) for lo in range(0, p, per)]
        lo, n, _ = chunks[-1]
        if n * rep <= self.TAIL_MAX_SAMPLES and self.tail_split and rep > 1:
            chunks[-1] = (lo, n, True)
        return chunks

    def _forward_chunks(self, sample, timestep, text, out, chunks):
        rep, dev = self.latent_repeat, sample.device
        p = sample.shape[0]
        st = getattr(self, "_split", None)
        if st is None or st["key"] != (p, tuple(chunks), dev):
            tshape, oshape = tuple(text.shape[1:]), tuple(out.shape[1:])
            parts = [dict(lo=lo, n=n, side=side, net=self if i == 0 else self.sibling(),
                          text=None if rep == 1 else torch.empty((rep * n,) + tshape, dtype=self.dtype, device=dev),
                          out=None if rep == 1 else torch.empty((rep * n,) + oshape, dtype=torch.float32, device=dev))
                     for i, (lo, n, side) in enumerate(chunks)]
            st = self._split = dict(key=(p, tuple(chunks), dev), parts=parts, text_key=None,
                                    side=torch.cuda.Stream(device=dev) if any(c[2] for c in chunks) else None)
        ver = int(getattr(self, "_text_version", 0))
        tkey = (ver, text.data_ptr())
        if rep > 1 and (ver == 0 or st["text_key"] != tkey):
            tv = text.view(rep, p, *text.shape[1:])
            for c in st["parts"]:
                c["text"].view(rep, c["n"], *text.shape[1:]).copy_(tv[:, c["lo"]:c["lo"] + c["n"]])
            st["text_key"] = tkey
        cur = torch.cuda.current_stream(dev)
        if st["side"] is not None:
            st["side"].wait_stream(cur)

        def run(c):
            net, lo, n = c["net"], c["lo"], c["n"]
            if net is not self:
                net._weights = self._weights
                net.set_text_version(ver)
            if rep == 1:
                net._forward_one(sample[lo:lo + n], timestep, text[lo:lo + n], out[lo:lo + n])
            else:
                net._forward_one(sample[lo:lo + n], timestep, c["text"], c["out"])

        for c in st["parts"]:
            if c["side"]:
                with torch.cuda.stream(st["side"]):
                    run(c)
        for c in st["parts"]:
            if not c["side"]:
                run(c)
        if st["side"] is not None:
            cur.wait_stream(st["side"])
        if rep > 1:
            ov = out.view(rep, p, -1)
            for c in st["parts"]:
                ov[:, c["lo"]:c["lo"] + c["n"]].copy_(c["out"].view(rep, c["n"], -1))
        return out

    def forward_into(self, sample, timestep, text_bf16, out):
        b = text_bf16.shape[0]
        if sample.shape[0] * self.latent_repeat != b or out.shape[0] != b:
            raise _lib.SdnError(f"batch mismatch: {sample.shape[0]} latents x latent_repeat {self.latent_repeat} vs {b} text rows")
        chunks = self._chunks_of(b)
        if chunks is not None:
            _lib.dptr(sample, torch.float32), _lib.dptr(text_bf16, self.dtype), _lib.dptr(out, torch.float32)
            return self._forward_chunks(sample, timestep, text_bf16, out, chunks)
        return self._forward_one(sample, timestep, text_bf16, out)

    def _forward_one(self, sample, timestep, text_bf16, out):
        b = text_bf16.shape[0]
        if b > self.max_samples():
            raise _lib.SdnError(f"{b} samples exceed what one launch plan addresses ({self.max_samples()}): forward_into cuts such batches")
        ws = self._workspace(b, sample.device)
        _lib.check(_lib.lib().sdn_unet_forward(self._h, _lib.dptr(self._weights), _lib.dptr(sample, torch.float32),
                                               float(timestep), _lib.dptr(text_bf16, self.dtype),
                                               _lib.dptr(out, torch.float32), b, _lib.dptr(ws), ws.numel(),
                                               _lib.stream_ptr()), "sdn_unet_forward")
        return out

    def __call__(self, sample, timestep, encoder_hidden_states=None, return_dict=True, **unused):
        _lib.require_gpu()
        if self._weights is None:
            raise _lib.SdnError("no weights loaded: call load_state_dict() first")
        x = sample.float().contiguous()
        s = self.config.sample_size
        if tuple(x.shape[1:]) != (self.config.in_channels, s, s):
            raise _lib.SdnError(f"sample must be [B,{self.config.in_channels},{s},{s}], got {tuple(x.shape)}")
        e = self.prepare_text(encoder_hidden_states)
        if e.shape[0] != x.shape[0] * self.latent_repeat:
            raise _lib.SdnError("batch mismatch between sample and encoder_hidden_states")
        out = torch.empty((e.shape[0], self.config.out_channels, s, s), dtype=torch.float32, device=x.device)
        self.forward_into(x, float(timestep), e, out)
        return UNetOutput(out) if return_dict else (out,)
```

Baseline: 8.634 images/sec.

## Fold nearest-upsample into 3x3 conv as four 2x2 sub-pixel convolutions

Upsample-then-3x3 conv layers in the UNet are replaced by a phase-decomposed form. Each of the four output parities becomes a 2x2 conv on the low-resolution input, using weights pre-summed from the 3x3 kernel at prepare time. This cuts the GEMM K dimension from 9*Cin to 4*Cin and avoids reading an upsampled activation. The cost is a new GEMM variant with scattered output-row addressing, four times the weight memory for these layers, and no split-k or slab path for them.

```diff
diff --git a/include/sdn.h b/include/sdn.h
--- a/include/sdn.h
+++ b/include/sdn.h
@@ -309,6 +309,8 @@
 int sdn_gemm_splitk_f16(const sdn_gemm_desc* d, const void* a, const void* a2, const void* w, const float* bias,
                         const float* rowbias, const float* rowgate, const void* residual, void* out, void* partials,
                         size_t partial_bytes, void* stream);
+
+int sdn_conv_up4_weights(int32_t dtype, const void* w9, int32_t N, int32_t Cin, void* out, void* stream);
 
 int sdn_repeat(const void* in, size_t bytes, int32_t rep, void* out, void* stream);
 
@@ -439,6 +441,7 @@
 
 void sdn_unet_set_graph_mode(sdn_unet* u, int32_t on);
 void sdn_unet_set_split_k(sdn_unet* u, int32_t on);
+void sdn_unet_set_conv_up4(sdn_unet* u, int32_t on);
 
 typedef struct sdn_profile_row {
   char    kernel[24];
diff --git a/safe_denoiser_amd/_lib.py b/safe_denoiser_amd/_lib.py
--- a/safe_denoiser_amd/_lib.py
+++ b/safe_denoiser_amd/_lib.py
@@ -220,6 +220,8 @@
     "sdn_unet_set_graph_mode": (None, [_vp, _i32]),
     "sdn_unet_set_text_version": (None, [_vp, C.c_uint64]),
     "sdn_unet_set_split_k": (None, [_vp, _i32]),
+    "sdn_unet_set_conv_up4": (None, [_vp, _i32]),
+    "sdn_conv_up4_weights": (C.c_int, [_i32, _vp, _i32, _i32, _vp, _vp]),
     "sdn_unet_profile_next": (None, [_vp]),
     "sdn_unet_profile_read": (C.c_int, [_vp, C.POINTER(ProfileRow), _i32]),
 }
diff --git a/safe_denoiser_amd/csrc/sdn_gemm.hip b/safe_denoiser_amd/csrc/sdn_gemm.hip
--- a/safe_denoiser_amd/csrc/sdn_gemm.hip
+++ b/safe_denoiser_amd/csrc/sdn_gemm.hip
@@ -19,7 +19,7 @@
     g.stamps[(long)blockIdx.x * 8 + (IDX)] = t_;                                                         \
   }
 
-template <typename T, int NREP, int WGM, int NSTAGE, int LNF, bool H8>
+template <typename T, int NREP, int WGM, int NSTAGE, int LNF, bool H8, bool UP4 = false>
 __device__ __forceinline__ void gemm_dma_body(const GemmArgs& g) {
 #if defined(__HIP_DEVICE_COMPILE__)
   SDN_STAMP(0)
@@ -61,7 +61,25 @@
   unsigned a_base[A_PIECES];
   unsigned a_aux[A_PIECES];
   const int ld1 = g.a_mode == 1 ? g.Cin : g.K1, ld2 = g.K - g.K1;
-  if (g.a_mode == 1) {
+  [[maybe_unused]] int up_d0 = 0, up_m0 = 0, up_out0 = 0;
+  if constexpr (UP4) {
+    const int hw = g.Hs * g.Ws;
+    const int sp = m0 / hw;
+    const int py = (sp >> 1) & 1, px = sp & 1;
+    up_d0 = (((py - 1) * g.Ws + (px - 1)) * g.Cin) * 2;
+    up_m0 = sp * hw;
+    up_out0 = (sp >> 2) * 4 * hw + py * 2 * g.Ws + px;
+    const int q = m0 - up_m0 + wid * A_PIECES * 8 + lrow;
+    int y = q / g.Ws, x = q - y * g.Ws;
+#pragma unroll
+    for (int i = 0; i < A_PIECES; ++i) {
+      if (i > 0) { x += 8; if (x >= g.Ws) { x -= g.Ws; ++y; } }
+      const unsigned rb = ((y + py >= 1) ? 1u : 0u) | ((y + py < g.Hs) ? 2u : 0u);
+      const unsigned cb = ((x + px >= 1) ? 1u : 0u) | ((x + px < g.Ws) ? 2u : 0u);
+      a_aux[i] = 0u;
+      a_base[i] = (unsigned)(((((sp >> 2) * g.Hs + y) * g.Ws + x) * g.Cin + lchunk * 8) * 2) | ((rb & 1u) ? cb : 0u) | ((rb & 2u) ? cb << 2 : 0u);
+    }
+  } else if (g.a_mode == 1) {
     const int hw = g.Ho * g.Wo;
     const int Hi = g.upsample ? g.Hs * 2 : g.Hs, Wi = g.upsample ? g.Ws * 2 : g.Ws;
     const int mb = m0 + wid * A_PIECES * 8 + lrow;
@@ -109,8 +127,9 @@
     const int piece = wid * W_PIECES + i;
     w_ok[i] = piece * 8 < BN;
     w_off[i] = (unsigned)(((long)(n0 + piece * 8 + lrow) * g.K + lchunk * 8) * 2);
-  }
-  const __amdgpu_buffer_rsrc_t rs_w = make_rsrc(g.w, (unsigned)((long)g.N * g.K * 2));
+    if constexpr (UP4) w_off[i] += (unsigned)((long)((m0 / (g.Hs * g.Ws)) & 3) * g.N * g.K * 2);
+  }
+  const __amdgpu_buffer_rsrc_t rs_w = make_rsrc(g.w, (unsigned)((long)g.N * g.K * 2 * (UP4 ? 4 : 1)));
   const long a_rows = g.a_mode == 1 ? (long)(g.M / (g.Ho * g.Wo)) * g.Hs * g.Ws : (long)g.M;
   const __amdgpu_buffer_rsrc_t rs_a1 = make_rsrc(g.a, (unsigned)(a_rows * ld1 * 2));
   const __amdgpu_buffer_rsrc_t rs_a2 = make_rsrc(g.a2 ? g.a2 : g.a, (unsigned)(g.a2 ? a_rows * ld2 * 2 : 0));
@@ -120,7 +139,16 @@
   auto issue_aw = [&](int buf, bool with_w) {
     unsigned char* sa = smem + buf * STAGE;
     unsigned char* sw = sa + BM * 128;
-    if (g.a_mode == 1) {
+    if constexpr (UP4) {
+      const int tap = (cur_k0 >> 6) & 3, c0 = (cur_k0 >> 8) << 6;
+      const int delta = up_d0 + (((tap >> 1) * g.Ws + (tap & 1)) * g.Cin + c0) * 2;
+#pragma unroll
+      for (int i = 0; i < A_PIECES; ++i) {
+        const unsigned off = ((a_base[i] >> tap) & 1u) ? (a_base[i] & ~15u) + (unsigned)delta : OOB;
+        __builtin_amdgcn_raw_ptr_buffer_load_lds(rs_a1, (lds_ptr_t)(sa + (wid * A_PIECES + i) * 1024), 16, off, 0, 0, 0);
+      }
+      w_k0 = tap * g.Cin + c0;
+    } else if (g.a_mode == 1) {
       const int dy = cur_ty - 1, dx = cur_tx - 1, tap = cur_ty * 3 + cur_tx;
       if (!g.upsample) {
         const int delta = ((dy * g.Ws + dx) * g.Cin + cur_c0) * 2;
@@ -409,6 +437,16 @@
   constexpr int WM_PER_PASS = WGM / PASSES, ROWS_PER_PASS = 64 * WM_PER_PASS;
   static_assert(WGM % PASSES == 0, "pass split must divide the wave rows");
   static_assert(PASSES <= 2, "epilogue is written for at most two staging passes");
+  [[maybe_unused]] auto epi_out_row = [&](int m) -> int {
+    if constexpr (UP4) {
+      const int q = m - up_m0;
+      const int y = q / g.Ws, x = q - y * g.Ws;
+      return up_out0 + 4 * g.Ws * y + 2 * x;
+    } else {
+      return m;
+    }
+  };
+#define SDN_EPI_OUT_ROW(m) epi_out_row(m)
 #define SDN_PASS 0
 #include "sdn_gemm_epilogue.inc"
 #undef SDN_PASS
@@ -417,6 +455,7 @@
 #include "sdn_gemm_epilogue.inc"
 #undef SDN_PASS
   }
+#undef SDN_EPI_OUT_ROW
   SDN_STAMP(3)
 #endif
 }
@@ -428,6 +467,10 @@
 template <typename T, int NREP>
 __global__ void __launch_bounds__(512, 2)
 k_gemm_h8(const GemmArgs g) { gemm_dma_body<T, NREP, 4, 2, 0, true>(g); }
+
+template <typename T, int NREP>
+__global__ void __launch_bounds__(512, 2)
+k_gemm_up4(const GemmArgs g) { gemm_dma_body<T, NREP, 4, 2, 0, false, true>(g); }
 
 
 template <typename T>
@@ -528,6 +571,16 @@
   }
 }
 
+template <typename T>
+int dispatch_up4(int nrep, const GemmArgs& g, hipStream_t st) {
+  const int grid = g.tiles_m * g.tiles_n;
+  record_gemm_launch(5, T::kDtype, nrep, 4, 2, 0, g.tiles_m, g.tiles_n, 1, 0);
+  if (nrep == 10) hipLaunchKernelGGL((k_gemm_up4<T, 10>), dim3(grid), dim3(512), 0, st, g);
+  else if (nrep == 8) hipLaunchKernelGGL((k_gemm_up4<T, 8>), dim3(grid), dim3(512), 0, st, g);
+  else return SDN_E_INVALID;
+  return sdn_launch_status();
+}
+
 inline bool al16(const void* p) { return (reinterpret_cast<uintptr_t>(p) & 15) == 0; }
 
 }
@@ -617,6 +670,14 @@
   const bool res_pre = d->res_pre && residual && !x3 && !rowgate && !d->residual_bcast && d->split_k <= 1 && !partials && !ln_c &&
                        d->out_kind == SDN_OUT_BF16 && n_valid == d->N && d->act == SDN_ACT_NONE;
   int nrep = sdn_gemm_pick_tile(d->M, d->N, d->K, d->act, ((residual && !x3 && !res_pre) || rowgate) ? 1 : 0);
+  const bool up4 = d->a_mode == SDN_A_CONV3X3 && d->upsample == 2;
+  if (up4) {
+    if (x3 || rowbias || rowgate || residual || d->act != SDN_ACT_NONE || n_valid != d->N || d->out_kind != SDN_OUT_BF16 || d->split_k > 1 ||
+        partials || ln_c || ln_d || d->stride != 1 || d->asym_pad || d->K != 4 * d->Cin || d->Hs <= 0 || d->Ws <= 0)
+      return SDN_E_INVALID;
+    nrep = sdn_conv_up4_tile(d->Hs, d->Ws, d->Cin, d->N);
+    if (nrep == 0 || (long)4 * d->N * d->K * 2 >= (1L << 31)) return SDN_E_INVALID;
+  }
   if ((ln_c || ln_d) && nrep == 8 && d->N % 320 == 0) nrep = 10;
   if (h8) {
     if (d->N % 256 == 0) nrep = 8;
@@ -635,7 +696,7 @@
     g.K1 = (d->K1 > 0 && d->K1 < d->K) ? d->K1 : d->K;
     if (g.K1 != d->K && (!a2 || (g.K1 % BK) != 0)) return SDN_E_INVALID;
   } else if (d->a_mode == SDN_A_CONV3X3) {
-    if (d->Cin <= 0 || (d->Cin % BK) != 0 || d->K != 9 * d->Cin || d->Hs <= 0 || d->Ws <= 0 || d->Ho <= 0 ||
+    if (d->Cin <= 0 || (d->Cin % BK) != 0 || d->K != (up4 ? 4 : 9) * d->Cin || d->upsample < 0 || d->upsample > 2 || d->Hs <= 0 || d->Ws <= 0 || d->Ho <= 0 ||
         d->Wo <= 0 || (d->stride != 1 && d->stride != 2) || d->M % (d->Ho * d->Wo) != 0)
       return SDN_E_INVALID;
     const int Hi = d->upsample ? 2 * d->Hs : d->Hs, Wi = d->upsample ? 2 * d->Ws : d->Ws;
@@ -722,6 +783,10 @@
                          (const unsigned short*)residual, d->residual_bcast, g.ldc, d->act, (unsigned short*)out);
     return sdn_launch_status();
   }
+  if (up4) {
+    ++g_gemm_launches[1];
+    return dtype == 0 ? dispatch_up4<SdnBF16>(nrep, g, st) : dispatch_up4<SdnF16>(nrep, g, st);
+  }
   if (nrep == 10 && g_gemm_variant != 13) {
     const int rc = dispatch_conv_slab(dtype, g, st);
     if (rc != SDN_GEMM_NOT_SLAB) { ++g_gemm_launches[0]; return rc; }
@@ -803,6 +868,50 @@
   return sdn_launch_status();
 }
 
+int sdn_conv_up4_tile(int Hs, int Ws, int Cin, int N) {
+  if (Hs <= 0 || Ws < 8 || Cin <= 0 || N <= 0 || ((long)Hs * Ws) % 256 != 0 || Cin % BK != 0) return 0;
+  return N % 320 == 0 ? 10 : (N % 256 == 0 ? 8 : 0);
+}
+
+namespace {
+template <typename T>
+__global__ void __launch_bounds__(256)
+k_conv_up4_weights(const unsigned short* __restrict__ w9, int N, int Cin, unsigned short* __restrict__ out) {
+  const long per = (long)N * 4 * Cin;
+  const long e = (long)blockIdx.x * 256 + threadIdx.x;
+  if (e >= 4 * per) return;
+  const int p = (int)(e / per);
+  const long r = e - p * per;
+  const int n = (int)(r / (4 * Cin)), k = (int)(r - (long)n * 4 * Cin);
+  const int tap = k / Cin, c = k - tap * Cin;
+  const int py = p >> 1, px = p & 1, a = tap >> 1, b = tap & 1;
+  const int ty0 = a == 0 ? 0 : (py ? 2 : 1), ty1 = a == 0 ? (py ? 1 : 0) : 2;
+  const int tx0 = b == 0 ? 0 : (px ? 2 : 1), tx1 = b == 0 ? (px ? 1 : 0) : 2;
+  float acc = 0.f;
+  bool first = true;
+  for (int ty = ty0; ty <= ty1; ++ty)
+    for (int tx = tx0; tx <= tx1; ++tx) {
+      const float v = T::to_f(w9[(long)n * 9 * Cin + (3 * ty + tx) * Cin + c]);
+      acc = first ? v : acc + v;
+      first = false;
+    }
+  out[e] = (unsigned short)(T::pack2(acc, 0.f) & 0xffffu);
+}
+}
+
+extern "C" int sdn_conv_up4_weights(int32_t dtype, const void* w9, int32_t N, int32_t Cin, void* out, void* stream) {
+  if (!w9 || !out || N <= 0 || Cin <= 0 || dtype < 0 || dtype > 1) return SDN_E_INVALID;
+  const long total = (long)16 * N * Cin;
+  const unsigned grid = (unsigned)((total + 255) / 256);
+  if (dtype == 1)
+    hipLaunchKernelGGL((k_conv_up4_weights<SdnF16>), dim3(grid), dim3(256), 0, (hipStream_t)stream, (const unsigned short*)w9, N, Cin,
+                       (unsigned short*)out);
+  else
+    hipLaunchKernelGGL((k_conv_up4_weights<SdnBF16>), dim3(grid), dim3(256), 0, (hipStream_t)stream, (const unsigned short*)w9, N, Cin,
+                       (unsigned short*)out);
+  return sdn_launch_status();
+}
+
 namespace {
 template <typename T>
 __global__ void __launch_bounds__(256)
diff --git a/safe_denoiser_amd/csrc/sdn_gemm_epilogue.inc b/safe_denoiser_amd/csrc/sdn_gemm_epilogue.inc
--- a/safe_denoiser_amd/csrc/sdn_gemm_epilogue.inc
+++ b/safe_denoiser_amd/csrc/sdn_gemm_epilogue.inc
@@ -290,8 +290,13 @@
     for (int e = tid; e < ROWS_PER_PASS * cpr; e += THREADS) {
       const int r = e / cpr, c = e - r * cpr;
       const int m = m0 + pass * ROWS_PER_PASS + r;
+#ifdef SDN_EPI_OUT_ROW
+      if (m < g.M && !(g.dbg & 1))
+        *reinterpret_cast<u32x4*>(out16 + (long)SDN_EPI_OUT_ROW(m) * g.ldc + col0 + c * 8) = *reinterpret_cast<const u32x4*>(smem + r * CW + c * 16);
+#else
       if (m < g.M && !(g.dbg & 1))
         *reinterpret_cast<u32x4*>(out16 + (long)m * g.ldc + col0 + c * 8) = *reinterpret_cast<const u32x4*>(smem + r * CW + c * 16);
+#endif
     }
     if (g.col_stats) {
       constexpr int CPR = BN / 8, RG = 8;
diff --git a/safe_denoiser_amd/csrc/sdn_ops.h b/safe_denoiser_amd/csrc/sdn_ops.h
--- a/safe_denoiser_amd/csrc/sdn_ops.h
+++ b/safe_denoiser_amd/csrc/sdn_ops.h
@@ -17,6 +17,8 @@
 
 int sdn_conv_slab_shape_ok(int M, int N, int Cin, int side, int stride, int upsample, int asym_pad, int out_kind, int n_valid);
 
+int sdn_conv_up4_tile(int Hs, int Ws, int Cin, int N);
+
 enum { SDN_NL_KERNEL, SDN_NL_DTYPE, SDN_NL_NQ, SDN_NL_R, SDN_NL_NCH, SDN_NL_CT, SDN_NL_NTILES, SDN_NL_ROWS_PER_TILE, SDN_NL_RPC,
        SDN_NL_NCHUNK, SDN_NL_STATS_SRC, SDN_NL_TRIPLE, SDN_NL_COUNT };
 struct sdn_norm_launch { int kernel, dtype, nq, r, nch, ct, ntiles, rows_per_tile, rpc, nchunk, stats_src, triple; };
diff --git a/safe_denoiser_amd/csrc/sdn_plan.h b/safe_denoiser_amd/csrc/sdn_plan.h
--- a/safe_denoiser_amd/csrc/sdn_plan.h
+++ b/safe_denoiser_amd/csrc/sdn_plan.h
@@ -161,6 +161,7 @@
   bool res_pre = true;
   bool x3_expand = true;
   bool split_k = false;
+  bool conv_up4 = true;
   struct GraphKey {
     int batch; const void *w, *lat, *text, *pooled, *out, *ws;
     bool operator<(const GraphKey& o) const {
@@ -215,6 +216,9 @@
   bool plan_bad = false;
   bool force_x3t_next = false;
   std::set<int64_t> pairs;
+  struct Up4 { int64_t op; int64_t w9; int N, Cin; };
+  std::vector<Up4> up4_pending;
+  void finish_up4();
   struct Res { std::string pfx; int cout; };
 
   Ref param(const std::string& name, int kind, int rows, int cols, int rows_padded = 0);
diff --git a/safe_denoiser_amd/csrc/sdn_plan_api.hip b/safe_denoiser_amd/csrc/sdn_plan_api.hip
--- a/safe_denoiser_amd/csrc/sdn_plan_api.hip
+++ b/safe_denoiser_amd/csrc/sdn_plan_api.hip
@@ -153,6 +153,11 @@
     if (j.kind == 2) {
       const int rc2 = sdn_expand3_weights((const float*)(W + j.w), j.rows, j.cols, j.group, W + j.wf, stream);
       if (rc2 != SDN_OK) return rc2;
+      continue;
+    }
+    if (j.kind == 3) {
+      const int rc3 = sdn_conv_up4_weights(dt, W + j.w, j.rows, j.cols, W + j.wf, stream);
+      if (rc3 != SDN_OK) return rc3;
       continue;
     }
     if (j.kind == 1) {
@@ -317,6 +322,11 @@
   set_plan_toggle(u, &sdn_unet::split_k, on != 0);
 }
 
+void sdn_unet_set_conv_up4(sdn_unet* u, int32_t on) {
+  if (!u || u->kind != UNET || u->dtype() >= 2 || u->conv_up4 == (on != 0)) return;
+  set_plan_toggle(u, &sdn_unet::conv_up4, on != 0);
+}
+
 void sdn_unet_set_graph_mode(sdn_unet* u, int32_t on) {
   if (!u) return;
   u->use_graph = on != 0;
diff --git a/safe_denoiser_amd/csrc/sdn_plan_core.hip b/safe_denoiser_amd/csrc/sdn_plan_core.hip
--- a/safe_denoiser_amd/csrc/sdn_plan_core.hip
+++ b/safe_denoiser_amd/csrc/sdn_plan_core.hip
@@ -134,7 +134,8 @@
 void Builder::push_gemm(Op& o) {
   o.col = pending_cols; pending_cols = Ref();
   const int nv = o.gd.n_valid > 0 ? o.gd.n_valid : o.gd.N;
-  const int split = (!u->split_k || nv != o.gd.N) ? 1 : sdn_gemm_pick_split(o.gd.M, o.gd.N, o.gd.K, o.gd.act, o.gd.out_kind);
+  const int split = (!u->split_k || nv != o.gd.N || (o.gd.a_mode == SDN_A_CONV3X3 && o.gd.upsample == 2)) ? 1
+                    : sdn_gemm_pick_split(o.gd.M, o.gd.N, o.gd.K, o.gd.act, o.gd.out_kind);
   if (split > 1) {
     const int64_t bytes = (int64_t)split * o.gd.M * o.gd.N * 4;
     const int64_t off = arena.alloc(bytes);
@@ -184,12 +185,35 @@
   o.flops = 2.0 * (double)o.gd.M * (double)cout * (double)o.gd.K;
   o.bytes = 2.0 * ((double)B * in.side * in.side * in.C + (double)n_pad * o.gd.K + (double)o.gd.M * cout) +
             (residual.space != SP_NONE ? 2.0 * (double)o.gd.M * cout : 0.0);
+  const int up4 = (upsample == 1 && u->kind == UNET && es == 2 && stride == 1 && !asym_pad && out_kind == SDN_OUT_BF16 && n_valid == 0 &&
+                   n_pad == cout && residual.space == SP_NONE && rowbias.space == SP_NONE && w.space == SP_W)
+                      ? sdn_conv_up4_tile(in.side, in.side, in.C, n_pad) : 0;
+  if (up4) {
+    up4_pending.push_back({u->conv_up4 ? (int64_t)plan->ops.size() : -1, w.off, n_pad, in.C});
+    if (u->conv_up4) {
+      o.gd.K = 4 * in.C; o.gd.upsample = 2; o.gd.res_pre = 0;
+      o.bytes = 2.0 * ((double)B * in.side * in.side * in.C + 4.0 * n_pad * o.gd.K + (double)o.gd.M * cout);
+      snprintf(o.label, sizeof(o.label), "k_conv_up4<%d>", up4);
+      push_gemm(o);
+      return;
+    }
+  }
   if (Ho == in.side && sdn_conv_slab_shape_ok(o.gd.M, n_pad, in.C, in.side, stride, upsample, asym_pad, out_kind, n_valid) &&
       sdn_gemm_pick_tile(o.gd.M, n_pad, o.gd.K, SDN_ACT_NONE) == 10)
     snprintf(o.label, sizeof(o.label), "k_conv_slab<%d>", in.side);
   else
     snprintf(o.label, sizeof(o.label), "k_gemm<%d>", sdn_gemm_pick_tile(o.gd.M, n_pad, o.gd.K, SDN_ACT_NONE));
   push_gemm(o);
+}
+void Builder::finish_up4() {
+  for (const Up4& p : up4_pending) {
+    const std::string name = "up4@" + std::to_string((long long)p.w9);
+    const bool fresh = u->param_index.find(name) == u->param_index.end();
+    Ref d = derived(name, (int64_t)16 * p.N * p.Cin * 2);
+    if (fresh) { sdn_unet::FoldJob j{p.w9, -1, -1, -1, d.off, -1, -1, p.N, p.Cin}; j.kind = 3; u->fold_jobs.push_back(j); }
+    if (p.op >= 0) plan->ops[(size_t)p.op].w = d;
+  }
+  up4_pending.clear();
 }
 void Builder::groupnorm(const Act& x, const Act* x2, float eps, int silu, Ref gamma, Ref beta, const Act& out) {
   Op o; o.kind = OP_GN; o.a = R(x); if (x2) o.a2 = R(*x2);
diff --git a/safe_denoiser_amd/csrc/sdn_plan_unet.hip b/safe_denoiser_amd/csrc/sdn_plan_unet.hip
--- a/safe_denoiser_amd/csrc/sdn_plan_unet.hip
+++ b/safe_denoiser_amd/csrc/sdn_plan_unet.hip
@@ -384,6 +384,7 @@
   drop(cur);
   conv3x3(g, c.out_channels, npad, cow, cob, Ref{SP_OUT, 0}, 1, 0, Ref(), Ref(), 0, SDN_OUT_F32_NCHW, c.out_channels);
   drop(g);
+  finish_up4();
   plan->kv_base = Arena::up(arena.peak);
   plan->ws_bytes = plan_bad ? -1 : plan->kv_base + kv_top;
 }
diff --git a/safe_denoiser_amd/unet.py b/safe_denoiser_amd/unet.py
--- a/safe_denoiser_amd/unet.py
+++ b/safe_denoiser_amd/unet.py
@@ -50,6 +50,7 @@
                             norm_groups=cfg["norm_num_groups"],
                             dtype=code, latent_repeat=self.latent_repeat)
         self.tail_split = False
+        self.conv_up4 = True
         self._create("sdn_unet_create", c)
 
     def _source_shape(self, p: dict) -> tuple:
@@ -69,6 +70,8 @@
         net = UNet2DConditionModel(text_len=self.text_len, dtype=self.dtype, precision=self.precision,
                                    latent_repeat=self.latent_repeat if latent_repeat is None else latent_repeat, **vars(self.config))
         net._weights = self._weights
+        if not self.conv_up4:
+            net.set_conv_up4(False)
         return net
 
     def set_graph_mode(self, on: bool = True):
@@ -82,6 +85,12 @@
 
     def set_split_k(self, on: bool = True):
         _lib.lib().sdn_unet_set_split_k(self._h, 1 if on else 0)
+        self._ws = {}
+        return self
+
+    def set_conv_up4(self, on: bool = True):
+        _lib.lib().sdn_unet_set_conv_up4(self._h, 1 if on else 0)
+        self.conv_up4 = bool(on)
         self._ws = {}
         return self
 
```

New measurement: 8.841 images/sec (median of 6 runs). 2.4% higher.
